# XuyangBai/D3Feat

Hardware: AMD Instinct MI355X
Metric: fragments/sec (30k-pt clouds) (higher is better)
Workload: dtype f32; 1 GPU; SURVEY §8d config #2: synthetic 3DMatch room fragment, 300k raw pts -> grid subsample 0.03 m (~29k pts per cloud) -> self-pair -> 5-level pyramid -> full KPFCNN forward (random-init weights (reference initialiser, seed 42), 14.1M params)...; points_per_cloud=29369, fragments_per_gpu=2141, parallelism=fragment-dp1, fragments_per_replay=12, engine_fallbacks=0, engine_isolated_replays=0

## Files before the change

d3feat_amd/_lib.py:

```python
import ctypes as C
import os

_HERE = os.path.dirname(os.path.abspath(__file__))
LIB_PATH = os.environ.get("D3FEAT_AMD_LIB") or os.path.join(_HERE, "lib", "libd3feat_amd.so")

D3F_OK = 0
ERRORS = {-1: "HIP runtime / kernel launch failure", -2: "workspace too small", -3: "invalid argument"}
ST_EMPTY_ELEMENT, ST_NEG_CELL, ST_KEY_RANGE, ST_HIT_OVERFLOW, ST_OUT_OVERFLOW, ST_KEY_WIDTH = 1, 2, 4, 8, 16, 32
PAD_NUM_SUPPORTS = -2147483648
NEIGHBOR_CAP = 1024
MAX_BATCH = 255
TOPK_MAX = 8192
PAIRS_KMAX = 1024
REPEAT_COUNTS_MAX = 16
MATCH_KMAX = 8192
VALIDATION_NMAX = 1024
SCENES_MAX = 256
VP_INDEX_RANGE, VP_COUNT_RANGE = 1, 2

_vp, _sz, _i, _f = C.c_void_p, C.c_size_t, C.c_int, C.c_float

SIGNATURES = {
    "d3f_version": (_i, []),
    "d3f_trace_marker": (_i, [_i, _vp]),
    "d3f_pack_status": (_i, [_vp, _vp, _i, _vp, _i, _vp, _i, _vp, _i, _vp, _i, _i, _i, _vp]),
    "d3f_grid_subsample_workspace_bytes": (_sz, [_i, _i, _i, _i]),
    "d3f_batch_grid_subsample": (_i, [_vp, _i, _vp, _i, _f, _vp, _i, _vp, _i, _vp, _vp, _vp, _vp, _vp, _vp, _sz, _vp]),
    "d3f_batch_grid_subsample_async": (_i, [_vp, _i, _vp, _i, _f, _vp, _i, _i, _i, _vp, _vp, _vp, _sz, _vp]),
    "d3f_batch_grid_subsample_async_inplace": (_i, [_vp, _i, _vp, _i, _f, _vp, _i, _i, _vp, _vp, _vp, _sz, _vp]),
    "d3f_stack_self_pair": (_i, [_vp, _i, _vp, _i, _vp, _vp, _vp, _vp]),
    "d3f_radius_neighbors_workspace_bytes": (_sz, [_i, _i, _i]),
    "d3f_batch_radius_neighbors": (_i, [_vp, _i, _vp, _i, _vp, _vp, _i, _f, _vp, _i, _i, _i, _vp, _vp, _sz, _vp]),
    "d3f_neighbor_grid_bytes": (_sz, [_i, _i]),
    "d3f_neighbor_grid_order_offset": (_sz, [_i, _i]),
    "d3f_neighbor_grid_build": (_i, [_vp, _i, _vp, _i, _f, _vp, _sz, _vp]),
    "d3f_neighbor_grid_search": (_i, [_vp, _sz, _i, _vp, _i, _vp, _i, _f, _i, _vp, _i, _i, _i, _i, _i, _f, _i, _vp, _vp]),
    "d3f_neighbor_grid_search_ordered": (_i, [_vp, _sz, _i, _vp, _i, _vp, _i, _f, _vp, _sz, _vp, _i, _i, _i, _i, _i, _f, _i, _vp, _vp]),
    "d3f_neighbor_grid_inv_offset": (_sz, [_i, _i]),
    "d3f_neighbor_grid_xyz_offset": (_sz, [_i, _i]),
    "d3f_row_positive": (_i, [_vp, _i, _i, _i, _vp, _vp, _i, _vp]),
    "d3f_kpconv_aggregate": (_i, [_vp, _i, _vp, _i, _vp, _i, _i, _vp, _i, _i, _vp, _vp, _i, _f, _i, _i, _vp, _vp, _vp, _vp,
                                  _vp, _i, _vp]),
    "d3f_kpconv_deform_aggregate": (_i, [_vp, _i, _vp, _i, _vp, _i, _i, _vp, _i, _i, _vp, _i, _f, _vp, _i, _i, _vp, _i, _f, _i, _i, _vp,
                                         _vp, _vp, _vp, _i, _vp]),
    "d3f_kpconv_fused_c1": (_i, [_vp, _i, _vp, _i, _vp, _i, _i, _vp, _i, _vp, _i, _f, _i, _i, _vp, _i, _vp, _vp, _vp, _i, _i,
                                 _f, _vp, _i, _vp, _vp, _vp, _i, _vp]),
    "d3f_kpconv_fused32": (_i, [_vp, _i, _vp, _i, _vp, _i, _i, _vp, _i, _vp, _vp, _i, _f, _i, _i, _vp, _vp, _vp, _vp, _i, _i, _f, _vp,
                                _i, _vp, _vp, _vp, _i, _vp]),
    "d3f_kpconv_fused_supported": (_i, [_i, _i, _i, _i, _i]),
    "d3f_kpconv_pack_weights": (_i, [_vp, _i, _i, _vp, _vp]),
    "d3f_kpconv_fused": (_i, [_vp, _i, _vp, _i, _vp, _i, _i, _vp, _i, _i, _vp, _vp, _i, _f, _i, _i, _vp, _i, _vp, _vp, _vp, _i, _i,
                              _f, _vp, _i, _vp, _vp, _vp, _i, _vp]),
    "d3f_kpconv_fused32_x3": (_i, [_vp, _i, _vp, _i, _vp, _i, _i, _vp, _i, _vp, _vp, _i, _f, _i, _i, _vp, _vp, _vp, _vp, _i, _i, _f, _vp,
                                   _i, _vp, _vp, _vp, _i, _vp]),
    "d3f_kpconv_packed_x3_bytes": (_sz, [_i, _i]),
    "d3f_kpconv_pack_weights_x3": (_i, [_vp, _i, _i, _vp, _vp]),
    "d3f_kpconv_fused_x3": (_i, [_vp, _i, _vp, _i, _vp, _i, _i, _vp, _i, _i, _vp, _vp, _i, _f, _i, _i, _vp, _i, _vp, _vp, _vp, _i, _i,
                                 _f, _vp, _i, _vp, _vp, _vp, _i, _vp]),
    "d3f_gemm_workspace_bytes": (_sz, [_i, _i, _i, _i]),
    "d3f_gemm_bf16_workspace_bytes": (_sz, [_i, _i, _i, _i]),
    "d3f_gemm_f32": (_i, [_vp, _i, _vp, _i, _vp, _i, _i, _i, _i, _vp, _vp, _vp, _vp, _i, _i, _f, _vp, _sz, _vp, _i, _vp]),
    "d3f_gemm_upsample_cat_f32": (_i, [_vp, _i, _i, _i, _vp, _i, _vp, _i, _i, _vp, _i, _vp, _i, _i, _i, _vp, _vp, _i, _f, _vp, _sz,
                                       _vp, _vp, _i, _vp]),
    "d3f_ind_max_pool": (_i, [_vp, _i, _i, _i, _vp, _i, _i, _i, _vp, _i, _vp, _vp, _vp, _vp, _i, _vp]),
    "d3f_closest_pool_cat": (_i, [_vp, _i, _i, _i, _vp, _i, _i, _vp, _i, _i, _vp, _i, _vp, _vp, _vp]),
    "d3f_affine_act": (_i, [_vp, _i, _i, _i, _vp, _vp, _vp, _i, _i, _f, _vp, _i, _vp, _vp]),
    "d3f_pack_descriptors": (_i, [_vp, _vp, _i, _i, _vp, _i, _vp, _i, _vp, _vp]),
    "d3f_pack_descriptors_to": (_i, [_vp, _vp, _i, _i, _vp, _i, _vp, _i, _vp, _vp, _i, _i, _i, _vp, _vp, _vp]),
    "d3f_topk_workspace_bytes": (_sz, [_i, _i, _i, _i]),
    "d3f_topk_records": (_i, [_vp, _i, _vp, _i, _i, _vp, _i, _i, _vp, _vp, _i, _i, _i, _vp, _i, _i, _vp, _i, _vp, _vp, _vp, _vp, _sz,
                              _vp]),
    "d3f_feature_nn_workspace_bytes": (_sz, [_i]),
    "d3f_feature_nn": (_i, [_vp, _i, _i, _vp, _i, _i, _i, _vp, _vp, _vp, _sz, _vp]),
    "d3f_mutual_matches_workspace_bytes": (_sz, [_i]),
    "d3f_mutual_matches": (_i, [_vp, _i, _vp, _i, _vp, _vp, _vp, _sz, _vp]),
    "d3f_ransac_hypotheses": (_i, [_vp, _i, _vp, _i, _vp, _i, _f, _f, C.c_uint64, C.c_uint64, _i, _vp, _vp, _vp]),
    "d3f_ransac_draw": (_i, [C.c_uint64, C.c_uint64, _i, _i]),
    "d3f_neighbor_grid_score": (_i, [_vp, _sz, _i, _vp, _i, _vp, _i, _f, _vp, _vp, _vp, _vp]),
    "d3f_register_pairs_workspace_bytes": (_sz, [_i, _i, _i, _i]),
    "d3f_register_pairs": (_i, [_vp, _i, _i, _i, _i, _vp, _vp, _i, _i, _f, _i, _f, _f, _i, _i, C.c_uint64, _vp, _f] + [_vp] * 11
                           + [_sz, _vp]),
    "d3f_repeatability_pairs": (_i, [_vp, _i, _i, _i, _vp, _vp, _i, _vp, _i, _vp, _vp, _i, _vp, _vp, _vp]),
    "d3f_match_pairs_workspace_bytes": (_sz, [_i, _vp, _i]),
    "d3f_match_pairs": (_i, [_vp, _i, _i, _i, _i, _vp, _vp, _i, _vp, _f, _vp, _i, _vp, _vp, _vp, _sz, _vp]),
    "d3f_register_pairs_counts_workspace_bytes": (_sz, [_i, _i, _i, _vp, _i, _i]),
    "d3f_register_pairs_counts": (_i, [_vp, _i, _i, _i, _i, _vp, _vp, _i, _vp, _i, _f, _i, _f, _f, _i, _i, C.c_uint64, _vp, _f] + [_vp] * 10
                                  + [_sz, _vp]),
    "d3f_overlap_pairs": (_i, [_vp, _sz, _i, _i, _vp, _i, _f, _vp, _vp, _i, _vp]),
    "d3f_validation_pairs_workspace_bytes": (_sz, [_i, _i]),
    "d3f_validation_pairs": (_i, [_vp, _i, _i, _vp, _i, _vp, _i, _i, _vp, _vp, _vp, _i, _vp, _i, _f, _i, _f, _f, _f, _f] + [_vp] * 5
                             + [_sz, _vp]),
    "d3f_pose_errors": (_i, [_vp, _vp, _i, _i, _vp, _vp, _vp, _vp, _vp, _vp]),
    "d3f_sanitize_descriptors": (_i, [_vp, _i, _i, _i, _i, _vp]),
    "d3f_matching_summary": (_i, [_vp, _vp, _vp, _i, _i, _vp, _i, _vp, _vp, _vp, _vp]),
    "d3f_registration_recall": (_i, [_vp, _i, _vp, _vp, _vp, _vp, _vp, _i, _i, _vp, _i, _vp, _vp, _vp, _vp, _vp]),
    "d3f_icp_pairs_workspace_bytes": (_sz, [_i, _i]),
    "d3f_icp_pairs": (_i, [_vp, _sz, _i, _vp, _i, _vp, _i, _vp, _vp, _i, _i] + [_vp] * 9 + [_sz, _vp]),
    "d3f_gemm_pack_bf16": (_i, [_vp, _i, _i, _i, _vp, _vp]),
    "d3f_gemm_pack_f32t": (_i, [_vp, _i, _i, _i, _vp, _vp]),
    "d3f_gemm_f32t": (_i, [_vp, _i, _i, _i, _vp, _i, _vp, _i, _i, _vp, _vp, _i, _i, _i, _vp, _vp, _vp, _vp, _i, _i, _f, _vp, _sz,
                           _vp, _vp, _i, _vp]),
    "d3f_gemm_x3_packed_bytes": (_sz, [_i, _i]),
    "d3f_gemm_pack_x3": (_i, [_vp, _i, _i, _i, _vp, _vp]),
    "d3f_gemm_x3_workspace_bytes": (_sz, [_i, _i, _i, _i]),
    "d3f_gemm_x3_plan": (_i, [_i, _i, _i, _i, _vp, _vp, _vp]),
    "d3f_gemm_x3_resident": (_i, [_i, _i, _i, _i]),
    "d3f_gemm_x3": (_i, [_vp, _i, _i, _i, _vp, _i, _vp, _i, _i, _vp, _vp, _i, _i, _i, _vp, _vp, _vp, _vp, _i, _i, _f, _vp, _sz,
                         _vp, _vp, _i, _vp]),
    "d3f_gemm_x3_gres": (_i, [_vp, _i, _i, _i, _vp, _i, _vp, _i, _i, _vp, _vp, _i, _i, _i, _vp, _vp, _vp, _vp, _i, _vp, _i, _i, _vp, _i, _f,
                              _vp, _sz, _vp, _vp, _i, _vp]),
    "d3f_gemm_bf16": (_i, [_vp, _i, _i, _i, _vp, _i, _vp, _i, _i, _vp, _vp, _i, _i, _i, _vp, _vp, _vp, _vp, _i, _i, _f, _vp, _sz,
                           _vp, _vp, _i, _i, _i, _vp]),
    "d3f_decode_xyz_records": (_i, [_vp, _i, _i, _i, _i, _i, _i, _i, _vp, _vp]),
    "d3f_detect_head": (_i, [_vp, _i, _i, _i, _vp, _i, _i, _vp, _vp, _i, _i, _vp, _i, _vp, _vp, _vp, _vp]),
}

_lib = None

# ... 26 lines not shown
```

d3feat_amd/csrc/grid_subsample.hip:

```cpp
#include <cstdlib>
#include "prims.h"
#include "radix_sort.h"

#define GS_EMPTY 0xFFFFFFFFFFFFFFFFull
#define GS_KEYBITS 56
#define GS_KEYMASK ((1ull << GS_KEYBITS) - 1ull)
#define GS_MAX_PROBE 4096

__constant__ unsigned long long D3F_CHAIN_DEV[D3F_NCHAIN] = {
    13ull, 29ull, 59ull, 127ull, 257ull, 541ull, 1109ull, 2357ull, 5087ull, 10273ull, 20753ull, 42043ull, 85229ull,
    172933ull, 351061ull, 712697ull, 1447153ull, 2938679ull, 5967347ull, 12117689ull, 24607243ull, 49969847ull,
    101473717ull, 206062531ull, 418451333ull, 849749479ull, 1725587117ull, 3504151727ull};

struct GsElem {
    float org[3];
    int pad0;
    unsigned long long NX, NY, NZ;
    long long bbase;
};

static unsigned long long gs_chain_ge(long long n) {
    for (int j = 0; j < D3F_NCHAIN; ++j)
        if ((long long)D3F_CHAIN_HOST[j] >= n) return D3F_CHAIN_HOST[j];
    return D3F_CHAIN_HOST[D3F_NCHAIN - 1];
}

__device__ __forceinline__ unsigned long long gs_mix(unsigned long long x) {
    x ^= x >> 33; x *= 0xff51afd7ed558ccdull; x ^= x >> 33; x *= 0xc4ceb9fe1a85ec53ull; x ^= x >> 33;
    return x;
}

__device__ __forceinline__ int gs_bits(unsigned long long x) {
    int b = 0;
    while (x) { ++b; x >>= 1; }
    return b;
}
__device__ __forceinline__ void gs_prep(const unsigned* __restrict__ bbox, const int* __restrict__ offs, int B, float dl,
                                        GsElem* __restrict__ el, int* __restrict__ status, RsMeta* __restrict__ smeta,
                                        int n_cap) {
    __shared__ unsigned long long sCells[256];
    const int b = threadIdx.x;
    unsigned long long cells = 0ull;
    if (b < B) {
        GsElem e;
        e.pad0 = 0;
        const int len = offs[b + 1] - offs[b];
        if (len <= 0) {
            atomicOr(&status[1], D3F_ST_EMPTY_ELEMENT);
            e.org[0] = e.org[1] = e.org[2] = 0.f;
            e.NX = e.NY = e.NZ = 1;
        } else {
            const float inv = __fdiv_rn(1.0f, dl);
            float mx[3];
#pragma unroll
            for (int d = 0; d < 3; ++d) {
                float mn = d3f_ord2f(__hip_atomic_load(&bbox[b * 6 + d], __ATOMIC_RELAXED, __HIP_MEMORY_SCOPE_AGENT));
                mx[d] = d3f_ord2f(__hip_atomic_load(&bbox[b * 6 + 3 + d], __ATOMIC_RELAXED, __HIP_MEMORY_SCOPE_AGENT));
                e.org[d] = __fmul_rn(floorf(__fmul_rn(mn, inv)), dl);
            }
            e.NX = (unsigned long long)fmaxf(floorf(__fdiv_rn(__fsub_rn(mx[0], e.org[0]), dl)), 0.f) + 1ull;
            e.NY = (unsigned long long)fmaxf(floorf(__fdiv_rn(__fsub_rn(mx[1], e.org[1]), dl)), 0.f) + 1ull;
            e.NZ = (unsigned long long)fmaxf(floorf(__fdiv_rn(__fsub_rn(mx[2], e.org[2]), dl)), 0.f) + 1ull;
        }
        long long base = 0;
        for (int j = 0; j < b; ++j) {
            long long l = offs[j + 1] - offs[j];
            unsigned long long nb = D3F_CHAIN_DEV[D3F_NCHAIN - 1];
            for (int c = 0; c < D3F_NCHAIN; ++c)
                if ((long long)D3F_CHAIN_DEV[c] >= l) { nb = D3F_CHAIN_DEV[c]; break; }
            base += (long long)nb;
        }
        e.bbase = base;
        el[b] = e;
        const double c = (double)e.NX * (double)e.NY * (double)e.NZ;
        cells = c >= 1.8e19 ? 0xFFFFFFFFFFFFFFFFull : e.NX * e.NY * e.NZ;
    }
    if (!smeta) return;
    sCells[threadIdx.x] = cells;
    __syncthreads();
    if (threadIdx.x == 0) {
        unsigned long long mx = 1ull;
        for (int j = 0; j < B; ++j) mx = sCells[j] > mx ? sCells[j] : mx;
        int kb = gs_bits(mx - 1ull);
        if (kb < 1) kb = 1;
        const int eb = gs_bits((unsigned long long)(B - 1));
        RsMeta m;
        m.n = min(offs[B], n_cap);
        m.kb = kb;
        m.bits = kb + eb;
        if (m.bits > 32) {
            atomicOr(&status[1], D3F_ST_KEY_WIDTH);
            m.n = 0;
            m.bits = 8;
        }
        m.npass = (m.bits + 7) / 8;
        *smeta = m;
    }
}
struct GsPrepEpi {
    const unsigned* bbox; const int* offs; int B; float dl; GsElem* el; int* status; RsMeta* smeta; int n_cap;
    __device__ __forceinline__ void operator()() const { gs_prep(bbox, offs, B, dl, el, status, smeta, n_cap); }
};

__global__ void __launch_bounds__(256) gs_insert_kernel(const float* __restrict__ pts, int N, const int* __restrict__ offs,
                                                        int B, float dl, const GsElem* __restrict__ el,
                                                        unsigned long long* __restrict__ tkey, unsigned* __restrict__ tfirst,
                                                        unsigned long long capmask, int* __restrict__ slot,
                                                        int* __restrict__ status) {
    const int i = blockIdx.x * blockDim.x + threadIdx.x;
    if (i >= min(N, offs[B])) return;
    const int b = d3f_find_elem(offs, B, i);
    const GsElem e = el[b];
    const float fx = floorf(__fdiv_rn(__fsub_rn(pts[3 * (size_t)i + 0], e.org[0]), dl));
    const float fy = floorf(__fdiv_rn(__fsub_rn(pts[3 * (size_t)i + 1], e.org[1]), dl));
    const float fz = floorf(__fdiv_rn(__fsub_rn(pts[3 * (size_t)i + 2], e.org[2]), dl));
    int st = 0;
    if (fx < 0.f || fy < 0.f || fz < 0.f) st |= D3F_ST_NEG_CELL;
    const unsigned long long ix = (unsigned long long)fmaxf(fx, 0.f), iy = (unsigned long long)fmaxf(fy, 0.f),
                             iz = (unsigned long long)fmaxf(fz, 0.f);
    const unsigned long long key = ix + e.NX * iy + e.NX * e.NY * iz;
    if (key > GS_KEYMASK) st |= D3F_ST_KEY_RANGE;
    if (st) atomicOr(&status[1], st);
    const unsigned long long word = ((unsigned long long)b << GS_KEYBITS) | (key & GS_KEYMASK);
    unsigned long long h = gs_mix(word) & capmask;
    bool placed = false;
    for (int probe = 0; probe < GS_MAX_PROBE; ++probe) {
        unsigned long long prev = atomicCAS(&tkey[h], GS_EMPTY, word);
        if (prev == GS_EMPTY || prev == word) { placed = true; break; }
        h = (h + 1) & capmask;
    }
    if (!placed) atomicOr(&status[1], D3F_ST_OUT_OVERFLOW);
    atomicMin(&tfirst[h], (unsigned)i);
    slot[i] = (int)h;
}

struct GsMarkIn {
    const int* n_dev; const int* slot; const unsigned* tfirst;
    __device__ __forceinline__ int operator()(int i) const { return (i < *n_dev && tfirst[slot[i]] == (unsigned)i) ? 1 : 0; }
};

__global__ void __launch_bounds__(256) gs_chain_kernel(int N, const int* __restrict__ slot, const unsigned* __restrict__ tfirst,
                                                       const unsigned long long* __restrict__ tkey,
                                                       const int* __restrict__ vscan, const int* __restrict__ vbase,
                                                       int* __restrict__ pvid,
                                                       unsigned long long* __restrict__ vkey, int* __restrict__ vhead,
                                                       int* __restrict__ vcnt, int* __restrict__ pnext,
                                                       const int* __restrict__ n_dev) {
    const int i = blockIdx.x * blockDim.x + threadIdx.x;
    if (i >= min(N, *n_dev)) return;
    const int s = slot[i];
    const int fi = (int)tfirst[s];
    const int v = d3f_scan_at(vscan, vbase, fi);
    pvid[i] = v;
    if (fi == i) vkey[v] = tkey[s] & GS_KEYMASK;
    pnext[i] = atomicExch(&vhead[v], i);
    atomicAdd(&vcnt[v], 1);
}

struct GsRankScan {
    const int* vscan; const int* vbase;
    __device__ __forceinline__ int operator()(int p) const { return d3f_scan_at(vscan, vbase, p); }
};
struct GsRankBits {
    const unsigned* fbits; const int* wscan; const int* wbase;
    __device__ __forceinline__ int operator()(int p) const {
        const int w = p >> 5;
        return d3f_scan_at(wscan, wbase, w) + __popc(fbits[w] & ((1u << (p & 31)) - 1u));
    }
};
template <class Rank>
struct GsMoffsEpi {
    const int* offs; int B; Rank rank; int* meta; int* moffs; int* sub_lens; int* status_dev;
    int out_cap;
    int elem_cap;
    __device__ __forceinline__ void operator()(int M) const {
        if (threadIdx.x != 0) return;
        meta[0] = M;
        const int N = offs[B];
        for (int b = 0; b <= B; ++b) moffs[b] = (b == B || offs[b] >= N) ? M : rank(offs[b]);
        bool over = M > out_cap ||
                    (__hip_atomic_load(&meta[1], __ATOMIC_RELAXED, __HIP_MEMORY_SCOPE_AGENT) & (D3F_ST_OUT_OVERFLOW | D3F_ST_KEY_WIDTH));
        for (int b = 0; b < B; ++b) over = over || (moffs[b + 1] - moffs[b] > elem_cap);
        if (over && !(__hip_atomic_load(&meta[1], __ATOMIC_RELAXED, __HIP_MEMORY_SCOPE_AGENT) & D3F_ST_KEY_WIDTH))
            atomicOr(&meta[1], D3F_ST_OUT_OVERFLOW);
        for (int b = 0; b < B; ++b) {
// ... 343 lines not shown
            const unsigned ix = (unsigned)fmaxf(fx, 0.f), iy = (unsigned)fmaxf(fy, 0.f), iz = (unsigned)fmaxf(fz, 0.f);
            const unsigned k = ix + NX * (iy + NY * iz);
            key[r] = (kb < 32 ? ((unsigned)b << kb) : 0u) | (kb < 32 ? (k & ((1u << kb) - 1u)) : k);
            skey[i] = key[r];
            vm |= 1u << r;
        }
    }
    if (st) atomicOr(&status[1], st);
    rs_tile_histogram(key, vm, 0, sHist, hist + (size_t)tile * 256);
}

__global__ void __launch_bounds__(256) gs_heads_kernel(int N, const RsMeta* __restrict__ smeta, const unsigned* __restrict__ key0,
                                                       const unsigned* __restrict__ key1, const unsigned* __restrict__ val0,
                                                       const unsigned* __restrict__ val1, unsigned* __restrict__ fbits) {
    const int j = blockIdx.x * blockDim.x + threadIdx.x;
    if (j >= min(N, smeta->n)) return;
    const unsigned* __restrict__ ks = (smeta->npass & 1) ? key1 : key0;
    const unsigned* __restrict__ vs = (smeta->npass & 1) ? val1 : val0;
    const unsigned k = ks[j];
    if (j == 0 || ks[j - 1] != k) {
        const unsigned i = vs[j];
        atomicOr(&fbits[i >> 5], 1u << (i & 31u));
    }
}
struct GsBitsIn {
    const unsigned* fbits;
    __device__ __forceinline__ int operator()(int w) const { return __popc(fbits[w]); }
};
__global__ void __launch_bounds__(256) gs_runs_kernel(int N, const RsMeta* __restrict__ smeta, const unsigned* __restrict__ key0,
                                                      const unsigned* __restrict__ key1, const unsigned* __restrict__ val0,
                                                      const unsigned* __restrict__ val1, GsRankBits rank,
                                                      const float* __restrict__ pts, const float* const* __restrict__ ptrs,
                                                      const int* __restrict__ offs, unsigned long long* __restrict__ vkey,
                                                      float* __restrict__ bary) {
    __shared__ float sx[256], sy[256], sz[256];
    __shared__ unsigned sk[256];
    const int n = min(N, smeta->n);
    const int j0 = blockIdx.x * 256;
    if (j0 >= n) return;
    const int t = threadIdx.x, j = j0 + t;
    const unsigned* __restrict__ ks = (smeta->npass & 1) ? key1 : key0;
    const unsigned* __restrict__ vs = (smeta->npass & 1) ? val1 : val0;
    unsigned k = 0u, pi = 0u, kprev = 0u;
    float px = 0.f, py = 0.f, pz = 0.f;
    if (j < n) {
        k = ks[j];
        pi = vs[j];
        kprev = j > 0 ? ks[j - 1] : 0u;
        if (ptrs) {
            const int b = smeta->kb < 32 ? (int)(k >> smeta->kb) : 0;
            pts = ptrs[b] - 3 * (size_t)offs[b];
        }
        px = pts[3 * (size_t)pi + 0]; py = pts[3 * (size_t)pi + 1]; pz = pts[3 * (size_t)pi + 2];
    }
    sx[t] = px; sy[t] = py; sz[t] = pz;
    sk[t] = k;
    __syncthreads();
    if (j >= n || (j != 0 && kprev == k)) return;
    const int v = rank((int)pi);
    float ax = px, ay = py, az = pz;
    int c = 1;
    const int lim = min(256, n - j0);
    while (t + c < lim && sk[t + c] == k) {
        ax = __fadd_rn(ax, sx[t + c]);
        ay = __fadd_rn(ay, sy[t + c]);
        az = __fadd_rn(az, sz[t + c]);
        ++c;
    }
    if (t + c == 256) {
        while (j + c < n && ks[j + c] == k) {
            const size_t q = vs[j + c];
            ax = __fadd_rn(ax, pts[3 * q + 0]);
            ay = __fadd_rn(ay, pts[3 * q + 1]);
            az = __fadd_rn(az, pts[3 * q + 2]);
            ++c;
        }
    }
    const float sc = (float)(1.0 / (double)c);
    vkey[v] = (unsigned long long)(smeta->kb < 32 ? (k & ((1u << smeta->kb) - 1u)) : k);
    bary[3 * (size_t)v + 0] = __fmul_rn(ax, sc);
    bary[3 * (size_t)v + 1] = __fmul_rn(ay, sc);
    bary[3 * (size_t)v + 2] = __fmul_rn(az, sc);
}
__global__ void __launch_bounds__(256) gs_emit_kernel(int* __restrict__ status, const int* __restrict__ moffs, int B,
                                                      const int* __restrict__ vpos, const float* __restrict__ bary,
                                                      float* __restrict__ out_p, int out_cap) {
    const int v = blockIdx.x * blockDim.x + threadIdx.x;
    if (v >= status[0]) return;
    if (status[1] & (D3F_ST_OUT_OVERFLOW | D3F_ST_KEY_WIDTH)) return;
    const int b = d3f_find_elem(moffs, B, v);
    const size_t dest = (size_t)moffs[b] + (size_t)vpos[v];
    if (dest >= (size_t)out_cap) {
        atomicOr(&status[1], D3F_ST_OUT_OVERFLOW);
        return;
    }
    out_p[3 * dest + 0] = bary[3 * (size_t)v + 0];
    out_p[3 * dest + 1] = bary[3 * (size_t)v + 1];
    out_p[3 * dest + 2] = bary[3 * (size_t)v + 2];
}


__global__ void __launch_bounds__(256) gs_accum_kernel(const float* __restrict__ pts, const float* __restrict__ feat,
                                                       int fdim, int* __restrict__ status,
                                                       const int* __restrict__ moffs, int B,
                                                       const int* __restrict__ vstart, const int* __restrict__ sbase,
                                                       const int* __restrict__ vcnt,
                                                       const int* __restrict__ sorted, const int* __restrict__ vpos,
                                                       float* __restrict__ out_p, float* __restrict__ out_f, int out_cap) {
    const int v = blockIdx.x * blockDim.x + threadIdx.x;
    if (v >= status[0]) return;
    const int b = d3f_find_elem(moffs, B, v);
    const int n = vcnt[v], st = sbase ? d3f_scan_at(vstart, sbase, v) : vstart[v];
    const size_t dest = (size_t)moffs[b] + (size_t)vpos[v];
    if (dest >= (size_t)out_cap) {
        atomicOr(&status[1], D3F_ST_OUT_OVERFLOW);
        return;
    }
    float sx = 0.f, sy = 0.f, sz = 0.f;
    for (int t = 0; t < n; ++t) {
        const size_t i = (size_t)sorted[st + t];
        sx = __fadd_rn(sx, pts[3 * i + 0]);
        sy = __fadd_rn(sy, pts[3 * i + 1]);
        sz = __fadd_rn(sz, pts[3 * i + 2]);
    }
    const float sc = (float)(1.0 / (double)n);
    out_p[3 * dest + 0] = __fmul_rn(sx, sc);
    out_p[3 * dest + 1] = __fmul_rn(sy, sc);
    out_p[3 * dest + 2] = __fmul_rn(sz, sc);
    if (fdim > 0) {
        const float cf = (float)n;
        for (int f = 0; f < fdim; ++f) {
            float s = 0.f;
            for (int t = 0; t < n; ++t) s = __fadd_rn(s, feat[(size_t)sorted[st + t] * fdim + f]);
            out_f[dest * fdim + f] = __fdiv_rn(s, cf);
        }
    }
}

__global__ void __launch_bounds__(256) gs_fill_kernel(int* __restrict__ p, size_t n, int v) {
    const size_t i = (size_t)blockIdx.x * blockDim.x + threadIdx.x;
    if (i < n) p[i] = v;
}
__global__ void __launch_bounds__(256) gs_labels_kernel(int N, int ldim, const int* __restrict__ cls,
                                                        const int* __restrict__ pvid, const int* __restrict__ moffs, int B,
                                                        const int* __restrict__ vpos, int* __restrict__ out_c) {
    const int i = blockIdx.x * blockDim.x + threadIdx.x;
    if (i >= N) return;
    const int v = pvid[i];
    const int b = d3f_find_elem(moffs, B, v);
    const size_t dest = (size_t)moffs[b] + (size_t)vpos[v];
    for (int l = 0; l < ldim; ++l) atomicMax(&out_c[dest * ldim + l], cls[(size_t)i * ldim + l]);
}

struct GsLayout {
    size_t cap;
    long long bucket_total;
};
static GsLayout gs_layout(int N, int B, int keys = -1) {
    GsLayout L;
    L.cap = 64;
    const size_t nk = (size_t)((keys > 0 && keys < N) ? keys : (N > 0 ? N : 1));
    while (L.cap < (size_t)2 * nk) L.cap <<= 1;
    L.bucket_total = (long long)(2.24 * (double)N) + 16ll * B + 64;
    return L;
}

extern "C" size_t d3f_grid_subsample_workspace_bytes(int N, int B, int fdim, int ldim) {
    (void)fdim; (void)ldim;
    if (N < 0 || B < 1) return 0;
    GsLayout L = gs_layout(N, B);
    size_t n = (size_t)(N > 0 ? N : 1);
    size_t bytes = 0;
    bytes += d3f_align((B + 1) * sizeof(int)) * 2 + d3f_align((B + 2) * sizeof(int));
    bytes += d3f_align(B * 6 * sizeof(unsigned));
    bytes += d3f_align(B * sizeof(GsElem));
    bytes += d3f_align(L.cap * sizeof(unsigned long long));
    bytes += d3f_align(L.cap * sizeof(int));
    bytes += d3f_align(n * sizeof(unsigned long long));
    bytes += 16 * d3f_align(n * sizeof(int));
    bytes += 6 * d3f_align((size_t)L.bucket_total * sizeof(int));
    bytes += d3f_align((n / GS_TILE + B + 8) * sizeof(int));
    bytes += 2 * d3f_align(d3f_scan_base_ints(N) * sizeof(int)) + d3f_align((4 + D3F_NCHAIN * (size_t)B) * sizeof(unsigned));
    bytes += d3f_align(rs_hist_words(N) * sizeof(unsigned)) + d3f_align((n / 32 + 2) * sizeof(unsigned)) +
             d3f_align(3 * n * sizeof(float)) + d3f_align(sizeof(RsMeta));
    bytes += d3f_align(7 * (size_t)B * (n < 16384 ? n : 16384) * sizeof(float)) + 256 + 2 * d3f_align(B * sizeof(int));
    return bytes + 4096;
}

template <int T, int R>
static int gs_small_launch(const GsSmallArgs& A, float* sub_points, int* sub_lens_dev, int* status_dev, hipStream_t stream) {
    static std::atomic<unsigned long long> lds_done{0ull};
    const void* const fns[] = {(const void*)gs_small_kernel<T, R>};
    if (d3f_opt_in_lds(lds_done, fns, (int)gss_lds_bytes<T, R>(GSS_NB_MAX)) != D3F_OK) return D3F_ERR_HIP;
    gs_small_kernel<T, R><<<A.B, T, gss_lds_bytes<T, R>(A.nbmax), stream>>>(A);
    D3F_LAUNCH_CHECK();
    gs_small_pack_kernel<<<d3f_cdiv(A.out_cap, 256), 256, 0, stream>>>(A, sub_points, sub_lens_dev, status_dev);
    D3F_LAUNCH_CHECK();
    return D3F_OK;
}
static int gs_run_small(const float* points, int N, const int* lens_dev, int B, float dl, float* sub_points, int M_cap, int elem_cap,
                        int pc, int* sub_lens_dev, int* status_dev, void* workspace, size_t workspace_bytes, hipStream_t stream) {
    if (elem_cap <= 0 || elem_cap > M_cap) elem_cap = M_cap;
    if (elem_cap > pc) elem_cap = pc;
    D3fArena ar(workspace, workspace_bytes);
    GsSmallArgs A;
    A.stage = ar.take<float>(3 * (size_t)B * (size_t)elem_cap);
    A.recs = ar.take<float>(4 * (size_t)B * (size_t)elem_cap);
    A.mcount = ar.take<int>(B);
    A.cflags = ar.take<int>(B);
    if (!ar.ok) return D3F_ERR_WORKSPACE;
    A.pts = points; A.lens = lens_dev; A.B = B; A.dl = dl; A.elem_cap = elem_cap; A.pc = pc; A.out_cap = M_cap;
    A.nbmax = GSS_NB_MAX;
    for (int j = 0; j < D3F_NCHAIN; ++j)
        if ((long long)D3F_CHAIN_HOST[j] >= (long long)elem_cap) { A.nbmax = (int)D3F_CHAIN_HOST[j]; break; }
    if (A.nbmax > GSS_NB_MAX) A.nbmax = GSS_NB_MAX;
    if (A.nbmax < 1109) A.nbmax = 1109;
    if (pc <= 2048) return gs_small_launch<256, 8>(A, sub_points, sub_lens_dev, status_dev, stream);
    if (pc <= 4096) return gs_small_launch<512, 8>(A, sub_points, sub_lens_dev, status_dev, stream);
    if (pc <= 8192) return gs_small_launch<1024, 8>(A, sub_points, sub_lens_dev, status_dev, stream);
    if (pc <= 12288) return gs_small_launch<1024, 12>(A, sub_points, sub_lens_dev, status_dev, stream);
    return gs_small_launch<1024, 16>(A, sub_points, sub_lens_dev, status_dev, stream);
}

static int gs_run(const float* points, int N, const int* lens_dev, int B, float dl, const float* features, int fdim,
                  const int* classes, int ldim, float* sub_points, int M_cap, int elem_cap, int elem_points, float* sub_features,
                  int* sub_classes, int* sub_lens_dev, int* status_host, int* status_dev, void* workspace,
                  size_t workspace_bytes, hipStream_t stream, const float* const* ptrs = nullptr) {
    const bool async = status_dev != nullptr;
    if (async && !features && ldim == 0 && !ptrs) {
        const int pc = (elem_points > 0 && elem_points < N) ? elem_points : N;
        int ec = (elem_cap > 0 && elem_cap < M_cap) ? elem_cap : M_cap;
        if (ec > pc) ec = pc;
        if (pc <= 16384 && ec <= GSS_NB_MAX) return gs_run_small(points, N, lens_dev, B, dl, sub_points, M_cap, elem_cap, pc, sub_lens_dev, status_dev,
                                             workspace, workspace_bytes, stream);
    }
    GsLayout L = gs_layout(N, B, async ? M_cap : -1);
    D3fArena ar(workspace, workspace_bytes);
    const size_t n = (size_t)N;
    int* offs = ar.take<int>(B + 1);
    int* moffs = ar.take<int>(B + 1);
    unsigned* bbox = ar.take<unsigned>(B * 6);
    GsElem* el = ar.take<GsElem>(B);
    const int ncounters = 4 + D3F_NCHAIN * B;
    unsigned* counters = ar.take<unsigned>(ncounters);
    unsigned long long* tkey = ar.take<unsigned long long>(L.cap);
    unsigned* tfirst = ar.take<unsigned>(L.cap);
    int* vhead = ar.take<int>(n);
    int* meta = ar.take<int>(B + 2);
    int* vcnt = ar.take<int>(n);
    unsigned long long* vkey = ar.take<unsigned long long>(n);
    int* slot = ar.take<int>(n);
    int* vscan = ar.take<int>(n);
    int* pvid = ar.take<int>(n);
    int* pnext = ar.take<int>(n);
    int* vstart = ar.take<int>(n);
    int* sorted = ar.take<int>(n);
    GsOrderArgs A;
    A.vpos = ar.take<int>(n);
    A.P[0] = ar.take<int>(n);
    A.P[1] = ar.take<int>(n);
    A.nx[0] = ar.take<int>(n);
    A.nx[1] = ar.take<int>(n);
    A.cd = ar.take<int>(n);
    A.bkt[0] = ar.take<int>(n);
    A.bkt[1] = ar.take<int>(n);
    for (int k = 0; k < 2; ++k) {
        A.bf[k] = ar.take<int>((size_t)L.bucket_total);
        A.bc[k] = ar.take<int>((size_t)L.bucket_total);
        A.bh[k] = ar.take<int>((size_t)L.bucket_total);
    }
    A.tsum = ar.take<int>(n / GS_TILE + B + 8);
    int* vbase = ar.take<int>(d3f_scan_base_ints(N));
    int* sbase = ar.take<int>(d3f_scan_base_ints(N));
    const bool use_sort = async && !features && ldim == 0;
    unsigned* rs_hist = ar.take<unsigned>(rs_hist_words(N));
    unsigned* fbits = ar.take<unsigned>(n / 32 + 2);
    float* bary = ar.take<float>(3 * n);
    RsMeta* smeta = ar.take<RsMeta>(1);
    if (!ar.ok) return D3F_ERR_WORKSPACE;
    A.vkey = vkey; A.moffs = moffs; A.offs = offs; A.el = el;
    if (elem_cap <= 0 || elem_cap > M_cap) elem_cap = M_cap;
    if (elem_cap > N) elem_cap = N;
    A.max_m = async ? elem_cap : 0x7fffffff;

    int rc;
    const D3fFill none{nullptr, 0ull, 0u};
    const unsigned long long ones_words = (unsigned long long)((char*)(vhead + n) - (char*)tkey) / 4ull;
    const unsigned long long zero_words = (unsigned long long)((char*)(vcnt + n) - (char*)meta) / 4ull;
    if ((rc = use_sort ? d3f_begin_launch(lens_dev, B, offs, bbox, counters, ncounters, D3fFill{fbits, (unsigned long long)(n / 32 + 2), 0u},
                                          D3fFill{(unsigned*)meta, (unsigned long long)(B + 2), 0u}, none, none, stream)
                       : d3f_begin_launch(lens_dev, B, offs, bbox, counters, ncounters, D3fFill{(unsigned*)tkey, ones_words, 0xFFFFFFFFu},
                                          D3fFill{(unsigned*)meta, zero_words, 0u}, none, none, stream)) != D3F_OK) return rc;
    GsPrepEpi prep{bbox, offs, B, dl, el, meta, use_sort ? smeta : nullptr, N};
    if ((rc = d3f_bbox_launch_t(points, offs, B, N, bbox, counters, prep, stream, ptrs)) != D3F_OK) return rc;
    const int nblk = d3f_cdiv(N, 256);
    const int elem_lim = async ? elem_cap : 0x7fffffff;
    int M, maxM;
    if (use_sort) {
        unsigned *key0 = (unsigned*)slot, *key1 = (unsigned*)pnext, *val0 = (unsigned*)pvid, *val1 = (unsigned*)sorted;
        gs_sortkey_kernel<<<rs_tiles(N), RS_THREADS, 0, stream>>>(points, ptrs, offs, B, dl, el, smeta, key0, rs_hist, meta);
        D3F_LAUNCH_CHECK();
        if ((rc = rs_sort_launch(smeta, N, key0, key1, val0, val1, rs_hist, stream)) != D3F_OK) return rc;
        gs_heads_kernel<<<nblk, 256, 0, stream>>>(N, smeta, key0, key1, val0, val1, fbits);
        D3F_LAUNCH_CHECK();
        const GsRankBits rank{fbits, vscan, vbase};
        GsMoffsEpi<GsRankBits> mepi{offs, B, rank, meta, moffs, sub_lens_dev, status_dev, M_cap, elem_lim};
        if ((rc = d3f_scan_fold_launch(GsBitsIn{fbits}, N / 32 + 1, nullptr, vscan, vbase, counters + 1, mepi, stream)) != D3F_OK)
            return rc;
        gs_runs_kernel<<<nblk, 256, 0, stream>>>(N, smeta, key0, key1, val0, val1, rank, points, ptrs, offs, vkey, bary);
        D3F_LAUNCH_CHECK();
        M = N < M_cap ? N : M_cap;
        maxM = elem_cap;
    } else {
    GsMoffsEpi<GsRankScan> mepi{offs, B, GsRankScan{vscan, vbase}, meta, moffs, sub_lens_dev, status_dev, M_cap, elem_lim};
    gs_insert_kernel<<<nblk, 256, 0, stream>>>(points, N, offs, B, dl, el, tkey, tfirst, (unsigned long long)L.cap - 1ull,
                                               slot, meta);
    D3F_LAUNCH_CHECK();
    if ((rc = d3f_scan_fold_launch(GsMarkIn{offs + B, slot, tfirst}, N, offs + B, vscan, vbase, counters + 1, mepi, stream)) != D3F_OK)
        return rc;
    if (!async) {
        D3F_HIP_TRY(hipMemcpyAsync(status_host, meta, (B + 2) * sizeof(int), hipMemcpyDeviceToHost, stream));
        D3F_HIP_TRY(hipStreamSynchronize(stream));
        M = status_host[0];
        if (status_host[1] != 0 || M <= 0) return D3F_OK;
        maxM = 0;
        for (int b = 0; b < B; ++b) maxM = status_host[2 + b] > maxM ? status_host[2 + b] : maxM;
    } else {
        M = N < M_cap ? N : M_cap;
        maxM = elem_cap;
    }

    gs_chain_kernel<<<nblk, 256, 0, stream>>>(N, slot, tfirst, tkey, vscan, vbase, pvid, vkey, vhead, vcnt, pnext, offs + B);
    D3F_LAUNCH_CHECK();
    if ((rc = d3f_scan_fold_launch(D3fScanIn{vcnt}, async ? N : M, meta, vstart, sbase, counters + 2, D3fNoEpi{}, stream)) != D3F_OK)
        return rc;
    gs_rank_kernel<<<nblk, 256, 0, stream>>>(N, offs + B, pvid, vhead, pnext, vstart, sbase, sorted);
    }
    const int small_last = GS_SMALL_LAST;
    gs_order_small_kernel<<<B, GS_SMALL_T, 0, stream>>>(A, small_last);
    for (int j = small_last + 1; j < D3F_NCHAIN && (long long)D3F_CHAIN_HOST[j - 1] < (long long)maxM; ++j) {
        const long long nbj = (long long)D3F_CHAIN_HOST[j];
        const int hi = (int)((long long)maxM < nbj ? (long long)maxM : nbj);
        const bool more = j + 1 < D3F_NCHAIN && nbj < (long long)maxM;
        const long long nbn = more ? (long long)D3F_CHAIN_HOST[j + 1] : 0;
        const int hin = more ? (int)((long long)maxM < nbn ? (long long)maxM : nbn) : hi;
        dim3 g(d3f_cdiv(hi, 256), B), gt(d3f_cdiv(hi, GS_TILE), B), gp(d3f_cdiv(hin > hi ? hin : hi, 256), B);
        if (j == small_last + 1) gs_order_insert_kernel<<<g, 256, 0, stream>>>(A, j);
        gs_order_scan_tiles_kernel<<<gt, 256, 0, stream>>>(A, j, B, counters + 4 + j * B);
        gs_order_place_kernel<<<gp, 256, 0, stream>>>(A, j);
    }
    if (use_sort)
        gs_emit_kernel<<<d3f_cdiv(M, 256), 256, 0, stream>>>(meta, moffs, B, A.vpos, bary, sub_points, M_cap);
    else
        gs_accum_kernel<<<d3f_cdiv(async ? N : M, 256), 256, 0, stream>>>(points, features, fdim, meta, moffs, B, vstart, sbase,
                                                                         vcnt, sorted, A.vpos, sub_points, sub_features, M_cap);
    if (ldim > 0) {
        const size_t tot = (size_t)M * (size_t)ldim;
        gs_fill_kernel<<<d3f_cdiv((long long)tot, 256), 256, 0, stream>>>(sub_classes, tot, (int)0x80000000);
        gs_labels_kernel<<<nblk, 256, 0, stream>>>(N, ldim, classes, pvid, moffs, B, A.vpos, sub_classes);
    }
    D3F_LAUNCH_CHECK();
    return D3F_OK;
}

extern "C" int d3f_batch_grid_subsample(const float* points, int N, const int* lens_dev, int B, float dl,
                                        const float* features, int fdim, const int* classes, int ldim,
                                        float* sub_points, float* sub_features, int* sub_classes, int* sub_lens_dev,
                                        int* status_host, void* workspace, size_t workspace_bytes, void* stream_) {
    hipStream_t stream = (hipStream_t)stream_;
    if (N < 0 || N > (1 << 30) || B < 1 || B > D3F_MAX_BATCH || !(dl > 0.f) || fdim < 0 || ldim < 0) return D3F_ERR_ARG;
    if (!points || !lens_dev || !sub_points || !sub_lens_dev || !status_host) return D3F_ERR_ARG;
    if ((fdim > 0 && (!features || !sub_features)) || (ldim > 0 && (!classes || !sub_classes))) return D3F_ERR_ARG;
    for (int i = 0; i < B + 2; ++i) status_host[i] = 0;
    if (N == 0) return d3f_fill_u32(sub_lens_dev, B, 0u, stream);
    return gs_run(points, N, lens_dev, B, dl, features, fdim, classes, ldim, sub_points, N, N, 0, sub_features, sub_classes,
                  sub_lens_dev, status_host, nullptr, workspace, workspace_bytes, stream);
}

extern "C" int d3f_batch_grid_subsample_async(const float* points, int N_cap, const int* lens_dev, int B, float dl,
                                              float* sub_points, int M_cap, int elem_cap, int elem_points_cap, int* sub_lens_dev,
                                              int* status_dev, void* workspace, size_t workspace_bytes, void* stream_) {
    hipStream_t stream = (hipStream_t)stream_;
    if (N_cap < 1 || N_cap > (1 << 30) || M_cap < 1 || elem_cap < 0 || elem_points_cap < 0 || B < 1 || B > D3F_MAX_BATCH || !(dl > 0.f))
        return D3F_ERR_ARG;
    if (!points || !lens_dev || !sub_points || !sub_lens_dev || !status_dev) return D3F_ERR_ARG;
    return gs_run(points, N_cap, lens_dev, B, dl, nullptr, 0, nullptr, 0, sub_points, M_cap, elem_cap, elem_points_cap, nullptr,
                  nullptr, sub_lens_dev, nullptr, status_dev, workspace, workspace_bytes, stream);
}

extern "C" int d3f_batch_grid_subsample_async_inplace(const float* const* clouds_dev, int N_cap, const int* lens_dev, int B, float dl,
                                                      float* sub_points, int M_cap, int elem_cap, int* sub_lens_dev, int* status_dev,
                                                      void* workspace, size_t workspace_bytes, void* stream_) {
    hipStream_t stream = (hipStream_t)stream_;
    if (N_cap < 1 || N_cap > (1 << 30) || M_cap < 1 || elem_cap < 0 || B < 1 || B > D3F_MAX_BATCH || !(dl > 0.f)) return D3F_ERR_ARG;
    if (!clouds_dev || !lens_dev || !sub_points || !sub_lens_dev || !status_dev) return D3F_ERR_ARG;
    return gs_run(nullptr, N_cap, lens_dev, B, dl, nullptr, 0, nullptr, 0, sub_points, M_cap, elem_cap, 0, nullptr, nullptr, sub_lens_dev,
                  nullptr, status_dev, workspace, workspace_bytes, stream, clouds_dev);
}

__global__ void __launch_bounds__(256) gs_stack_pair_kernel(const float* __restrict__ pts, int M_cap, const int* __restrict__ lens_in,
                                                            int B, float* __restrict__ out, int* __restrict__ lens_out,
                                                            int* __restrict__ total) {
    const int i = blockIdx.x * blockDim.x + threadIdx.x;
    int tot = 0;
    for (int b = 0; b < B; ++b) tot += lens_in[b];
    tot = min(tot, M_cap);
    if (i == 0) {
        int room = M_cap;
        for (int b = 0; b < B; ++b) {
            const int m = min(lens_in[b], room);
            room -= m;
            lens_out[2 * b] = m;
            lens_out[2 * b + 1] = m;
        }
        *total = 2 * tot;
    }
    if (i >= 3 * tot) return;
    const int pi = i / 3, c = i - 3 * pi;
    int start = 0, m = 0;
    for (int b = 0; b < B; ++b) {
        m = lens_in[b];
        if (pi < start + m || b == B - 1) break;
        start += m;
    }
    m = min(m, tot - start);
    const float v = pts[i];
    const size_t row = 2 * (size_t)start + (size_t)(pi - start);
    out[3 * row + c] = v;
    out[3 * (row + m) + c] = v;
}

extern "C" int d3f_stack_self_pair(const float* pts, int M_cap, const int* lens_in_dev, int B, float* out, int* lens_out_dev,
                                   int* total_dev, void* stream_) {
    hipStream_t stream = (hipStream_t)stream_;
    if (M_cap < 1 || B < 1 || 2 * B > D3F_MAX_BATCH || !pts || !lens_in_dev || !out || !lens_out_dev || !total_dev)
        return D3F_ERR_ARG;
    gs_stack_pair_kernel<<<d3f_cdiv(3ll * M_cap, 256), 256, 0, stream>>>(pts, M_cap, lens_in_dev, B, out, lens_out_dev, total_dev);
    D3F_LAUNCH_CHECK();
    return D3F_OK;
}
```

d3feat_amd/csrc/gs_small.h:

```cpp
#pragma once

#define GSS_NB_MAX 5087

struct GsSmallArgs {
    const float* pts;
    const int* lens;
    int B;
    float dl;
    float* stage;
    float* recs;
    int elem_cap;
    int pc;
    int out_cap;
    int nbmax;
    int* mcount;
    int* cflags;
};

template <int T>
__device__ __forceinline__ int gss_block_excl_scan(int v, int* __restrict__ wsum, int* total) {
    const int lane = threadIdx.x & 63, w = threadIdx.x >> 6;
    int x = v;
#pragma unroll
    for (int d = 1; d < 64; d <<= 1) {
        const int y = __shfl_up(x, d, 64);
        if (lane >= d) x += y;
    }
    if (lane == 63) wsum[w] = x;
    __syncthreads();
    int base = 0, tot = 0;
#pragma unroll
    for (int q = 0; q < T / 64; ++q) {
        const int s = wsum[q];
        if (q < w) base += s;
        tot += s;
    }
    __syncthreads();
    *total = tot;
    return base + x - v;
}

template <int T, int R>
static inline size_t gss_lds_bytes(int nbmax) {
    const size_t sortw = 2 * (size_t)T * R + (size_t)(T / 64) * 256 + 2 * ((size_t)T * R / 32);
    const size_t orderw = 7 * (size_t)nbmax;
    return (128 + (sortw > orderw ? sortw : orderw)) * 4;
}

template <int T, int R>
__global__ void __launch_bounds__(T) gs_small_kernel(GsSmallArgs A) {
    extern __shared__ __attribute__((aligned(16))) unsigned gss_lds[];
    constexpr int W = T / 64, NI = T * R;
    int* sScr = (int*)gss_lds;
    unsigned* sK = gss_lds + 128;
    unsigned* sV = sK + NI;
    unsigned (*sCnt)[256] = (unsigned (*)[256])(sV + NI);
    unsigned* sBits = sV + NI + W * 256;
    int* sWS = (int*)(sBits + NI / 32);
    const int b = blockIdx.x, tid = threadIdx.x, lane = tid & 63, w = tid >> 6;
    int lo = 0;
    for (int j = 0; j < b; ++j) lo += A.lens[j];
    const int len = A.lens[b];
    int* sFlag = sScr + 127;
    if (tid == 0) { A.mcount[b] = 0; *sFlag = 0; }
    if (len <= 0 || len > NI || len > A.pc) {
        if (tid == 0) A.cflags[b] = len <= 0 ? D3F_ST_EMPTY_ELEMENT : D3F_ST_OUT_OVERFLOW;
        return;
    }
    const float* __restrict__ P = A.pts + 3 * (size_t)lo;
    const float dl = A.dl;

    unsigned mn[3] = {0xFFFFFFFFu, 0xFFFFFFFFu, 0xFFFFFFFFu}, mx[3] = {0u, 0u, 0u};
    for (int i = tid; i < len; i += T) {
#pragma unroll
        for (int d = 0; d < 3; ++d) {
            const unsigned u = d3f_f2ord(P[3 * (size_t)i + d]);
            mn[d] = min(mn[d], u);
            mx[d] = max(mx[d], u);
        }
    }
#pragma unroll
    for (int d = 0; d < 3; ++d) {
#pragma unroll
        for (int o = 32; o > 0; o >>= 1) {
            mn[d] = min(mn[d], (unsigned)__shfl_xor((int)mn[d], o, 64));
            mx[d] = max(mx[d], (unsigned)__shfl_xor((int)mx[d], o, 64));
        }
    }
    if (lane == 0) {
#pragma unroll
        for (int d = 0; d < 3; ++d) { sScr[w * 6 + d] = (int)mn[d]; sScr[w * 6 + 3 + d] = (int)mx[d]; }
    }
    __syncthreads();
    float org[3];
    unsigned dims[3];
    {
        const float inv = __fdiv_rn(1.0f, dl);
#pragma unroll
        for (int d = 0; d < 3; ++d) {
// ... 129 lines not shown
    }

    float4* __restrict__ rec = (float4*)A.recs + (size_t)b * (size_t)A.elem_cap;
#pragma unroll
    for (int r = 0; r < R; ++r) {
        if (headmask & (1u << r)) {
            const int i = base + r * 64;
            const unsigned k = key[r];
            unsigned pi = val[r];
            const int vid = sWS[pi >> 5] + __popc(sBits[pi >> 5] & ((1u << (pi & 31u)) - 1u));
            float sx = P[3 * (size_t)pi + 0], sy = P[3 * (size_t)pi + 1], sz = P[3 * (size_t)pi + 2];
            int c = 1;
            while (i + c < len && sK[i + c] == k) {
                pi = sV[i + c];
                sx = __fadd_rn(sx, P[3 * (size_t)pi + 0]);
                sy = __fadd_rn(sy, P[3 * (size_t)pi + 1]);
                sz = __fadd_rn(sz, P[3 * (size_t)pi + 2]);
                ++c;
            }
            const float sc = (float)(1.0 / (double)c);
            rec[vid] = make_float4(__fmul_rn(sx, sc), __fmul_rn(sy, sc), __fmul_rn(sz, sc), __uint_as_float(k));
        }
    }
    __syncthreads();

    const int NB = A.nbmax;
    unsigned* sKey = gss_lds + 128;
    int* sBF = (int*)(sKey + NB);
    int* sBC = sBF + NB;
    int* sBH = sBC + NB;
    int* sNX = sBH + NB;
    int* sL0 = sNX + NB;
    int* sL1 = sL0 + NB;
    for (int v = tid; v < M; v += T) sKey[v] = __float_as_uint(rec[v].w);
    __syncthreads();
    int* La = sL0;
    int* Lb = sL1;
    int lo_r = 0;
    for (int j = 0; j < D3F_NCHAIN; ++j) {
        const int nb = (int)D3F_CHAIN_DEV[j];
        const double inv_nb = 1.0 / (double)nb;
        const bool last = M <= nb;
        const int hi = last ? M : nb;
        for (int t = tid; t < nb; t += T) { sBF[t] = 0x7fffffff; sBC[t] = 0; sBH[t] = -1; }
        __syncthreads();
        for (int t = tid; t < hi; t += T) {
            const int id = (t < lo_r) ? La[t] : t;
            const int bk = gs_mod((unsigned long long)sKey[id], (unsigned)nb, inv_nb);
            atomicMin(&sBF[bk], t);
            atomicAdd(&sBC[bk], 1);
            sNX[t] = atomicExch(&sBH[bk], t);
        }
        __syncthreads();
        int carry = 0;
        for (int c0 = 0; c0 < hi; c0 += T) {
            const int u = c0 + tid, t = hi - 1 - u;
            int c = 0, bk = 0;
            if (u < hi) {
                const int id = (t < lo_r) ? La[t] : t;
                bk = gs_mod((unsigned long long)sKey[id], (unsigned)nb, inv_nb);
                c = (sBF[bk] == t) ? sBC[bk] : 0;
            }
            int tot;
            const int e = gss_block_excl_scan<T>(c, sScr, &tot);
            if (u < hi && sBF[bk] == t) sBC[bk] = carry + e;
            carry += tot;
        }
        __syncthreads();
        for (int t = tid; t < hi; t += T) {
            const int id = (t < lo_r) ? La[t] : t;
            const int bk = gs_mod((unsigned long long)sKey[id], (unsigned)nb, inv_nb);
            int rk = 0;
            for (int q = sBH[bk]; q >= 0; q = sNX[q]) rk += (q > t) ? 1 : 0;
            const int dest = sBC[bk] + rk;
            if (last) Lb[id] = dest;
            else Lb[dest] = id;
        }
        __syncthreads();
        int* tmp = La; La = Lb; Lb = tmp;
        if (last) break;
        lo_r = hi;
    }
    float* __restrict__ out = A.stage + 3 * (size_t)b * (size_t)A.elem_cap;
    for (int v = tid; v < M; v += T) {
        const float4 q = rec[v];
        const size_t d = (size_t)La[v];
        out[3 * d + 0] = q.x;
        out[3 * d + 1] = q.y;
        out[3 * d + 2] = q.z;
    }
    if (tid == 0) { A.mcount[b] = M; A.cflags[b] = *sFlag; }
}

__global__ void __launch_bounds__(256) gs_small_pack_kernel(GsSmallArgs A, float* __restrict__ out, int* __restrict__ sub_lens,
                                                            int* __restrict__ status_dev) {
    __shared__ int sOff[D3F_MAX_BATCH + 1];
    if (threadIdx.x == 0) {
        int s = 0;
        for (int b = 0; b < A.B; ++b) { sOff[b] = s; s += A.mcount[b]; }
        sOff[A.B] = s;
    }
    __syncthreads();
    const int M = sOff[A.B];
    int flags = 0;
    for (int b = 0; b < A.B; ++b) flags |= A.cflags[b];
    const bool over = M > A.out_cap || (flags & (D3F_ST_OUT_OVERFLOW | D3F_ST_KEY_WIDTH));
    if (blockIdx.x == 0) {
        for (int b = threadIdx.x; b < A.B; b += 256) sub_lens[b] = over ? 0 : A.mcount[b];
        if (threadIdx.x == 0) {
            const int fl = flags | ((M > A.out_cap) ? D3F_ST_OUT_OVERFLOW : 0);
            status_dev[0] = over ? 0 : M;
            status_dev[1] = fl;
        }
    }
    if (over) return;
    const int i = blockIdx.x * 256 + threadIdx.x;
    if (i >= M) return;
    int b = 0;
    while (b + 1 < A.B && i >= sOff[b + 1]) ++b;
    const float* __restrict__ src = A.stage + 3 * ((size_t)b * (size_t)A.elem_cap + (size_t)(i - sOff[b]));
    out[3 * (size_t)i + 0] = src[0];
    out[3 * (size_t)i + 1] = src[1];
    out[3 * (size_t)i + 2] = src[2];
}
```

d3feat_amd/csrc/prims.h:

```cpp
#pragma once
#include "common.h"

#define D3F_SCAN_TILE 1024

struct D3fFill {
    unsigned* p;
    unsigned long long n;
    unsigned v;
};

__device__ __forceinline__ bool d3f_last_block(unsigned* counter, unsigned nblocks) {
    __shared__ int last_flag;
    asm volatile("s_waitcnt vmcnt(0)" ::: "memory");
    __syncthreads();
    if (threadIdx.x == 0) {
        __builtin_amdgcn_fence(__ATOMIC_RELEASE, "agent");
        asm volatile("s_waitcnt vmcnt(0)" ::: "memory");
        const unsigned t = atomicAdd(counter, 1u);
        last_flag = (t == nblocks - 1u) ? 1 : 0;
        if (last_flag) __builtin_amdgcn_fence(__ATOMIC_ACQUIRE, "agent");
    }
    __syncthreads();
    return last_flag != 0;
}

static __global__ void __launch_bounds__(256) begin_kernel(const int* __restrict__ lens, int B, int* __restrict__ offs,
                                                    unsigned* __restrict__ bbox, unsigned* __restrict__ counters,
                                                    int ncounters, D3fFill f0, D3fFill f1, D3fFill f2, D3fFill f3) {
    const size_t tid = (size_t)blockIdx.x * blockDim.x + threadIdx.x, stride = (size_t)gridDim.x * blockDim.x;
    if (blockIdx.x == 0) {
        if (threadIdx.x == 0 && lens) {
            int s = 0;
            for (int b = 0; b < B; ++b) { offs[b] = s; s += lens[b]; }
            offs[B] = s;
        }
        if (bbox)
            for (int i = threadIdx.x; i < B * 6; i += blockDim.x) bbox[i] = ((i % 6) < 3) ? 0xFFFFFFFFu : 0u;
        for (int i = threadIdx.x; i < ncounters; i += blockDim.x) counters[i] = 0u;
    }
    const D3fFill f[4] = {f0, f1, f2, f3};
#pragma unroll
    for (int k = 0; k < 4; ++k) {
        unsigned* p = f[k].p;
        const size_t n = (size_t)f[k].n;
        if (n == 0) continue;
        const size_t n4 = (((uintptr_t)p & 15) == 0) ? n / 4 : 0;
        const uint4 v4 = make_uint4(f[k].v, f[k].v, f[k].v, f[k].v);
        for (size_t j = tid; j < n4; j += stride) ((uint4*)p)[j] = v4;
        for (size_t j = n4 * 4 + tid; j < n; j += stride) p[j] = f[k].v;
    }
}

static inline int d3f_begin_launch(const int* lens, int B, int* offs, unsigned* bbox, unsigned* counters, int ncounters,
                                   D3fFill f0, D3fFill f1, D3fFill f2, D3fFill f3, hipStream_t stream) {
    const unsigned long long words = f0.n + f1.n + f2.n + f3.n;
    long long blocks = (long long)(words / 4 / 256) + 1;
    if (blocks > 1024) blocks = 1024;
    begin_kernel<<<(int)blocks, 256, 0, stream>>>(lens, B, offs, bbox, counters, ncounters, f0, f1, f2, f3);
    D3F_LAUNCH_CHECK();
    return D3F_OK;
}

template <class Epi>
__global__ void __launch_bounds__(256) bbox_kernel(const float* __restrict__ pts, const float* const* __restrict__ ptrs,
                                                   const int* __restrict__ offs, int B,
                                                   unsigned* __restrict__ bbox, unsigned* __restrict__ counter, Epi epi) {
    const int b = blockIdx.y;
    const int lo = offs[b], hi = offs[b + 1];
    if (ptrs) pts = ptrs[b] - 3 * (size_t)lo;
    unsigned mn[3] = {0xFFFFFFFFu, 0xFFFFFFFFu, 0xFFFFFFFFu}, mx[3] = {0u, 0u, 0u};
    const int stride = gridDim.x * blockDim.x;
    for (int i = lo + blockIdx.x * blockDim.x + threadIdx.x; i < hi; i += 4 * stride) {
        float v[4][3];
#pragma unroll
        for (int u = 0; u < 4; ++u) {
            const int iu = min(i + u * stride, hi - 1);
#pragma unroll
            for (int d = 0; d < 3; ++d) v[u][d] = pts[3 * (size_t)iu + d];
        }
#pragma unroll
        for (int u = 0; u < 4; ++u) {
#pragma unroll
            for (int d = 0; d < 3; ++d) {
                const unsigned x = d3f_f2ord(v[u][d]);
                mn[d] = min(mn[d], x);
                mx[d] = max(mx[d], x);
            }
        }
    }
#pragma unroll
    for (int d = 0; d < 3; ++d) {
#pragma unroll
        for (int o = 32; o > 0; o >>= 1) {
            mn[d] = min(mn[d], (unsigned)__shfl_xor((int)mn[d], o, 64));
            mx[d] = max(mx[d], (unsigned)__shfl_xor((int)mx[d], o, 64));
        }
    }
    __shared__ unsigned red[4][6];
    const int wv = threadIdx.x >> 6;
    if ((threadIdx.x & 63) == 0) {
#pragma unroll
        for (int d = 0; d < 3; ++d) { red[wv][d] = mn[d]; red[wv][3 + d] = mx[d]; }
    }
    __syncthreads();
    if (threadIdx.x < 6 && lo < hi) {
        unsigned v = red[0][threadIdx.x];
        for (int k = 1; k < 4; ++k) v = (threadIdx.x < 3) ? min(v, red[k][threadIdx.x]) : max(v, red[k][threadIdx.x]);
        if (threadIdx.x < 3) atomicMin(&bbox[b * 6 + threadIdx.x], v);
        else atomicMax(&bbox[b * 6 + threadIdx.x], v);
    }
    if (d3f_last_block(counter, gridDim.x * gridDim.y)) epi();
}

template <class Epi>
static inline int d3f_bbox_launch_t(const float* pts, const int* offs, int B, int N, unsigned* bbox, unsigned* counter, Epi epi,
                                    hipStream_t stream, const float* const* ptrs = nullptr) {
    int chunks = d3f_cdiv(d3f_cdiv(N > 0 ? N : 1, B), 256 * 8);
    const int per_elem = 512 / B > 1 ? 512 / B : 1;
    if (chunks > per_elem) chunks = per_elem;
    bbox_kernel<Epi><<<dim3(chunks, B), 256, 0, stream>>>(pts, ptrs, offs, B, bbox, counter, epi);
    D3F_LAUNCH_CHECK();
    return D3F_OK;
}

__device__ __forceinline__ int d3f_block_excl_scan_256(int v, int* lds4, int* total) {
    const int lane = threadIdx.x & 63, w = threadIdx.x >> 6;
    int x = v;
#pragma unroll
    for (int d = 1; d < 64; d <<= 1) {
        const int y = __shfl_up(x, d, 64);
        if (lane >= d) x += y;
    }
    if (lane == 63) lds4[w] = x;
    __syncthreads();
    int base = 0, tot = 0;
#pragma unroll
    for (int i = 0; i < 4; ++i) {
        const int s = lds4[i];
        if (i < w) base += s;
        tot += s;
    }
    __syncthreads();
    *total = tot;
    return base + x - v;
}

__device__ __forceinline__ int d3f_scan_at(const int* __restrict__ local, const int* __restrict__ base, int i) {
    return local[i] + base[i / D3F_SCAN_TILE];
}

template <class In, class Epi>
__global__ void __launch_bounds__(256) scan_fold_kernel(In in, int n, const int* __restrict__ n_dev, int* __restrict__ local,
                                                        int* __restrict__ base, unsigned* __restrict__ counter, Epi epi) {
    __shared__ int lds[4];
    n = d3f_dyn(n, n_dev);
    const int live = max(1, (n + D3F_SCAN_TILE - 1) / D3F_SCAN_TILE);
    if ((int)blockIdx.x >= live) return;
    const int i0 = blockIdx.x * D3F_SCAN_TILE + threadIdx.x * 4;
    int v[4], s = 0;
#pragma unroll
    for (int k = 0; k < 4; ++k) {
        v[k] = (i0 + k < n) ? in(i0 + k) : 0;
        s += v[k];
    }
    int tot;
    int ex = d3f_block_excl_scan_256(s, lds, &tot);
#pragma unroll
    for (int k = 0; k < 4; ++k) {
        if (i0 + k < n) local[i0 + k] = ex;
        ex += v[k];
    }
    if (threadIdx.x == 0) base[blockIdx.x] = tot;
    if (!d3f_last_block(counter, (unsigned)live)) return;
    const int nblocks = live;
    int carry = 0;
    for (int c = 0; c < nblocks; c += 256) {
        const int i = c + threadIdx.x;
        const int x = (i < nblocks) ? __hip_atomic_load(&base[i], __ATOMIC_RELAXED, __HIP_MEMORY_SCOPE_AGENT) : 0;
        int t;
        const int e = d3f_block_excl_scan_256(x, lds, &t);
        if (i < nblocks) base[i] = carry + e;
        carry += t;
    }
    __syncthreads();
    epi(carry);
}

struct D3fScanIn {
    const int* p;
    __device__ __forceinline__ int operator()(int i) const { return p[i]; }
};
struct D3fNoEpi {
    __device__ __forceinline__ void operator()(int) const {}
    __device__ __forceinline__ void operator()() const {}
};

static inline size_t d3f_scan_base_ints(int n) { return (size_t)d3f_cdiv(n > 0 ? n : 1, D3F_SCAN_TILE) + 64; }

template <class In, class Epi>
static inline int d3f_scan_fold_launch(In in, int n, const int* n_dev, int* local, int* base, unsigned* counter, Epi epi,
                                       hipStream_t stream) {
    const int nb = d3f_cdiv(n > 0 ? n : 1, D3F_SCAN_TILE);
    scan_fold_kernel<In, Epi><<<nb, 256, 0, stream>>>(in, n, n_dev, local, base, counter, epi);
    D3F_LAUNCH_CHECK();
    return D3F_OK;
}
```

d3feat_amd/csrc/radius_neighbors.hip:

```cpp
#include "prims.h"
#include <cstdlib>

struct NbElem {
    double mn[3];
    double inv_h;
    int dims[3];
    int cbase;
};

#define NB_WAVES_PER_BLOCK 4
#define NB_EL_LDS 40

__device__ __forceinline__ void nb_prep(const unsigned* __restrict__ bbox, const int* __restrict__ soffs, int B, float radius,
                                        long long cell_budget, NbElem* __restrict__ el, int* __restrict__ ncells_total) {
    if (threadIdx.x != 0) return;
    long long base = 0;
    const long long per = cell_budget / B;
    for (int b = 0; b < B; ++b) {
        NbElem e;
        const int len = soffs[b + 1] - soffs[b];
        if (len <= 0) {
            e.mn[0] = e.mn[1] = e.mn[2] = 0.0;
            e.inv_h = 1.0;
            e.dims[0] = e.dims[1] = e.dims[2] = 1;
        } else {
            double mx[3];
            for (int d = 0; d < 3; ++d) {
                e.mn[d] = (double)d3f_ord2f(__hip_atomic_load(&bbox[b * 6 + d], __ATOMIC_RELAXED, __HIP_MEMORY_SCOPE_AGENT));
                mx[d] = (double)d3f_ord2f(__hip_atomic_load(&bbox[b * 6 + 3 + d], __ATOMIC_RELAXED, __HIP_MEMORY_SCOPE_AGENT));
            }
            double h = (double)radius * (1.0 + 1.0 / 1048576.0);
            if (!(h > 0.0)) h = 1.0;
            bool fits = false;
            for (int it = 0; it < 64; ++it) {
                e.inv_h = 1.0 / h;
                double tot = 1.0;
                for (int d = 0; d < 3; ++d) {
                    double n = floor((mx[d] - e.mn[d]) * e.inv_h) + 1.0;
                    e.dims[d] = (n < 1073741824.0) ? (int)n : 1073741824;
                    tot *= n;
                }
                if (tot <= (double)per) { fits = true; break; }
                h *= 2.0;
            }
            if (!fits) {
                e.mn[0] = e.mn[1] = e.mn[2] = 0.0;
                e.inv_h = 0.0;
                e.dims[0] = e.dims[1] = e.dims[2] = 1;
            }
        }
        e.cbase = (int)base;
        base += (long long)e.dims[0] * e.dims[1] * e.dims[2];
        el[b] = e;
    }
    ncells_total[0] = (int)base;
    ncells_total[1] = (int)base + 1;
}

struct NbPrepEpi {
    const unsigned* bbox; const int* soffs; int B; float radius; long long cell_budget; NbElem* el; int* ncells;
    __device__ __forceinline__ void operator()() const { nb_prep(bbox, soffs, B, radius, cell_budget, el, ncells); }
};

__device__ __forceinline__ void nb_cell_of(const NbElem& e, float x, float y, float z, int& cx, int& cy, int& cz) {
    cx = (int)floor(((double)x - e.mn[0]) * e.inv_h);
    cy = (int)floor(((double)y - e.mn[1]) * e.inv_h);
    cz = (int)floor(((double)z - e.mn[2]) * e.inv_h);
}

__global__ void __launch_bounds__(256) nb_count_kernel(const float* __restrict__ s, int Ns, const int* __restrict__ soffs,
                                                       int B, const NbElem* __restrict__ el, int* __restrict__ cell_of,
                                                       int* __restrict__ cell_cnt) {
    const int i = blockIdx.x * blockDim.x + threadIdx.x;
    if (i >= min(Ns, soffs[B])) return;
    const int b = d3f_find_elem(soffs, B, i);
    const NbElem e = el[b];
    int cx, cy, cz;
    nb_cell_of(e, s[3 * (size_t)i], s[3 * (size_t)i + 1], s[3 * (size_t)i + 2], cx, cy, cz);
    cx = min(max(cx, 0), e.dims[0] - 1);
    cy = min(max(cy, 0), e.dims[1] - 1);
    cz = min(max(cz, 0), e.dims[2] - 1);
    const int c = e.cbase + cx + e.dims[0] * (cy + e.dims[1] * cz);
    cell_of[i] = c;
    atomicAdd(&cell_cnt[c], 1);
}

__global__ void __launch_bounds__(256) nb_scatter_kernel(const float* __restrict__ s, int Ns, const int* __restrict__ ns_dev,
                                                         const int* __restrict__ cell_of,
                                                         const int* __restrict__ cell_start, const int* __restrict__ cell_base,
                                                         int* __restrict__ cell_cur,
                                                         float4* __restrict__ sorted, int* __restrict__ order,
                                                         int* __restrict__ inv, float* __restrict__ xyz) {
    const int i = blockIdx.x * blockDim.x + threadIdx.x;
    if (i >= min(Ns, *ns_dev)) return;
    const int c = cell_of[i];
    const int pos = d3f_scan_at(cell_start, cell_base, c) + atomicAdd(&cell_cur[c], 1);
    const float x = s[3 * (size_t)i], y = s[3 * (size_t)i + 1], z = s[3 * (size_t)i + 2];
    sorted[pos] = make_float4(x, y, z, __int_as_float(i));
    order[pos] = i;
    inv[i] = pos;
    xyz[3 * (size_t)pos] = x; xyz[3 * (size_t)pos + 1] = y; xyz[3 * (size_t)pos + 2] = z;
}

template <int J>
__device__ __forceinline__ unsigned nb_xor_lane(unsigned v) {
    if constexpr (J == 1) return (unsigned)__builtin_amdgcn_mov_dpp((int)v, 0xB1, 0xF, 0xF, true);
    else if constexpr (J == 2) return (unsigned)__builtin_amdgcn_mov_dpp((int)v, 0x4E, 0xF, 0xF, true);
    else return (unsigned)__builtin_amdgcn_ds_swizzle((int)v, (J << 10) | 0x1F);
}
template <int J>
__device__ __forceinline__ void nb_cmpx(unsigned& hi, unsigned& lo, bool take_min) {
    const unsigned phi = nb_xor_lane<J>(hi), plo = nb_xor_lane<J>(lo);
    const bool p_less = (phi < hi) || (phi == hi && plo < lo);
    const bool take_p = (take_min == p_less);
    hi = take_p ? phi : hi;
    lo = take_p ? plo : lo;
}
__device__ __forceinline__ void nb_bitonic64(int lane, unsigned& h0, unsigned& l0, unsigned& h1, unsigned& l1) {
#define NB_STAGE(K_, J_)                                                                         \
    do {                                                                                         \
        const bool low_ = (lane & (J_)) == 0;                                                    \
        const bool up0_ = ((K_) >= 32) ? true : ((lane & (K_)) == 0);                            \
        const bool up1_ = ((K_) == 64) ? true : (((K_) == 32) ? false : ((lane & (K_)) == 0));   \
        nb_cmpx<J_>(h0, l0, up0_ == low_);                                                       \
        nb_cmpx<J_>(h1, l1, up1_ == low_);                                                       \
    } while (0)
    NB_STAGE(2, 1);
    NB_STAGE(4, 2); NB_STAGE(4, 1);
    NB_STAGE(8, 4); NB_STAGE(8, 2); NB_STAGE(8, 1);
    NB_STAGE(16, 8); NB_STAGE(16, 4); NB_STAGE(16, 2); NB_STAGE(16, 1);
    NB_STAGE(32, 16); NB_STAGE(32, 8); NB_STAGE(32, 4); NB_STAGE(32, 2); NB_STAGE(32, 1);
    {
        const bool swap = (h1 < h0) || (h1 == h0 && l1 < l0);
        const unsigned th = swap ? h1 : h0, tl = swap ? l1 : l0;
        h1 = swap ? h0 : h1; l1 = swap ? l0 : l1;
        h0 = th; l0 = tl;
    }
    NB_STAGE(64, 16); NB_STAGE(64, 8); NB_STAGE(64, 4); NB_STAGE(64, 2); NB_STAGE(64, 1);
#undef NB_STAGE
}

__device__ __forceinline__ void nb_cmpx_own(unsigned& ha, unsigned& la, unsigned& hb, unsigned& lb, bool ascending) {
    const bool b_less = (hb < ha) || (hb == ha && lb < la);
    const bool swap = (b_less == ascending);
    const unsigned th = swap ? hb : ha, tl = swap ? lb : la;
    hb = swap ? ha : hb; lb = swap ? la : lb;
    ha = th; la = tl;
}
__device__ __forceinline__ void nb_bitonic64x16(int lane, unsigned (&h)[4], unsigned (&l)[4]) {
#define NB_UP(K_, S_) (((K_) == 64) ? true : ((K_) >= 16 ? ((((S_) * 16) & (K_)) == 0) : ((lane & (K_)) == 0)))
#define NB_XSTAGE(K_, J_)                                                                        \
    do {                                                                                         \
        const bool low_ = (lane & (J_)) == 0;                                                    \
        nb_cmpx<J_>(h[0], l[0], NB_UP(K_, 0) == low_);                                           \
        nb_cmpx<J_>(h[1], l[1], NB_UP(K_, 1) == low_);                                           \
        nb_cmpx<J_>(h[2], l[2], NB_UP(K_, 2) == low_);                                           \
        nb_cmpx<J_>(h[3], l[3], NB_UP(K_, 3) == low_);                                           \
    } while (0)
    NB_XSTAGE(2, 1);
    NB_XSTAGE(4, 2); NB_XSTAGE(4, 1);
    NB_XSTAGE(8, 4); NB_XSTAGE(8, 2); NB_XSTAGE(8, 1);
    NB_XSTAGE(16, 8); NB_XSTAGE(16, 4); NB_XSTAGE(16, 2); NB_XSTAGE(16, 1);
    nb_cmpx_own(h[0], l[0], h[1], l[1], true);
    nb_cmpx_own(h[2], l[2], h[3], l[3], false);
    NB_XSTAGE(32, 8); NB_XSTAGE(32, 4); NB_XSTAGE(32, 2); NB_XSTAGE(32, 1);
    nb_cmpx_own(h[0], l[0], h[2], l[2], true);
    nb_cmpx_own(h[1], l[1], h[3], l[3], true);
    nb_cmpx_own(h[0], l[0], h[1], l[1], true);
    nb_cmpx_own(h[2], l[2], h[3], l[3], true);
    NB_XSTAGE(64, 8); NB_XSTAGE(64, 4); NB_XSTAGE(64, 2); NB_XSTAGE(64, 1);
#undef NB_XSTAGE
#undef NB_UP
}

template <bool FIRST_ONLY, int LPQ, bool HINT>
__device__ __forceinline__ void
nb_search_body(const float* __restrict__ q, int Nq, const int* __restrict__ qlens, int B,
               const NbElem* __restrict__ el, const int* __restrict__ cell_start, const int* __restrict__ cell_base,
               const float4* __restrict__ sorted,
               const float4* __restrict__ qorder, float r2, int pad, const int* __restrict__ ns_dev, int* __restrict__ out,
               int ld, int width, int cap, int* __restrict__ status, int want_kmax, float nn_hint, const int* __restrict__ inv) {
    extern __shared__ __attribute__((aligned(16))) char smem[];
    constexpr int QPB = 64 * NB_WAVES_PER_BLOCK / LPQ;
    const int grp = threadIdx.x / LPQ, lane = threadIdx.x % LPQ;
// ... 110 lines not shown
    };
    if (FIRST_ONLY && HINT) {
        scan(true);
        if (!(n > 0 && bd2 <= 0.998f * nn_hint * nn_hint)) scan(false);
    } else {
        scan(false);
    }
    if (lane == 0) {
        if (want_kmax && n > __hip_atomic_load(&status[0], __ATOMIC_RELAXED, __HIP_MEMORY_SCOPE_AGENT)) atomicMax(&status[0], n);
        if (!FIRST_ONLY && n > cap) atomicOr(&status[1], D3F_ST_HIT_OVERFLOW);
    }
    int* row = out + (size_t)(inv ? wq : qi) * ld;
    if (FIRST_ONLY) {
        if (lane == 0 && width > 0) row[0] = (n > 0) ? (inv ? inv[bidx] : bidx) : pad;
        for (int j = 1 + lane; j < width; j += LPQ) row[j] = pad;
        return;
    }
    const int m = min(n, cap);
    const int m4 = (m + 3) & ~3;
    if (m + lane < m4) { hd2[m + lane] = 3.4e38f; hidx[m + lane] = 0x7fffffff; }
    __builtin_amdgcn_fence(__ATOMIC_RELEASE, "wavefront");
    __builtin_amdgcn_wave_barrier();
    if (LPQ == 16 && n <= 64 && cap >= 64) {
        unsigned h[4], l4[4];
#pragma unroll
        for (int sl = 0; sl < 4; ++sl) {
            h[sl] = 0xFFFFFFFFu; l4[sl] = 0xFFFFFFFFu;
            if (lane + 16 * sl < m) { h[sl] = __float_as_uint(hd2[lane + 16 * sl]); l4[sl] = (unsigned)hidx[lane + 16 * sl]; }
        }
        nb_bitonic64x16(lane, h, l4);
        const int mw = min(m, width);
#pragma unroll
        for (int sl = 0; sl < 4; ++sl)
            if (lane + 16 * sl < mw) row[lane + 16 * sl] = inv ? inv[(int)l4[sl]] : (int)l4[sl];
        for (int j = m + lane; j < width; j += LPQ) row[j] = pad;
        return;
    }
    if (LPQ == 32 && n <= 64 && cap >= 64) {
        unsigned h0 = 0xFFFFFFFFu, l0 = 0xFFFFFFFFu, h1 = 0xFFFFFFFFu, l1 = 0xFFFFFFFFu;
        if (lane < m) { h0 = __float_as_uint(hd2[lane]); l0 = (unsigned)hidx[lane]; }
        if (lane + 32 < m) { h1 = __float_as_uint(hd2[lane + 32]); l1 = (unsigned)hidx[lane + 32]; }
        nb_bitonic64(lane, h0, l0, h1, l1);
        const int mw = min(m, width);
        if (lane < mw) row[lane] = inv ? inv[(int)l0] : (int)l0;
        if (lane + 32 < mw) row[lane + 32] = inv ? inv[(int)l1] : (int)l1;
        for (int j = m + lane; j < width; j += LPQ) row[j] = pad;
        return;
    }
    for (int e0 = 0; e0 < m; e0 += LPQ) {
        const int ei = e0 + lane;
        if (ei < m) {
            const float kd = hd2[ei];
            const int ki = hidx[ei];
            int rank = 0;
            for (int j = 0; j < m4; j += 4) {
                const float4 dj = *(const float4*)&hd2[j];
                const int4 ij = *(const int4*)&hidx[j];
                rank += (dj.x < kd || (dj.x == kd && ij.x < ki)) ? 1 : 0;
                rank += (dj.y < kd || (dj.y == kd && ij.y < ki)) ? 1 : 0;
                rank += (dj.z < kd || (dj.z == kd && ij.z < ki)) ? 1 : 0;
                rank += (dj.w < kd || (dj.w == kd && ij.w < ki)) ? 1 : 0;
            }
            if (rank < width) row[rank] = inv ? inv[ki] : ki;
        }
    }
    for (int j = m + lane; j < width; j += LPQ) row[j] = pad;
}

template <bool FIRST_ONLY, int LPQ, bool HINT>
__global__ void __launch_bounds__(64 * NB_WAVES_PER_BLOCK)
nb_search_kernel(const float* __restrict__ q, int Nq, const int* __restrict__ qlens, int B,
                 const NbElem* __restrict__ el, const int* __restrict__ cell_start, const int* __restrict__ cell_base,
                 const float4* __restrict__ sorted,
                 const float4* __restrict__ qorder, float r2, int pad, const int* __restrict__ ns_dev, int* __restrict__ out,
                 int ld, int width, int cap, int* __restrict__ status, int want_kmax, float nn_hint, const int* __restrict__ inv) {
    nb_search_body<FIRST_ONLY, LPQ, HINT>(q, Nq, qlens, B, el, cell_start, cell_base, sorted, qorder, r2, pad, ns_dev, out, ld, width,
                                          cap, status, want_kmax, nn_hint, inv);
}

#include "nb_cell_search.h"
#include "nb_nearest.h"
#include "nb_overlap.h"

static long long nb_cell_budget(int Ns) {
    long long b = 4ll * (long long)(Ns > 0 ? Ns : 1);
    if (b < (1ll << 16)) b = 1ll << 16;
    if (b > (1ll << 28)) b = 1ll << 28;
    return b;
}

struct NbGrid {
    int* soffs; unsigned* bbox; NbElem* el; int* ncells; unsigned* counters; int* cell_cnt; int* cell_cur; int* cell_start; int* cell_of;
    float4* sorted; int* order; int* stmp;
    int* inv;
    float* xyz;
    long long cells;
    bool ok;
};
static NbGrid nb_carve(void* ws, size_t bytes, int Ns, int B) {
    NbGrid g;
    g.cells = nb_cell_budget(Ns) + 8;
    D3fArena ar(ws, bytes);
    const size_t ns = (size_t)(Ns > 0 ? Ns : 1);
    g.soffs = ar.take<int>(B + 1);
    g.bbox = ar.take<unsigned>(B * 6);
    g.el = ar.take<NbElem>(B);
    g.ncells = ar.take<int>(16);
    g.counters = (unsigned*)(g.ncells + 8);
    g.cell_cnt = ar.take<int>((size_t)g.cells * 2);
    g.cell_cur = g.cell_cnt ? g.cell_cnt + g.cells : nullptr;
    g.cell_start = ar.take<int>((size_t)g.cells);
    g.cell_of = ar.take<int>(ns);
    g.sorted = ar.take<float4>(ns);
    g.order = ar.take<int>(ns);
    g.stmp = ar.take<int>(d3f_scan_base_ints((int)g.cells));
    g.inv = ar.take<int>(ns);
    g.xyz = ar.take<float>(3 * ns);
    g.ok = ar.ok;
    return g;
}

extern "C" size_t d3f_neighbor_grid_bytes(int Ns, int B) {
    if (Ns < 0 || B < 1) return 0;
    const long long cells = nb_cell_budget(Ns) + 8;
    const size_t ns = (size_t)(Ns > 0 ? Ns : 1);
    size_t bytes = 0;
    bytes += d3f_align((B + 1) * sizeof(int)) + d3f_align(B * 6 * sizeof(unsigned)) + d3f_align(B * sizeof(NbElem)) + d3f_align(64);
    bytes += d3f_align((size_t)cells * 2 * sizeof(int)) + d3f_align((size_t)cells * sizeof(int));
    bytes += 2 * d3f_align(ns * sizeof(int)) + d3f_align(ns * sizeof(float4));
    bytes += d3f_align(d3f_scan_base_ints((int)cells) * sizeof(int));
    bytes += d3f_align(ns * sizeof(int)) + d3f_align(3 * ns * sizeof(float));
    return bytes + 1024;
}

extern "C" size_t d3f_neighbor_grid_order_offset(int Ns, int B) {
    if (Ns < 0 || B < 1) return 0;
    NbGrid g = nb_carve((void*)0x1000, (size_t)1 << 60, Ns, B);
    return (size_t)((char*)g.order - (char*)0x1000);
}

extern "C" size_t d3f_neighbor_grid_inv_offset(int Ns, int B) {
    if (Ns < 0 || B < 1) return 0;
    NbGrid g = nb_carve((void*)0x1000, (size_t)1 << 60, Ns, B);
    return (size_t)((char*)g.inv - (char*)0x1000);
}
extern "C" size_t d3f_neighbor_grid_xyz_offset(int Ns, int B) {
    if (Ns < 0 || B < 1) return 0;
    NbGrid g = nb_carve((void*)0x1000, (size_t)1 << 60, Ns, B);
    return (size_t)((char*)g.xyz - (char*)0x1000);
}

extern "C" int d3f_neighbor_grid_build(const float* supports, int Ns, const int* s_lens_dev, int B, float radius,
                                       void* grid, size_t grid_bytes, void* stream_) {
    hipStream_t stream = (hipStream_t)stream_;
    if (Ns < 0 || B < 1 || B > D3F_MAX_BATCH || !(radius >= 0.f) || !s_lens_dev || (Ns > 0 && !supports) || !grid)
        return D3F_ERR_ARG;
    NbGrid g = nb_carve(grid, grid_bytes, Ns, B);
    if (!g.ok) return D3F_ERR_WORKSPACE;
    int rc;
    const D3fFill none{nullptr, 0ull, 0u};
    if ((rc = d3f_begin_launch(s_lens_dev, B, g.soffs, g.bbox, g.counters, 2,
                               D3fFill{(unsigned*)g.cell_cnt, (unsigned long long)g.cells * 2ull, 0u}, none, none, none,
                               stream)) != D3F_OK) return rc;
    NbPrepEpi prep{g.bbox, g.soffs, B, radius, nb_cell_budget(Ns), g.el, g.ncells};
    if ((rc = d3f_bbox_launch_t(supports, g.soffs, B, Ns, g.bbox, g.counters, prep, stream)) != D3F_OK) return rc;
    if (Ns > 0) {
        nb_count_kernel<<<d3f_cdiv(Ns, 256), 256, 0, stream>>>(supports, Ns, g.soffs, B, g.el, g.cell_of, g.cell_cnt);
        D3F_LAUNCH_CHECK();
    }
    if ((rc = d3f_scan_fold_launch(D3fScanIn{g.cell_cnt}, (int)g.cells, g.ncells + 1, g.cell_start, g.stmp, g.counters + 1, D3fNoEpi{},
                                   stream)) != D3F_OK) return rc;
    if (Ns > 0) {
        nb_scatter_kernel<<<d3f_cdiv(Ns, 256), 256, 0, stream>>>(supports, Ns, g.soffs + B, g.cell_of, g.cell_start, g.stmp,
                                                                 g.cell_cur, g.sorted, g.order, g.inv, g.xyz);
        D3F_LAUNCH_CHECK();
    }
    return D3F_OK;
}

static int nb_env(const char* name, int dflt) {
    const char* e = getenv(name);
    return e ? atoi(e) : dflt;
}
static int nb_search_dispatch(const NbGrid& g, const float* queries, int Nq, const int* q_lens_dev, int B, float radius,
                              const float4* qsorted, bool queries_are_supports, int* out, int ld, int width, int pad_value, int cap,
                              int first_only, float nn_hint, int want_kmax, int* status_dev, hipStream_t stream, bool internal = false) {
    const float r2 = radius * radius;
    if (internal && !qsorted) return D3F_ERR_ARG;
    const int* inv = internal ? g.inv : nullptr;
    if (first_only && !want_kmax) {
        const int mode = nb_env("D3F_NB_NEAREST", 1);
        if (mode == 2 || (mode == 1 && Nq >= 40000)) {
            const int blocks = d3f_cdiv(Nq, 64);
            if (nn_hint > 0.f)
                nb_nearest_kernel<true><<<blocks, 256, 0, stream>>>(queries, Nq, q_lens_dev, B, g.el, g.cell_start, g.stmp, g.sorted, qsorted,
                                                                    r2, pad_value, g.soffs + B, out, ld, width, nn_hint, inv);
            else
                nb_nearest_kernel<false><<<blocks, 256, 0, stream>>>(queries, Nq, q_lens_dev, B, g.el, g.cell_start, g.stmp, g.sorted, qsorted,
                                                                     r2, pad_value, g.soffs + B, out, ld, width, nn_hint, inv);
            D3F_LAUNCH_CHECK();
            return D3F_OK;
        }
    }
    if (!first_only && queries_are_supports) {
        const int mode = nb_env("D3F_NB_CELL", 1);
        if (mode == 2 || (mode == 1 && (Nq >= 40000 || Nq < 6000))) {
            cap = (cap + 1) & ~1;
            const int q_forced = nb_env("D3F_NBC_Q", 0);
            int Q = q_forced > 0 ? q_forced : Nq / 2048;
            Q = Q < 1 ? 1 : (Q > 16 ? 16 : Q);
            if (Q > NBC_QMAX) Q = NBC_QMAX;
            const int dbg = nb_env("D3F_NBC_DBG", 0);
            const char* prof_env = getenv("D3F_NBC_PROF");
            unsigned long long* prof = prof_env ? (unsigned long long*)strtoull(prof_env, nullptr, 16) : nullptr;
            const int blocks = d3f_cdiv(d3f_cdiv(Nq, Q), 4);
            const size_t lds = (size_t)4 * ((size_t)cap * 8 + NBC_BATCH * 64 * 8);
            if (inv)
                nb_cell_search_kernel<true, true><<<blocks, 256, lds, stream>>>(queries, Nq, q_lens_dev, B, g.el, g.cell_start, g.stmp, g.sorted, r2,
                                                                                pad_value, g.soffs + B, out, ld, width, cap, status_dev, want_kmax, Q, dbg, prof, inv);
            else
                nb_cell_search_kernel<true, false><<<blocks, 256, lds, stream>>>(queries, Nq, q_lens_dev, B, g.el, g.cell_start, g.stmp, g.sorted, r2,
                                                                                 pad_value, g.soffs + B, out, ld, width, cap, status_dev, want_kmax, Q, dbg, prof, inv);
            D3F_LAUNCH_CHECK();
            return D3F_OK;
        }
    }
    cap = (cap + 3) & ~3;
    const int lpq = cap > 256 ? 64 : (Nq >= 100000 ? 16 : 32);
    const int qpb = 64 * NB_WAVES_PER_BLOCK / lpq;
    const int blocks = d3f_cdiv(Nq, qpb);
    const size_t lds = first_only ? 0 : (size_t)qpb * cap * 2 * sizeof(float);
    const int kcap = first_only ? 1 : cap;
#define D3F_NB(FO_, LPQ_)                                                                                              \
    if (FO_ && nn_hint > 0.f)                                                                                          \
        nb_search_kernel<FO_, LPQ_, FO_><<<blocks, 64 * NB_WAVES_PER_BLOCK, lds, stream>>>(                             \
            queries, Nq, q_lens_dev, B, g.el, g.cell_start, g.stmp, g.sorted, qsorted, r2, pad_value, g.soffs + B, out, ld, width, \
            kcap, status_dev, want_kmax, nn_hint, inv);                                                                \
    else                                                                                                               \
    nb_search_kernel<FO_, LPQ_, false><<<blocks, 64 * NB_WAVES_PER_BLOCK, lds, stream>>>(                               \
        queries, Nq, q_lens_dev, B, g.el, g.cell_start, g.stmp, g.sorted, qsorted, r2, pad_value, g.soffs + B, out, ld, width, \
        kcap, status_dev, want_kmax, nn_hint, inv)
    if (first_only) { if (lpq == 64) D3F_NB(true, 64); else if (lpq == 32) D3F_NB(true, 32); else D3F_NB(true, 16); }
    else { if (lpq == 64) D3F_NB(false, 64); else if (lpq == 32) D3F_NB(false, 32); else D3F_NB(false, 16); }
#undef D3F_NB
    D3F_LAUNCH_CHECK();
    return D3F_OK;
}

extern "C" int d3f_neighbor_grid_search_ordered(const void* grid, size_t grid_bytes, int Ns, const float* queries, int Nq,
                                                const int* q_lens_dev, int B, float radius, const void* query_grid,
                                                size_t query_grid_bytes, int* out, int ld, int width, int pad_value, int cap,
                                                int first_only, float nn_hint, int flags, int* status_dev, void* stream_) {
    hipStream_t stream = (hipStream_t)stream_;
    if (Nq < 0 || Ns < 0 || B < 1 || B > D3F_MAX_BATCH || width < 0 || ld < width || !(radius >= 0.f)) return D3F_ERR_ARG;
    if (!(nn_hint >= 0.f) || nn_hint >= radius) nn_hint = 0.f;
    if (cap < 1 || cap > D3F_NEIGHBOR_CAP) return D3F_ERR_ARG;
    if (!grid || !status_dev || !q_lens_dev || (Nq > 0 && (!queries || (width > 0 && !out)))) return D3F_ERR_ARG;
    if (flags & 1) { int rc0 = d3f_fill_u32(status_dev, 2, 0u, stream); if (rc0 != D3F_OK) return rc0; }
    const int want_kmax = (flags & D3F_NB_NO_KMAX) ? 0 : 1;
    if (Nq == 0) return D3F_OK;
    NbGrid g = nb_carve((void*)grid, grid_bytes, Ns, B);
    if (!g.ok) return D3F_ERR_WORKSPACE;
    const float4* qsorted = nullptr;
    bool same = false;
    if (query_grid == grid) {
        if (Nq != Ns) return D3F_ERR_ARG;
// ... 140 lines not shown
```

d3feat_amd/datasets/common.py:

```python
import time

import numpy as np
import torch

from .. import _lib, ops
from .. import tf_custom_ops


def tf_batch_subsampling(points, batches_len, sampleDl):
    return tf_custom_ops.batch_grid_subsampling(points, batches_len, sampleDl)


def tf_batch_neighbors(queries, supports, q_batches, s_batches, radius):
    return tf_custom_ops.batch_ordered_neighbors(queries, supports, q_batches, s_batches, radius)


def _host_lens(lens):
    return ops.host_lens(lens)


class Dataset:

    def __init__(self, name):
        self.name = name
# ... 127 lines not shown
            else:
                input_neighbors.append(empty_i)
            if pooled:
                if 'deformable' in block:
                    r = r_normal * config.density_parameter / (config.KP_extent * 2.5)
                else:
                    r = r_normal
                request(pool_p, stacked_points, pool_b, stacked_lengths, r, layer, input_pools)
                flush()
                request(stacked_points, pool_p, stacked_lengths, pool_b, 2 * r, layer, input_upsamples,
                        first_only=up_first_column_only, nn_hint=1.75 * dl)
            else:
                flush()
                input_pools.append(empty_i)
                pool_p = torch.zeros((0, 3), dtype=torch.float32, device=dev)
                pool_b = torch.zeros((0,), dtype=torch.int32, device=dev)
                input_upsamples.append(empty_i)
            input_points += [stacked_points]
            input_batches_len += [stacked_lengths]
            stacked_points = pool_p
            stacked_lengths = pool_b
            r_normal *= 2
            layer_blocks = []
        flush()

        overflow = False
        self.static_status = status_all[:len(pending)] if caps is not None else None
        self.level_lengths = input_batches_len
        if pending and caps is None:
            for kmax, flags in status_all[:len(pending)].tolist():
                if flags & _lib.ST_HIT_OVERFLOW and cap < _lib.NEIGHBOR_CAP:
                    overflow = True
                else:
                    ops._raise_flags(flags, 'tf_descriptor_input/neighbors')
        if overflow:
            self._neighbor_cap = _lib.NEIGHBOR_CAP
            return self.tf_descriptor_input(config, first_points, stacked_features, first_lengths, batch_inds,
                                            exact_shapes=exact_shapes, up_first_column_only=up_first_column_only)

        for l in range(len(input_pools) - 1):
            o = getattr(input_points[l + 1], 'order', None)
            if o is not None and input_pools[l].shape[0] > 0:
                input_pools[l].order = o

        if exact_shapes:
            stacked_batch_inds_0 = self.tf_stack_batch_inds(input_batches_len[0])
            stacked_batch_inds_1 = self.tf_stack_batch_inds(input_batches_len[-1])
        else:
            stacked_batch_inds_0 = ops.StackGroups(getattr(self, 'stack_group', 0))
            stacked_batch_inds_1 = None
        li = input_points + input_neighbors + input_pools + input_upsamples
        li += [stacked_features, stacked_weights, stacked_batch_inds_0, stacked_batch_inds_1]
        return li

    def _descriptor_input_internal(self, config, stacked_points, stacked_features, stacked_lengths, caps):
        dev = stacked_points.device
        lens_dev = ops.as_lens(stacked_lengths, dev)
        r_normal = config.first_subsampling_dl * config.KP_extent * 2.5
        status_all = getattr(self, "_status_all", None)
        if status_all is None or status_all.device != dev:
            status_all = self._status_all = torch.zeros((64, 2), dtype=torch.int32, device=dev)
        elif not torch.cuda.is_current_stream_capturing():
            status_all[:, 1].zero_()
        arch = config.architecture
        cap = getattr(self, '_neighbor_cap', 192)
        pending = []

        def status():
            st = status_all[len(pending)]
            pending.append(st)
            return st

        def search(grid, q, ql, qgrid, layer, first_only=False, nn_hint=0.0):
            lim = 1 if first_only else int(self.neighborhood_limits[layer])
            out, _ = grid.search(q, ql, lim, cap=cap, first_only=first_only, status=status(), reset_status=False, want_kmax=False,
                                 nn_hint=nn_hint, query_grid=qgrid, internal=True)
            return out
        empty_i = torch.zeros((0, 1), dtype=torch.int32, device=dev)
        points, lens_l, grids = [stacked_points], [lens_dev], []
        neighbors, pools, ups = [], [], []
        layer_blocks = []
        hints = getattr(self, 'hints', None)
        units = max(int(getattr(self, 'cap_units', 1)), 1)
        grids.append(ops.NeighborGrid(stacked_points, lens_dev, r_normal))
        for block_i, block in enumerate(arch):
            if 'global' in block or 'upsample' in block:
                break
            if 'deformable' in block:
                raise ValueError("internal numbering: deformable blocks are outside the inference path")
            if not ('pool' in block or 'strided' in block):
                layer_blocks += [block]
                if block_i < len(arch) - 1 and not ('upsample' in arch[block_i + 1]):
                    continue
            layer = len(neighbors)
            P, L, G = points[layer], lens_l[layer], grids[layer]
            pooled = 'pool' in block or 'strided' in block
            if pooled:
                dl = 2 * r_normal / (config.KP_extent * 2.5)
                pool_p, pool_b, _ = ops.batch_grid_subsample_async(P, L, dl, caps[layer + 1], status=status(),
                                                                   m_hint=hints[layer + 1] if hints else 0,
                                                                   elem_cap=-(-caps[layer + 1] // units),
                                                                   elem_points=-(-caps[layer] // units))
                Gn = ops.NeighborGrid(pool_p, pool_b, 2 * r_normal)
            neighbors.append(search(G, P, L, G, layer) if layer_blocks else empty_i)
            if pooled:
                pools.append(search(G, pool_p, pool_b, Gn, layer))
                ups.append(search(Gn, P, L, G, layer, first_only=True, nn_hint=1.75 * dl))
                points.append(pool_p)
                lens_l.append(pool_b)
                grids.append(Gn)
            else:
                pools.append(empty_i)
                ups.append(empty_i)
            r_normal *= 2
            layer_blocks = []
        self.static_status = status_all[:len(pending)]
        self.level_lengths = lens_l
        self.orders = [g.order for g in grids]
        self.level_points = points
        self._grids = grids
        li = [g.xyz for g in grids] + neighbors + pools + ups
        li += [stacked_features, None, ops.StackGroups(getattr(self, 'stack_group', 0)), None]
        return li

    def calibrate_neighbors(self, config, keep_ratio=0.8, samples_threshold=10000, verbose=False):
        split = 'train' if len(getattr(self, 'anc_points', {}).get('train', [])) > 0 else 'test'
        gen_function, _, _ = self.get_batch_gen(split, config)
        map_func = self.get_tf_mapping(config)
        hist_n = int(np.ceil(4 / 3 * np.pi * (config.density_parameter + 1) ** 3))
        neighb_hists = np.zeros((config.num_layers, hist_n), dtype=np.int64)
        for sample in gen_function():
            if np.min(np.sum(neighb_hists, axis=1)) >= samples_threshold:
                break
            flat = map_func(*self._to_device(sample))
            neighbors = flat[config.num_layers:2 * config.num_layers]
            for l, mat in enumerate(neighbors):
                neighb_hists[l] += self.neighbor_histogram(mat, hist_n)
        cumsum = np.cumsum(neighb_hists.T, axis=0)
        percentiles = np.sum(cumsum < (keep_ratio * cumsum[hist_n - 1, :]), axis=0)
        self.neighborhood_limits = percentiles.astype(np.int32)
        if verbose:
            print('neighborhood_limits', self.neighborhood_limits)
        return neighb_hists

    @staticmethod
    def neighbor_histogram(neighb_mat, hist_n):
        mat = neighb_mat.cpu().numpy()
        counts = np.sum(mat < mat.shape[0], axis=1)
        return np.bincount(counts, minlength=hist_n)[:hist_n].astype(np.int64)

    def _to_device(self, sample):
        pts, anc_k, pos_k, obj, lens, ids, backup = sample
        return (torch.from_numpy(np.ascontiguousarray(pts, dtype=np.float32)).to(self.device), anc_k, pos_k, obj,
                torch.from_numpy(np.ascontiguousarray(lens, dtype=np.int32)).to(self.device), ids,
                torch.from_numpy(np.ascontiguousarray(backup, dtype=np.float32)).to(self.device))

    def init_test_input_pipeline(self, config):
        config.num_classes = self.num_classes - len(self.ignored_labels)
        config.network_model = self.network_model
        hist_n = int(np.ceil(4 / 3 * np.pi * (config.density_parameter + 1) ** 3))
        self.neighborhood_limits = np.full(config.num_layers, hist_n, dtype=np.int32)
        self.calibrate_neighbors(config)
        print("self.neighborhood:", self.neighborhood_limits)
        gen_function, _, _ = self.get_batch_gen('test', config)
        map_func = self.get_tf_mapping(config)
        dataset = self

        class _Repeat:
            def __init__(self):
                self.it = None

            def reset(self):
                self.it = iter(gen_function())

            def __iter__(self):
                return self

            def __next__(self):
                if self.it is None:
                    self.reset()
                try:
                    sample = next(self.it)
                except StopIteration:
                    self.reset()
                    sample = next(self.it)
                return map_func(*dataset._to_device(sample))
# ... 42 lines not shown
```

d3feat_amd/engine.py:

```python
import warnings

import numpy as np
import torch

from . import _lib, keypoints as kpts, ops
from . import tf_custom_ops as tfo
from .datasets.common import FragmentDataset
from .models.KPFCNN_model import KernelPointFCNN


def level_caps(n0_cap, num_layers, ratio=0.4, clouds=2):
    caps = [clouds * int(n0_cap)]
    for _ in range(1, num_layers):
        caps.append(max(int(np.ceil(caps[-1] * ratio)), 256))
    return caps


def level_hints(n0_hint, num_layers, ratio=0.26, clouds=2):
    h = [clouds * int(n0_hint)]
    for _ in range(1, num_layers):
        h.append(max(int(h[-1] * ratio), 64))
    return h


class _Slot:
    pass


class FragmentEngine:
    def __init__(self, config, weights, neighborhood_limits, raw_cap=320000, n0_cap=40000, level_ratio=0.4, slots=2,
                 device=None, seed=42, n0_hint=None, mirror_self_pair=False, streams=None, two_clouds=False, batch=1,
                 bf16=False, bf16_features=False, stage0=True, internal_order=None, keypoints=None):
        if device is None:
            device = torch.device("cuda", torch.cuda.current_device())
        self.cfg, self.device = config, device
        self.limits = np.asarray(neighborhood_limits, np.int32)
        self.raw_cap, self.n0_cap = int(raw_cap), int(n0_cap)
        self.mirror = bool(mirror_self_pair)
        self.two = bool(two_clouds)
        if internal_order is None:
            import os
            internal_order = os.environ.get("D3F_INTERNAL_ORDER", "1") != "0" and \
                not any("deformable" in b for b in config.architecture)
        self.internal = bool(internal_order)
        self.stage0 = bool(stage0)
        if keypoints is not None and not 1 <= int(keypoints) <= _lib.TOPK_MAX:
            raise ValueError("keypoints = %s outside 1..%d" % (keypoints, _lib.TOPK_MAX))
        self.keypoints = int(keypoints) if keypoints is not None else None
        if not self.stage0:
            if self.mirror:
                raise ValueError("stage0=False is implemented for stacked self-pairs and for pairs of two clouds")
            self.raw_cap = self.n0_cap
        self.F = int(batch)
        self.bf16 = bool(bf16) or bool(bf16_features)
        self.bf16_features = bool(bf16_features)
        if self.two and self.mirror:
            raise ValueError("mirror_self_pair and two_clouds exclude each other")
        if self.F < 1 or 2 * self.F * (2 if self.two else 1) > _lib.MAX_BATCH:
            raise ValueError("batch out of range")
        self.nin = self.F * (2 if self.two else 1)
        self.keep_clouds = 2 if self.two else 1
        clouds = self.F * (1 if (self.mirror or self.two) else 2)
        self.level_ratio = float(level_ratio)
        self.caps = level_caps(n0_cap, config.num_layers, level_ratio, clouds)
        self.cap_units = clouds
        self.n0_hint = int(n0_hint if n0_hint is not None else n0_cap / 1.3)
        self.hints = level_hints(self.n0_hint, config.num_layers, clouds=clouds)
        self.model = KernelPointFCNN(None, config, weights=weights, seed=seed, device=device)
        self._eager_ds = FragmentDataset([], fast=True)
        self._eager_ds.device = device
        self._eager_ds.neighborhood_limits = self.limits
        self._eager_map = self._eager_ds.get_tf_mapping(config)
        g = torch.Generator(device="cpu").manual_seed(1)
        self._dummy = (torch.rand((256, 3), generator=g) * (6.0 * config.first_subsampling_dl)).to(device)
        self.neighbor_cap = 192
        if any("deformable" in b for b in config.architecture):
            self.neighbor_cap = self._eager_ds._neighbor_cap = _lib.NEIGHBOR_CAP
        self.slots = [self._build_slot(streams[i] if streams else None) for i in range(int(slots))]
        self.fallbacks = 0
        self.isolated = 0
        self.fragments = 0
        self._hit_overflows = 0
        self._warned = False

    def refresh_weights(self, values):
        assert not any(sl.busy for sl in self.slots), "refresh_weights with replays in flight"
        torch.cuda.synchronize(self.device)
        touched = self.model.variables.update_in_place(values)
        n = ops.refresh_packed_weights(touched)
        torch.cuda.synchronize(self.device)
        return n

    def _sequence(self, sl):
        cfg = self.cfg
        if self.stage0:
            sub, sub_l, st0 = ops.batch_grid_subsample_async(None, sl.raw_len, cfg.first_subsampling_dl, self.F * self.n0_cap,
                                                             status=sl.status0, m_hint=self.F * self.n0_hint,
                                                             elem_cap=self.n0_cap, clouds=sl.raw_ptrs, n_cap=self.F * self.raw_cap)
        else:
            sub, sub_l = sl.raw, sl.raw_len
            sub.n_hint = self.F * self.n0_hint
            if self.two:
                torch.sum(sub_l, 0, keepdim=True, dtype=torch.int32, out=sl.raw_total)
                sub.n_dev = sl.raw_total
        if self.mirror or self.two:
            pts, lens = sub, sub_l
        else:
            pts, lens = ops.stack_self_pair(sub, sub_l)
        flat = sl.map(pts, None, None, None, lens, ("a", "a"), pts)
        with ops.bf16_contraction(self.bf16, features=self.bf16_features):
            desc, score = self.model.run(flat)
        sl.flat, sl.level_lengths = flat, sl.ds.level_lengths
        row_map = None
        if self.internal:
            row_map = sl.ds.orders[0]
            ipts = flat[0]
            ipts.n_dev = pts.n_dev
            sl.orders = sl.ds.orders
        per = 1 if self.mirror else 2
        sl.packed = ops.pack_descriptors(flat[0] if self.internal else pts, desc, score, lens=lens, group=per, keep=self.keep_clouds,
                                         dst=sl.dst_ptrs, row_map=row_map)
        if self.keypoints:
            kpts.topk(flat[0] if self.internal else pts, desc, score, self.keypoints, lens=lens, group=per, keep=self.keep_clouds,
                      row_map=row_map, out=sl.kp, count=sl.kp_count, n_cap=self.n0_cap)
        if self.internal:
            desc, score = sl.packed[:, 3:3 + desc.shape[1]], sl.packed[:, 3 + desc.shape[1]:]
        return pts, desc, score, sl.ds.static_status, lens

    def _build_slot(self, stream=None):
        dev = self.device
        sl = _Slot()
        sl.stream = stream if stream is not None else torch.cuda.Stream(device=dev)
        sl.raw = torch.zeros((self.F * self.raw_cap, 3), dtype=torch.float32, device=dev)
        nw = 2 * self.nin + 2 * self.F
        sl.meta_dev = torch.zeros((nw + self.nin,), dtype=torch.int32, device=dev)
        sl.meta_host = torch.zeros((nw + self.nin,), dtype=torch.int32).pin_memory()
        sl.raw_ptrs = sl.meta_dev[: 2 * self.nin].view(torch.int64)
        sl.dst_ptrs = sl.meta_dev[2 * self.nin: nw].view(torch.int64)
        sl.raw_len = sl.meta_dev[nw:]
        sl.host_ptrs = sl.meta_host[: 2 * self.nin].view(torch.int64)
        sl.host_dst = sl.meta_host[2 * self.nin: nw].view(torch.int64)
        sl.host_n = sl.meta_host[nw:]
        sl.status0 = torch.zeros((2,), dtype=torch.int32, device=dev)
        sl.raw_total = torch.zeros((1,), dtype=torch.int32, device=dev)
        if self.keypoints:
            sl.kp = torch.zeros((self.F * self.keep_clouds, self.keypoints, 36), dtype=torch.float32, device=dev)
            sl.kp_count = torch.zeros((self.F * self.keep_clouds,), dtype=torch.int32, device=dev)
        sl.ds = FragmentDataset([], fast=True)
        sl.ds.device = dev
        sl.ds.neighborhood_limits = self.limits
        sl.ds.caps = self.caps
        sl.ds.hints = self.hints
        sl.ds.cap_units = self.cap_units
        sl.ds.stack_group = 1 if self.mirror else 2
        sl.ds.internal_order = self.internal
        sl.ds._neighbor_cap = self.neighbor_cap
        sl.cap = self.neighbor_cap
        sl.map = sl.ds.get_tf_mapping(self.cfg)
        sl.busy = False
        sl.raw_src = None
        with torch.cuda.stream(sl.stream):
            g = torch.Generator(device="cpu").manual_seed(0)
            per = min(2048, self.raw_cap)
            warm = (torch.rand((per * self.nin, 3), generator=g) * torch.tensor([1.0, 1.0, 0.05])).to(dev)
            sl.raw[: per * self.nin].copy_(warm)
            sl.raw_len.fill_(per)
            sl.raw_ptrs.copy_(torch.tensor([sl.raw.data_ptr() + 12 * per * i for i in range(self.nin)], dtype=torch.int64))
            with ops.private_workspace():
                _, _, _, w_status, w_lens = self._sequence(sl)
            w_status[:, 1].zero_()
        sl.stream.synchronize()
        sl.nl = w_lens.numel()
        sl.nstat = 1 + 2 + 2 * w_status.shape[0]
        sl.host_stat = torch.zeros((sl.nstat + sl.nl,), dtype=torch.int32).pin_memory()
        sl.dev_stat = torch.zeros((sl.nstat + sl.nl,), dtype=torch.int32, device=dev)
        sl.graph = torch.cuda.CUDAGraph()
        with ops.private_workspace() as pw:
            with torch.cuda.graph(sl.graph, stream=sl.stream):
                sl.pts, sl.desc, sl.score, sl.status, sl.lens = self._sequence(sl)
                ops.pack_status(sl.dev_stat, [sl.pts.n_dev, sl.status0, sl.status, sl.lens], clear=sl.status)
        sl.keep = pw.kept
        assert sl.lens.numel() == sl.nl and 1 + 2 + 2 * sl.status.shape[0] == sl.nstat
        sl.done = torch.cuda.Event()
        return sl

    def kept_rows_cap(self):
        return self.n0_cap * min(self.keep_clouds, self.F)

    def submit(self, slot, raw, out=None):
        sl = self.slots[slot]
        assert not sl.busy, "slot %d still holds an unfetched fragment" % slot
        single = not isinstance(raw, list)
        frags = [raw] if single else list(raw)
        if not 1 <= len(frags) <= self.F:
            raise ValueError("submit: %d fragments for a batch-%d engine" % (len(frags), self.F))
        outs = None
        if out is not None and not self.mirror:
            outs = [out] if (single and isinstance(out, torch.Tensor)) else list(out)
            assert len(outs) == len(frags) and all(o.is_cuda and o.dtype == torch.float32 and o.is_contiguous() and o.dim() == 2
                                                   and o.shape[1] == 36 for o in outs)
            need = self.kept_rows_cap()
            short = [int(o.shape[0]) for o in outs if int(o.shape[0]) < need]
            if short:
                raise ValueError("submit: a destination of %d rows, but a fragment of this engine can keep up to %d rows "
                                 "(n0_cap %d)" % (min(short), need, self.n0_cap))
        if sl.cap != self.neighbor_cap:
            sl = self.slots[slot] = self._build_slot(sl.stream)
        sl.single, sl.raw_src, sl.nfrag = single, frags, len(frags)
        sl.busy = True
        sl.out_dst = outs
        sl.out_given = outs is not None
        parts = []
        for fr in frags:
            p = list(fr) if self.two else [fr]
            if self.two and len(p) != 2:
                raise ValueError("two_clouds engine: a fragment is a pair (raw_a, raw_b)")
            parts += p
        per_frag = 2 if self.two else 1
        sizes = [sum(int(x.shape[0]) for x in parts[i * per_frag:(i + 1) * per_frag]) for i in range(len(frags))]
        if max(sizes) > self.raw_cap or min(int(x.shape[0]) for x in parts) == 0:
            sl.oversize = True
            return
        sl.oversize = False
        parts += [self._dummy] * (self.nin - len(parts))
        for i, p in enumerate(parts):
            sl.host_n[i] = int(p.shape[0])
        cur = torch.cuda.current_stream(self.device)
        with torch.cuda.stream(sl.stream):
            sl.stream.wait_stream(cur)
            o = 0
            sl.keep_in = []
            for i, p in enumerate(parts):
                n = int(p.shape[0])
                if isinstance(p, ops.RawRecords):
                    p.decode(self.device, out=sl.raw[o:o + n])
                    addr = sl.raw[o:].data_ptr()
                elif self.stage0 and isinstance(p, torch.Tensor) and p.is_cuda and p.device == self.device:
                    q = p if (p.dtype == torch.float32 and p.is_contiguous()) else p.to(torch.float32).contiguous()
# ... 169 lines not shown
```

d3feat_amd/ops.py:

```python
import ctypes

import os

import numpy as np
import torch

from . import _lib

_WS = {}

PROFILE = None


class _timed:
    def __init__(self, name, info, device):
        self.on = PROFILE is not None
        self.name, self.info, self.device = name, info, device

    def __enter__(self):
        if self.on:
            self.start = torch.cuda.Event(enable_timing=True)
            self.end = torch.cuda.Event(enable_timing=True)
            self.start.record(torch.cuda.current_stream(self.device))
        return self
# ... 76 lines not shown
        raise ValueError("%s has overlapping rows" % name)
    return t, int(max(ld, 1))


def as_lens(lens, device):
    if isinstance(lens, torch.Tensor):
        out = lens.to(device=device, dtype=torch.int32).contiguous()
        if out is not lens and hasattr(lens, "host_lens"):
            out.host_lens = lens.host_lens
        return out
    host = np.asarray(lens, dtype=np.int32).reshape(-1)
    out = torch.as_tensor(host, device=device)
    out.host_lens = [int(x) for x in host]
    return out


def host_lens(lens):
    if isinstance(lens, torch.Tensor):
        h = getattr(lens, "host_lens", None)
        return list(h) if h is not None else [int(x) for x in lens.tolist()]
    return [int(x) for x in np.asarray(lens).reshape(-1)]


def _raise_flags(flags, what):
    if flags:
        msgs = []
        if flags & _lib.ST_EMPTY_ELEMENT:
            msgs.append("a batch element is empty")
        if flags & _lib.ST_NEG_CELL:
            msgs.append("negative voxel index (origin above a point after fp32 rounding)")
        if flags & _lib.ST_KEY_RANGE:
            msgs.append("voxel key exceeds 2^56")
        if flags & _lib.ST_HIT_OVERFLOW:
            msgs.append("a query has more than %d in-radius supports" % _lib.NEIGHBOR_CAP)
        if flags & _lib.ST_OUT_OVERFLOW:
            msgs.append("more output rows than the capacity of the output buffer")
        if flags & _lib.ST_KEY_WIDTH:
            msgs.append("(element, voxel key) wider than the 32-bit sort key of the capacity-mode subsampling")
        raise _lib.D3FeatLibraryError("d3feat_amd.%s: %s" % (what, "; ".join(msgs)))
    return 0


def check_status(status, what):
    st = status.tolist()
    _raise_flags(st[1], what)
    return st[0]


def batch_grid_subsample(points, lens, dl, features=None, classes=None):
    lib = _lib.load()
    points = _req(points, torch.float32, "points", 2).contiguous()
    dev = points.device
    N = points.shape[0]
    lens_t = as_lens(lens, dev)
    B = lens_t.numel()
    fdim = ldim = 0
    if features is not None:
        features = _req(features, torch.float32, "features", 2).contiguous()
        fdim = features.shape[1]
    if classes is not None:
        classes = _req(classes, torch.int32, "classes", 2).contiguous()
        ldim = classes.shape[1]
    sub_p = torch.empty((max(N, 1), 3), dtype=torch.float32, device=dev)
    sub_f = torch.empty((max(N, 1), fdim), dtype=torch.float32, device=dev) if fdim else None
    sub_c = torch.empty((max(N, 1), ldim), dtype=torch.int32, device=dev) if ldim else None
    sub_l = torch.empty((B,), dtype=torch.int32, device=dev)
    status = (ctypes.c_int * (B + 2))()
    nbytes = lib.d3f_grid_subsample_workspace_bytes(N, B, fdim, ldim)
    ws = workspace(nbytes, dev)
    with _timed("grid_subsample", dict(N=N, M=None), dev) as tm:
        rc = lib.d3f_batch_grid_subsample(points.data_ptr(), N, lens_t.data_ptr(), B, float(dl),
                                          features.data_ptr() if fdim else None, fdim,
                                          classes.data_ptr() if ldim else None, ldim,
                                          sub_p.data_ptr(), sub_f.data_ptr() if fdim else None,
                                          sub_c.data_ptr() if ldim else None, sub_l.data_ptr(),
                                          ctypes.addressof(status), ws.data_ptr(), ws.numel(), _stream(dev))
        tm.info["M"] = int(status[0])
    _lib.check(rc, "batch_grid_subsample")
    M = _raise_flags(status[1], "batch_grid_subsample") or status[0]
    sub_l.host_lens = [int(status[2 + b]) for b in range(B)]
    return sub_p[:M], sub_l, (sub_f[:M] if fdim else None), (sub_c[:M] if ldim else None)


def batch_grid_subsample_async(points, lens, dl, m_cap, status=None, m_hint=0, elem_cap=0, elem_points=0, clouds=None, n_cap=0):
    lib = _lib.load()
    if clouds is not None:
        assert points is None and clouds.dtype == torch.int64 and clouds.is_contiguous() and int(n_cap) > 0
        dev, N = clouds.device, int(n_cap)
    else:
        points = _req(points, torch.float32, "points", 2).contiguous()
        dev = points.device
        N = points.shape[0]
    lens_t = as_lens(lens, dev)
    B = lens_t.numel()
    sub_p = torch.empty((int(m_cap), 3), dtype=torch.float32, device=dev)
    sub_l = torch.empty((B,), dtype=torch.int32, device=dev)
    if status is None:
        status = torch.empty((2,), dtype=torch.int32, device=dev)
    nbytes = lib.d3f_grid_subsample_workspace_bytes(N, B, 0, 0)
    ws = workspace(nbytes, dev)
    with _timed("grid_subsample", dict(N=N, M=int(m_cap)), dev):
        if clouds is not None:
            assert clouds.numel() == B
            rc = lib.d3f_batch_grid_subsample_async_inplace(clouds.data_ptr(), N, lens_t.data_ptr(), B, float(dl), sub_p.data_ptr(),
                                                            int(m_cap), int(elem_cap), sub_l.data_ptr(), status.data_ptr(),
                                                            ws.data_ptr(), ws.numel(), _stream(dev))
        else:
            rc = lib.d3f_batch_grid_subsample_async(points.data_ptr(), N, lens_t.data_ptr(), B, float(dl), sub_p.data_ptr(),
                                                    int(m_cap), int(elem_cap), int(elem_points), sub_l.data_ptr(), status.data_ptr(),
                                                    ws.data_ptr(), ws.numel(), _stream(dev))
    _lib.check(rc, "batch_grid_subsample_async")
    sub_p.n_dev = status[0:1]
    sub_p.n_hint = int(m_hint)
    return sub_p, sub_l, status


def pack_status(dst, blocks, clear=None):
    lib = _lib.load()
    assert 1 <= len(blocks) <= 4 and all(b.dtype == torch.int32 and b.is_contiguous() for b in blocks) and dst.dtype == torch.int32
    assert dst.is_contiguous()
    blocks = [b.view(-1) for b in blocks]
    assert dst.numel() >= sum(b.numel() for b in blocks)
    args = []
    for i in range(4):
        args += [blocks[i].data_ptr(), blocks[i].numel()] if i < len(blocks) else [None, 0]
    if clear is not None:
        assert clear.dtype == torch.int32 and clear.is_contiguous() and clear.dim() == 2 and clear.shape[1] == 2
    _lib.check(lib.d3f_pack_status(dst.data_ptr(), *args, _ptr(clear),
                                   clear.shape[0] if clear is not None else 0, 1, 2, _stream(dst.device)), "pack_status")
    return dst


def stack_self_pair(pts, lens=None):
    lib = _lib.load()
    pts = _req(pts, torch.float32, "pts", 2).contiguous()
    dev = pts.device
    cap = pts.shape[0]
    if lens is None:
        lens = getattr(pts, "n_dev", None)
        if lens is None:
            lens = torch.full((1,), cap, dtype=torch.int32, device=dev)
    B = lens.numel()
    out = torch.empty((2 * cap, 3), dtype=torch.float32, device=dev)
    lens_out = torch.empty((2 * B,), dtype=torch.int32, device=dev)
    total = torch.empty((1,), dtype=torch.int32, device=dev)
    rc = lib.d3f_stack_self_pair(pts.data_ptr(), cap, lens.data_ptr(), B, out.data_ptr(), lens_out.data_ptr(),
                                 total.data_ptr(), _stream(dev))
    _lib.check(rc, "stack_self_pair")
    out.n_dev = total
    out.n_hint = 2 * int(getattr(pts, "n_hint", 0) or 0)
    return out, lens_out


class NeighborGrid:

    def __init__(self, supports, s_lens, radius):
        lib = _lib.load()
        self.supports = _tag(_req(supports, torch.float32, "supports", 2).contiguous(), supports)
        dev = self.supports.device
        self.Ns = self.supports.shape[0]
        self.s_lens = as_lens(s_lens, dev)
        self.B = self.s_lens.numel()
        self.radius = float(radius)
        self.nbytes = lib.d3f_neighbor_grid_bytes(self.Ns, self.B)
        self.mem = torch.empty((self.nbytes,), dtype=torch.uint8, device=dev)
        with _timed("nb_grid_build", dict(Ns=self.Ns), dev):
            rc = lib.d3f_neighbor_grid_build(self.supports.data_ptr(), self.Ns, self.s_lens.data_ptr(), self.B, self.radius,
                                             self.mem.data_ptr(), self.nbytes, _stream(dev))
        _lib.check(rc, "neighbor_grid_build")
        off = lib.d3f_neighbor_grid_order_offset(self.Ns, self.B)
        self.order = self.mem[off: off + 4 * max(self.Ns, 1)].view(torch.int32)
        off = lib.d3f_neighbor_grid_inv_offset(self.Ns, self.B)
        self.inv = self.mem[off: off + 4 * max(self.Ns, 1)].view(torch.int32)
        off = lib.d3f_neighbor_grid_xyz_offset(self.Ns, self.B)
        self.xyz = self.mem[off: off + 12 * max(self.Ns, 1)].view(torch.float32).view(-1, 3)
        for a in ("n_dev", "n_hint"):
            if getattr(self.supports, a, None) is not None:
                setattr(self.xyz, a, getattr(self.supports, a))

    def search(self, queries, q_lens, width, ld=None, pad_value=None, cap=192, first_only=False, out=None, status=None,
               reset_status=True, want_kmax=True, nn_hint=0.0, query_grid=None, internal=False):
        lib = _lib.load()
        queries = _req(queries, torch.float32, "queries", 2).contiguous()
        dev = queries.device
        Nq = queries.shape[0]
        ql = as_lens(q_lens, dev)
        if ql.numel() != self.B:
            raise ValueError("q_batches and s_batches must have the same number of elements")
        ld = int(ld if ld is not None else width)
        if out is None:
            out = torch.empty((Nq, ld), dtype=torch.int32, device=dev)
        if status is None:
            status = torch.empty((2,), dtype=torch.int32, device=dev)
        same = 1 if (queries.data_ptr() == self.supports.data_ptr() and Nq == self.Ns) else 0
        if pad_value is None:
            pad_value = _lib.PAD_NUM_SUPPORTS if getattr(self.supports, "n_dev", None) is not None else self.Ns
        if query_grid is not None:
            if query_grid.Ns != Nq or query_grid.B != self.B or query_grid.supports.data_ptr() != queries.data_ptr():
                raise ValueError("query_grid was not built over these queries")
            with _timed("nb_search", dict(Nq=Nq, Ns=self.Ns, width=int(width), first_only=int(bool(first_only))), dev):
                rc = lib.d3f_neighbor_grid_search_ordered(self.mem.data_ptr(), self.nbytes, self.Ns, queries.data_ptr(), Nq, ql.data_ptr(),
                                                          self.B, self.radius, query_grid.mem.data_ptr(), query_grid.nbytes,
                                                          out.data_ptr(), ld, int(width), int(pad_value), int(cap),
                                                          1 if first_only else 0, float(nn_hint),
                                                          (1 if reset_status else 0) | (0 if want_kmax else 2) | (4 if internal else 0),
                                                          status.data_ptr(), _stream(dev))
            _lib.check(rc, "neighbor_grid_search_ordered")
            o = getattr(queries, "order", None)
            if o is not None and not internal:
                out.order = o
            return _tag(out, queries), status
        if internal:
            raise ValueError("internal numbering needs the queries' grid")
        with _timed("nb_search", dict(Nq=Nq, Ns=self.Ns, width=int(width), first_only=int(bool(first_only))), dev):
            rc = lib.d3f_neighbor_grid_search(self.mem.data_ptr(), self.nbytes, self.Ns, queries.data_ptr(), Nq,
                                              ql.data_ptr(), self.B, self.radius, same, out.data_ptr(), ld, int(width),
                                              int(pad_value), int(cap),
                                              1 if first_only else 0, float(nn_hint),
                                              (1 if reset_status else 0) | (0 if want_kmax else 2),
                                              status.data_ptr(),
                                              _stream(dev))
        _lib.check(rc, "neighbor_grid_search")
        o = getattr(queries, "order", None)
        if o is not None:
            out.order = o
        return _tag(out, queries), status


def batch_radius_neighbors(queries, supports, q_lens, s_lens, radius, width, ld=None, out=None, pad_value=None, cap=192,
                           first_only=False):
    grid = NeighborGrid(supports, s_lens, radius)
    return grid.search(queries, q_lens, width, ld=ld, pad_value=pad_value, cap=cap, first_only=first_only, out=out)


class StackGroups:

    def __init__(self, group=0):
        self.group = int(group)


_KP_HOST = {}


def _kp_host(K_points):
    if isinstance(K_points, torch.Tensor):
        key = (K_points.data_ptr(), K_points._version, tuple(K_points.shape))
        hit = _KP_HOST.get(key)
        if hit is None:
            if len(_KP_HOST) > 256:
                _KP_HOST.clear()
            hit = _KP_HOST[key] = (K_points, np.ascontiguousarray(K_points.detach().cpu().numpy(), dtype=np.float32))
        return hit[1]
# ... 667 lines not shown
```

include/d3feat_amd.h:

```cpp
#ifndef D3FEAT_AMD_H
#define D3FEAT_AMD_H

#include <stddef.h>
#include <stdint.h>

#ifdef __cplusplus
extern "C" {
#endif

#define D3F_OK 0
#define D3F_ERR_HIP (-1)
#define D3F_ERR_WORKSPACE (-2)
#define D3F_ERR_ARG (-3)

#define D3F_ST_EMPTY_ELEMENT 1
#define D3F_ST_NEG_CELL 2
#define D3F_ST_KEY_RANGE 4
#define D3F_ST_HIT_OVERFLOW 8
#define D3F_ST_OUT_OVERFLOW 16
#define D3F_ST_KEY_WIDTH 32

#define D3F_NB_NO_KMAX 2
#define D3F_PAD_NUM_SUPPORTS (-2147483647 - 1)

#define D3F_MAX_BATCH 255
#define D3F_NEIGHBOR_CAP 1024
#define D3F_TOPK_MAX 8192
#define D3F_PAIRS_KMAX 1024
#define D3F_REPEAT_COUNTS_MAX 16
#define D3F_SCENES_MAX 256
#define D3F_MATCH_KMAX 8192
#define D3F_VALIDATION_NMAX 1024
#define D3F_NUM_KP_MAX 16

int d3f_version(void);

int d3f_trace_marker(int id, void* stream);
int d3f_pack_status(int* dst, const int* a, int na, const int* b, int nb, const int* c, int nc, const int* d, int nd,
                    int* clear, int nclear, int clear_first, int clear_step, void* stream);


size_t d3f_grid_subsample_workspace_bytes(int N, int B, int fdim, int ldim);
int d3f_batch_grid_subsample_async(const float* points, int N_cap, const int* lens_dev, int B, float dl,
                                   float* sub_points, int M_cap, int elem_cap, int elem_points_cap, int* sub_lens_dev,
                                   int* status_dev, void* workspace, size_t workspace_bytes, void* stream);
int d3f_batch_grid_subsample_async_inplace(const float* const* clouds_dev, int N_cap, const int* lens_dev, int B, float dl,
                                           float* sub_points, int M_cap, int elem_cap, int* sub_lens_dev, int* status_dev,
                                           void* workspace, size_t workspace_bytes, void* stream);

int d3f_stack_self_pair(const float* pts, int M_cap, const int* lens_in_dev, int B, float* out, int* lens_out_dev,
                        int* total_dev, void* stream);
int d3f_batch_grid_subsample(const float* points, int N, const int* lens_dev, int B, float dl,
                             const float* features, int fdim, const int* classes, int ldim,
                             float* sub_points, float* sub_features, int* sub_classes, int* sub_lens_dev,
                             int* status_host, void* workspace, size_t workspace_bytes, void* stream);

size_t d3f_radius_neighbors_workspace_bytes(int Nq, int Ns, int B);
int d3f_batch_radius_neighbors(const float* queries, int Nq, const float* supports, int Ns,
                               const int* q_lens_dev, const int* s_lens_dev, int B, float radius,
                               int* out, int ld, int width, int pad_value, int* status_dev,
                               void* workspace, size_t workspace_bytes, void* stream);

size_t d3f_neighbor_grid_bytes(int Ns, int B);
size_t d3f_neighbor_grid_order_offset(int Ns, int B);
int d3f_neighbor_grid_build(const float* supports, int Ns, const int* s_lens_dev, int B, float radius,
                            void* grid, size_t grid_bytes, void* stream);
int d3f_neighbor_grid_search(const void* grid, size_t grid_bytes, int Ns, const float* queries, int Nq,
                             const int* q_lens_dev, int B, float radius, int queries_are_supports,
                             int* out, int ld, int width, int pad_value, int cap, int first_only, float nn_hint,
                             int reset_status, int* status_dev, void* stream);
#define D3F_NB_INTERNAL 4
int d3f_neighbor_grid_search_ordered(const void* grid, size_t grid_bytes, int Ns, const float* queries, int Nq,
                                     const int* q_lens_dev, int B, float radius, const void* query_grid, size_t query_grid_bytes,
                                     int* out, int ld, int width, int pad_value, int cap, int first_only, float nn_hint, int flags,
                                     int* status_dev, void* stream);
size_t d3f_neighbor_grid_inv_offset(int Ns, int B);
size_t d3f_neighbor_grid_xyz_offset(int Ns, int B);



int d3f_row_positive(const void* f, int Ns, int ldf, int Cin, unsigned char* row_pos, const int* Ns_dev, int feat_bf16,
                     void* stream);
int d3f_kpconv_aggregate(const float* q, int Nq, const float* s, int Ns, const int* idx, int ld_idx, int K,
                         const void* f, int ldf, int Cin, const unsigned char* row_pos, const float* kp_host,
                         int num_kp, float KP_extent, int influence, int aggregation, float* wf, float* inv_cnt,
                         const int* Nq_dev, const int* Ns_dev, const int* q_order, int feat_bf16, void* stream);

int d3f_kpconv_deform_aggregate(const float* q, int Nq, const float* s, int Ns, const int* idx, int ld_idx, int K,
                                const void* f, int ldf, int Cin, const float* offsets, int ld_off, float offset_scale,
                                const float* modulations, int ld_mod, int mod_logits, const float* kp_host, int num_kp,
                                float KP_extent, int influence, int aggregation, float* wf, const int* Nq_dev, const int* Ns_dev,
                                const int* q_order, int feat_bf16, void* stream);

int d3f_kpconv_fused_c1(const float* q, int Nq, const float* s, int Ns, const int* idx, int ld_idx, int K,
                        const float* f, int ldf, const float* kp_host, int num_kp, float KP_extent, int influence,
                        int aggregation, const float* W, int Cout, const float* col_scale, const float* col_shift,
                        const float* residual, int ldr, int leaky, float alpha, void* out, int ldo,
                        const int* Nq_dev, const int* Ns_dev, const int* q_order, int out_bf16, void* stream);

int d3f_kpconv_fused32(const float* q, int Nq, const float* s, int Ns, const int* idx, int ld_idx, int K,
                       const void* f, int ldf, const unsigned char* row_pos, const float* kp_host, int num_kp,
                       float KP_extent, int influence, int aggregation, const float* W, const float* col_scale,
                       const float* col_shift, const float* residual, int ldr, int leaky, float alpha, void* out, int ldo,
                       const int* Nq_dev, const int* Ns_dev, const int* q_order, int feat_bf16, void* stream);

int d3f_kpconv_fused_supported(int Cin, int Cout, int num_kp, int influence, int aggregation);
int d3f_kpconv_pack_weights(const float* W, int K, int N, float* W_packed, void* stream);
size_t d3f_kpconv_packed_x3_bytes(int K, int N);
int d3f_kpconv_pack_weights_x3(const float* W, int K, int N, void* W_planes, void* stream);
int d3f_kpconv_fused32_x3(const float* q, int Nq, const float* s, int Ns, const int* idx, int ld_idx, int K,
                          const void* f, int ldf, const unsigned char* rowpos, const float* kp_host, int num_kp,
                          float KP_extent, int influence, int aggregation, const float* W_planes, const float* col_scale,
                          const float* col_shift, const float* residual, int ldr, int leaky, float alpha, void* out,
                          int ldo, const int* Nq_dev, const int* Ns_dev, const int* q_order, int feat_bf16, void* stream);
int d3f_kpconv_fused_x3(const float* q, int Nq, const float* s, int Ns, const int* idx, int ld_idx, int K,
                        const void* f, int ldf, int Cin, const unsigned char* rowpos, const float* kp_host, int num_kp,
                        float KP_extent, int influence, int aggregation, const float* W_planes, int Cout,
                        const float* col_scale, const float* col_shift, const float* residual, int ldr, int leaky,
                        float alpha, void* out, int ldo, const int* Nq_dev, const int* Ns_dev, const int* q_order,
                        int feat_bf16, void* stream);
int d3f_kpconv_fused(const float* q, int Nq, const float* s, int Ns, const int* idx, int ld_idx, int K,
                     const void* f, int ldf, int Cin, const unsigned char* rowpos, const float* kp_host, int num_kp,
                     float KP_extent, int influence, int aggregation, const float* W_packed, int Cout,
                     const float* col_scale, const float* col_shift, const float* residual, int ldr, int leaky,
                     float alpha, void* out, int ldo, const int* Nq_dev, const int* Ns_dev, const int* q_order,
                     int feat_bf16, void* stream);

size_t d3f_gemm_workspace_bytes(int M, int N, int K, int M_hint);
int d3f_gemm_f32(const float* A, int lda, const float* B, int ldb, float* C, int ldc, int M, int N, int K,
                 const float* row_scale, const float* col_scale, const float* col_shift,
                 const float* residual, int ldr, int leaky, float alpha,
                 void* workspace, size_t workspace_bytes, const int* M_dev, int M_hint, void* stream);

int d3f_gemm_upsample_cat_f32(const float* x, int N1, int ldx, int C1, const int* idx, int ld_idx,
                              const float* skip, int lds, int C2, const float* W, int ldb, float* C, int ldc,
                              int M, int N, const float* col_scale, const float* col_shift, int leaky, float alpha,
                              void* workspace, size_t workspace_bytes, const int* M_dev, const int* N1_dev,
                              int M_hint, void* stream);

int d3f_ind_max_pool(const void* x, int N1, int ldx, int C, const int* idx, int N2, int ld_idx, int K,
                     void* out, int ldo, float* col_min_dev, const int* N1_dev, const int* N2_dev, const int* row_order,
                     int feat_bf16, void* stream);
int d3f_closest_pool_cat(const float* x, int N1, int ldx, int C1, const int* idx, int N2, int ld_idx,
                         const float* skip, int lds, int C2, float* out, int ldo, const int* N1_dev, const int* N2_dev,
                         void* stream);

int d3f_affine_act(const float* x, int ldx, int M, int N, const float* col_scale, const float* col_shift,
                   const float* residual, int ldr, int leaky, float alpha, float* out, int ldo, const int* M_dev,
                   void* stream);
// ... 124 lines not shown
```

Baseline: 1921 fragments/s.

## Carry per-cloud bounding boxes through subsample/stack into neighbor grid builds

Grid subsampling now computes per-cloud bounding boxes as a by-product of its emit stage, and the self-pair stack duplicates them. The neighbor-grid build consumes these precomputed boxes instead of running its own bbox reduction pass. A single geometry-reset launch clears all box buffers and grids for a pyramid chain of preallocated grids. The goal is to remove the separate bbox kernels and fill/begin launches at each level, at the cost of more plumbing and a larger emit block size.

```diff
diff --git a/d3feat_amd/_lib.py b/d3feat_amd/_lib.py
--- a/d3feat_amd/_lib.py
+++ b/d3feat_amd/_lib.py
@@ -16,6 +16,7 @@
 MATCH_KMAX = 8192
 VALIDATION_NMAX = 1024
 SCENES_MAX = 256
+GRID_RESET_MAX = 8
 VP_INDEX_RANGE, VP_COUNT_RANGE = 1, 2
 
 _vp, _sz, _i, _f = C.c_void_p, C.c_size_t, C.c_int, C.c_float
@@ -34,6 +35,11 @@
     "d3f_neighbor_grid_bytes": (_sz, [_i, _i]),
     "d3f_neighbor_grid_order_offset": (_sz, [_i, _i]),
     "d3f_neighbor_grid_build": (_i, [_vp, _i, _vp, _i, _f, _vp, _sz, _vp]),
+    "d3f_neighbor_grid_boxed_form": (_i, [_i, _i]),
+    "d3f_geometry_reset": (_i, [_vp, _i, _vp, _vp, _vp, _vp, _i, _vp]),
+    "d3f_neighbor_grid_build_boxed": (_i, [_vp, _i, _vp, _i, _f, _vp, _vp, _sz, _vp]),
+    "d3f_stack_self_pair_boxed": (_i, [_vp, _i, _vp, _i, _vp, _vp, _vp, _vp, _vp, _vp]),
+    "d3f_batch_grid_subsample_async_boxed": (_i, [_vp, _vp, _i, _vp, _i, _f, _vp, _i, _i, _i, _vp, _vp, _vp, _vp, _vp, _sz, _vp]),
     "d3f_neighbor_grid_search": (_i, [_vp, _sz, _i, _vp, _i, _vp, _i, _f, _i, _vp, _i, _i, _i, _i, _i, _f, _i, _vp, _vp]),
     "d3f_neighbor_grid_search_ordered": (_i, [_vp, _sz, _i, _vp, _i, _vp, _i, _f, _vp, _sz, _vp, _i, _i, _i, _i, _i, _f, _i, _vp, _vp]),
     "d3f_neighbor_grid_inv_offset": (_sz, [_i, _i]),
diff --git a/d3feat_amd/csrc/grid_subsample.hip b/d3feat_amd/csrc/grid_subsample.hip
--- a/d3feat_amd/csrc/grid_subsample.hip
+++ b/d3feat_amd/csrc/grid_subsample.hip
@@ -101,6 +101,25 @@
     const unsigned* bbox; const int* offs; int B; float dl; GsElem* el; int* status; RsMeta* smeta; int n_cap;
     __device__ __forceinline__ void operator()() const { gs_prep(bbox, offs, B, dl, el, status, smeta, n_cap); }
 };
+
+__global__ void __launch_bounds__(256) gs_begin_boxed_kernel(const int* __restrict__ lens, int B, int* __restrict__ offs,
+                                                             const unsigned* __restrict__ bbox, unsigned* __restrict__ counters,
+                                                             int ncounters, D3fFill f0, D3fFill fmeta, float dl, GsElem* __restrict__ el,
+                                                             int* __restrict__ status, RsMeta* __restrict__ smeta, int n_cap) {
+    const size_t tid = (size_t)blockIdx.x * blockDim.x + threadIdx.x, stride = (size_t)gridDim.x * blockDim.x;
+    d3f_fill_words(f0, tid, stride);
+    if (blockIdx.x != 0) return;
+    if (threadIdx.x == 0) {
+        int s = 0;
+        for (int b = 0; b < B; ++b) { offs[b] = s; s += lens[b]; }
+        offs[B] = s;
+    }
+    for (int i = threadIdx.x; i < ncounters; i += blockDim.x) counters[i] = 0u;
+    for (int i = threadIdx.x; i < (int)fmeta.n; i += blockDim.x) fmeta.p[i] = fmeta.v;
+    asm volatile("s_waitcnt vmcnt(0)" ::: "memory");
+    __syncthreads();
+    gs_prep(bbox, offs, B, dl, el, status, smeta, n_cap);
+}
 
 __global__ void __launch_bounds__(256) gs_insert_kernel(const float* __restrict__ pts, int N, const int* __restrict__ offs,
                                                         int B, float dl, const GsElem* __restrict__ el,
@@ -610,21 +629,28 @@
     bary[3 * (size_t)v + 1] = __fmul_rn(ay, sc);
     bary[3 * (size_t)v + 2] = __fmul_rn(az, sc);
 }
-__global__ void __launch_bounds__(256) gs_emit_kernel(int* __restrict__ status, const int* __restrict__ moffs, int B,
+template <bool BOX>
+__global__ void __launch_bounds__(BOX ? 1024 : 256) gs_emit_kernel(int* __restrict__ status, const int* __restrict__ moffs, int B,
                                                       const int* __restrict__ vpos, const float* __restrict__ bary,
-                                                      float* __restrict__ out_p, int out_cap) {
+                                                      float* __restrict__ out_p, int out_cap, unsigned* __restrict__ bbox_out) {
     const int v = blockIdx.x * blockDim.x + threadIdx.x;
-    if (v >= status[0]) return;
-    if (status[1] & (D3F_ST_OUT_OVERFLOW | D3F_ST_KEY_WIDTH)) return;
-    const int b = d3f_find_elem(moffs, B, v);
-    const size_t dest = (size_t)moffs[b] + (size_t)vpos[v];
-    if (dest >= (size_t)out_cap) {
-        atomicOr(&status[1], D3F_ST_OUT_OVERFLOW);
-        return;
-    }
-    out_p[3 * dest + 0] = bary[3 * (size_t)v + 0];
-    out_p[3 * dest + 1] = bary[3 * (size_t)v + 1];
-    out_p[3 * dest + 2] = bary[3 * (size_t)v + 2];
+    bool ok = v < status[0] && !(status[1] & (D3F_ST_OUT_OVERFLOW | D3F_ST_KEY_WIDTH));
+    int b = -1;
+    float x = 0.f, y = 0.f, z = 0.f;
+    if (ok) {
+        b = d3f_find_elem(moffs, B, v);
+        const size_t dest = (size_t)moffs[b] + (size_t)vpos[v];
+        if (dest >= (size_t)out_cap) {
+            atomicOr(&status[1], D3F_ST_OUT_OVERFLOW);
+            ok = false;
+        } else {
+            x = bary[3 * (size_t)v + 0]; y = bary[3 * (size_t)v + 1]; z = bary[3 * (size_t)v + 2];
+            out_p[3 * dest + 0] = x;
+            out_p[3 * dest + 1] = y;
+            out_p[3 * dest + 2] = z;
+        }
+    }
+    if constexpr (BOX) d3f_box_accum_block(bbox_out, ok ? b : -1, x, y, z);
 }
 
 
@@ -727,7 +753,8 @@
     return D3F_OK;
 }
 static int gs_run_small(const float* points, int N, const int* lens_dev, int B, float dl, float* sub_points, int M_cap, int elem_cap,
-                        int pc, int* sub_lens_dev, int* status_dev, void* workspace, size_t workspace_bytes, hipStream_t stream) {
+                        int pc, int* sub_lens_dev, int* status_dev, void* workspace, size_t workspace_bytes, hipStream_t stream,
+                        unsigned* bbox_out = nullptr) {
     if (elem_cap <= 0 || elem_cap > M_cap) elem_cap = M_cap;
     if (elem_cap > pc) elem_cap = pc;
     D3fArena ar(workspace, workspace_bytes);
@@ -737,6 +764,7 @@
     A.mcount = ar.take<int>(B);
     A.cflags = ar.take<int>(B);
     if (!ar.ok) return D3F_ERR_WORKSPACE;
+    A.bbox_out = bbox_out;
     A.pts = points; A.lens = lens_dev; A.B = B; A.dl = dl; A.elem_cap = elem_cap; A.pc = pc; A.out_cap = M_cap;
     A.nbmax = GSS_NB_MAX;
     for (int j = 0; j < D3F_NCHAIN; ++j)
@@ -753,14 +781,15 @@
 static int gs_run(const float* points, int N, const int* lens_dev, int B, float dl, const float* features, int fdim,
                   const int* classes, int ldim, float* sub_points, int M_cap, int elem_cap, int elem_points, float* sub_features,
                   int* sub_classes, int* sub_lens_dev, int* status_host, int* status_dev, void* workspace,
-                  size_t workspace_bytes, hipStream_t stream, const float* const* ptrs = nullptr) {
+                  size_t workspace_bytes, hipStream_t stream, const float* const* ptrs = nullptr, const unsigned* bbox_in = nullptr,
+                  unsigned* bbox_out = nullptr) {
     const bool async = status_dev != nullptr;
     if (async && !features && ldim == 0 && !ptrs) {
         const int pc = (elem_points > 0 && elem_points < N) ? elem_points : N;
         int ec = (elem_cap > 0 && elem_cap < M_cap) ? elem_cap : M_cap;
         if (ec > pc) ec = pc;
         if (pc <= 16384 && ec <= GSS_NB_MAX) return gs_run_small(points, N, lens_dev, B, dl, sub_points, M_cap, elem_cap, pc, sub_lens_dev, status_dev,
-                                             workspace, workspace_bytes, stream);
+                                             workspace, workspace_bytes, stream, bbox_out);
     }
     GsLayout L = gs_layout(N, B, async ? M_cap : -1);
     D3fArena ar(workspace, workspace_bytes);
@@ -815,12 +844,22 @@
     const D3fFill none{nullptr, 0ull, 0u};
     const unsigned long long ones_words = (unsigned long long)((char*)(vhead + n) - (char*)tkey) / 4ull;
     const unsigned long long zero_words = (unsigned long long)((char*)(vcnt + n) - (char*)meta) / 4ull;
+    if (bbox_in && use_sort) {
+        const unsigned long long words = (unsigned long long)(n / 32 + 2);
+        long long blocks = (long long)(words / 4 / 256) + 1;
+        if (blocks > 1024) blocks = 1024;
+        gs_begin_boxed_kernel<<<(int)blocks, 256, 0, stream>>>(lens_dev, B, offs, bbox_in, counters, ncounters, D3fFill{fbits, words, 0u},
+                                                               D3fFill{(unsigned*)meta, (unsigned long long)(B + 2), 0u}, dl, el, meta,
+                                                               smeta, N);
+        D3F_LAUNCH_CHECK();
+    } else {
     if ((rc = use_sort ? d3f_begin_launch(lens_dev, B, offs, bbox, counters, ncounters, D3fFill{fbits, (unsigned long long)(n / 32 + 2), 0u},
                                           D3fFill{(unsigned*)meta, (unsigned long long)(B + 2), 0u}, none, none, stream)
                        : d3f_begin_launch(lens_dev, B, offs, bbox, counters, ncounters, D3fFill{(unsigned*)tkey, ones_words, 0xFFFFFFFFu},
                                           D3fFill{(unsigned*)meta, zero_words, 0u}, none, none, stream)) != D3F_OK) return rc;
     GsPrepEpi prep{bbox, offs, B, dl, el, meta, use_sort ? smeta : nullptr, N};
     if ((rc = d3f_bbox_launch_t(points, offs, B, N, bbox, counters, prep, stream, ptrs)) != D3F_OK) return rc;
+    }
     const int nblk = d3f_cdiv(N, 256);
     const int elem_lim = async ? elem_cap : 0x7fffffff;
     int M, maxM;
@@ -878,7 +917,8 @@
         gs_order_place_kernel<<<gp, 256, 0, stream>>>(A, j);
     }
     if (use_sort)
-        gs_emit_kernel<<<d3f_cdiv(M, 256), 256, 0, stream>>>(meta, moffs, B, A.vpos, bary, sub_points, M_cap);
+        if (bbox_out) gs_emit_kernel<true><<<d3f_cdiv(M, 1024), 1024, 0, stream>>>(meta, moffs, B, A.vpos, bary, sub_points, M_cap, bbox_out);
+        else gs_emit_kernel<false><<<d3f_cdiv(M, 256), 256, 0, stream>>>(meta, moffs, B, A.vpos, bary, sub_points, M_cap, nullptr);
     else
         gs_accum_kernel<<<d3f_cdiv(async ? N : M, 256), 256, 0, stream>>>(points, features, fdim, meta, moffs, B, vstart, sbase,
                                                                          vcnt, sorted, A.vpos, sub_points, sub_features, M_cap);
@@ -926,10 +966,25 @@
                   nullptr, status_dev, workspace, workspace_bytes, stream, clouds_dev);
 }
 
+extern "C" int d3f_batch_grid_subsample_async_boxed(const float* points, const float* const* clouds_dev, int N_cap, const int* lens_dev,
+                                                    int B, float dl, float* sub_points, int M_cap, int elem_cap, int elem_points_cap,
+                                                    int* sub_lens_dev, int* status_dev, const unsigned* bbox_in_dev,
+                                                    unsigned* bbox_out_dev, void* workspace, size_t workspace_bytes, void* stream_) {
+    hipStream_t stream = (hipStream_t)stream_;
+    if (N_cap < 1 || N_cap > (1 << 30) || M_cap < 1 || elem_cap < 0 || elem_points_cap < 0 || B < 1 || B > D3F_MAX_BATCH || !(dl > 0.f))
+        return D3F_ERR_ARG;
+    if ((!points && !clouds_dev) || (points && clouds_dev) || !lens_dev || !sub_points || !sub_lens_dev || !status_dev) return D3F_ERR_ARG;
+    return gs_run(points, N_cap, lens_dev, B, dl, nullptr, 0, nullptr, 0, sub_points, M_cap, elem_cap, clouds_dev ? 0 : elem_points_cap,
+                  nullptr, nullptr, sub_lens_dev, nullptr, status_dev, workspace, workspace_bytes, stream, clouds_dev, bbox_in_dev,
+                  bbox_out_dev);
+}
+
 __global__ void __launch_bounds__(256) gs_stack_pair_kernel(const float* __restrict__ pts, int M_cap, const int* __restrict__ lens_in,
                                                             int B, float* __restrict__ out, int* __restrict__ lens_out,
-                                                            int* __restrict__ total) {
+                                                            int* __restrict__ total, const unsigned* __restrict__ bbox_in,
+                                                            unsigned* __restrict__ bbox_out) {
     const int i = blockIdx.x * blockDim.x + threadIdx.x;
+    if (bbox_out && i < 12 * B) bbox_out[i] = bbox_in[(i / 12) * 6 + i % 6];
     int tot = 0;
     for (int b = 0; b < B; ++b) tot += lens_in[b];
     tot = min(tot, M_cap);
@@ -958,12 +1013,18 @@
     out[3 * (row + m) + c] = v;
 }
 
+extern "C" int d3f_stack_self_pair_boxed(const float* pts, int M_cap, const int* lens_in_dev, int B, float* out, int* lens_out_dev,
+                                         int* total_dev, const unsigned* bbox_in_dev, unsigned* bbox_out_dev, void* stream_) {
+    hipStream_t stream = (hipStream_t)stream_;
+    if (M_cap < 1 || B < 1 || 2 * B > D3F_MAX_BATCH || !pts || !lens_in_dev || !out || !lens_out_dev || !total_dev ||
+        (bbox_out_dev && !bbox_in_dev))
+        return D3F_ERR_ARG;
+    gs_stack_pair_kernel<<<d3f_cdiv(3ll * M_cap, 256), 256, 0, stream>>>(pts, M_cap, lens_in_dev, B, out, lens_out_dev, total_dev,
+                                                                         bbox_in_dev, bbox_out_dev);
+    D3F_LAUNCH_CHECK();
+    return D3F_OK;
+}
 extern "C" int d3f_stack_self_pair(const float* pts, int M_cap, const int* lens_in_dev, int B, float* out, int* lens_out_dev,
                                    int* total_dev, void* stream_) {
-    hipStream_t stream = (hipStream_t)stream_;
-    if (M_cap < 1 || B < 1 || 2 * B > D3F_MAX_BATCH || !pts || !lens_in_dev || !out || !lens_out_dev || !total_dev)
-        return D3F_ERR_ARG;
-    gs_stack_pair_kernel<<<d3f_cdiv(3ll * M_cap, 256), 256, 0, stream>>>(pts, M_cap, lens_in_dev, B, out, lens_out_dev, total_dev);
-    D3F_LAUNCH_CHECK();
-    return D3F_OK;
-}
+    return d3f_stack_self_pair_boxed(pts, M_cap, lens_in_dev, B, out, lens_out_dev, total_dev, nullptr, nullptr, stream_);
+}
diff --git a/d3feat_amd/csrc/gs_small.h b/d3feat_amd/csrc/gs_small.h
--- a/d3feat_amd/csrc/gs_small.h
+++ b/d3feat_amd/csrc/gs_small.h
@@ -15,6 +15,7 @@
     int nbmax;
     int* mcount;
     int* cflags;
+    unsigned* bbox_out;
 };
 
 template <int T>
@@ -310,14 +311,39 @@
         lo_r = hi;
     }
     float* __restrict__ out = A.stage + 3 * (size_t)b * (size_t)A.elem_cap;
+    unsigned bmn[3] = {0xFFFFFFFFu, 0xFFFFFFFFu, 0xFFFFFFFFu}, bmx[3] = {0u, 0u, 0u};
     for (int v = tid; v < M; v += T) {
         const float4 q = rec[v];
         const size_t d = (size_t)La[v];
         out[3 * d + 0] = q.x;
         out[3 * d + 1] = q.y;
         out[3 * d + 2] = q.z;
+        const unsigned ux = d3f_f2ord(q.x), uy = d3f_f2ord(q.y), uz = d3f_f2ord(q.z);
+        bmn[0] = min(bmn[0], ux); bmn[1] = min(bmn[1], uy); bmn[2] = min(bmn[2], uz);
+        bmx[0] = max(bmx[0], ux); bmx[1] = max(bmx[1], uy); bmx[2] = max(bmx[2], uz);
     }
     if (tid == 0) { A.mcount[b] = M; A.cflags[b] = *sFlag; }
+    if (A.bbox_out) {
+#pragma unroll
+        for (int d = 0; d < 3; ++d) {
+#pragma unroll
+            for (int o = 32; o > 0; o >>= 1) {
+                bmn[d] = min(bmn[d], (unsigned)__shfl_xor((int)bmn[d], o, 64));
+                bmx[d] = max(bmx[d], (unsigned)__shfl_xor((int)bmx[d], o, 64));
+            }
+        }
+        __syncthreads();
+        if (lane == 0) {
+#pragma unroll
+            for (int d = 0; d < 3; ++d) { sScr[w * 6 + d] = (int)bmn[d]; sScr[w * 6 + 3 + d] = (int)bmx[d]; }
+        }
+        __syncthreads();
+        if (tid < 6) {
+            unsigned r = (unsigned)sScr[tid];
+            for (int k = 1; k < W; ++k) r = tid < 3 ? min(r, (unsigned)sScr[k * 6 + tid]) : max(r, (unsigned)sScr[k * 6 + tid]);
+            A.bbox_out[b * 6 + tid] = r;
+        }
+    }
 }
 
 __global__ void __launch_bounds__(256) gs_small_pack_kernel(GsSmallArgs A, float* __restrict__ out, int* __restrict__ sub_lens,
diff --git a/d3feat_amd/csrc/prims.h b/d3feat_amd/csrc/prims.h
--- a/d3feat_amd/csrc/prims.h
+++ b/d3feat_amd/csrc/prims.h
@@ -22,6 +22,16 @@
     }
     __syncthreads();
     return last_flag != 0;
+}
+
+__device__ __forceinline__ void d3f_fill_words(const D3fFill& f, size_t tid, size_t stride) {
+    unsigned* p = f.p;
+    const size_t n = (size_t)f.n;
+    if (n == 0) return;
+    const size_t n4 = (((uintptr_t)p & 15) == 0) ? n / 4 : 0;
+    const uint4 v4 = make_uint4(f.v, f.v, f.v, f.v);
+    for (size_t j = tid; j < n4; j += stride) ((uint4*)p)[j] = v4;
+    for (size_t j = n4 * 4 + tid; j < n; j += stride) p[j] = f.v;
 }
 
 static __global__ void __launch_bounds__(256) begin_kernel(const int* __restrict__ lens, int B, int* __restrict__ offs,
@@ -38,17 +48,10 @@
             for (int i = threadIdx.x; i < B * 6; i += blockDim.x) bbox[i] = ((i % 6) < 3) ? 0xFFFFFFFFu : 0u;
         for (int i = threadIdx.x; i < ncounters; i += blockDim.x) counters[i] = 0u;
     }
-    const D3fFill f[4] = {f0, f1, f2, f3};
-#pragma unroll
-    for (int k = 0; k < 4; ++k) {
-        unsigned* p = f[k].p;
-        const size_t n = (size_t)f[k].n;
-        if (n == 0) continue;
-        const size_t n4 = (((uintptr_t)p & 15) == 0) ? n / 4 : 0;
-        const uint4 v4 = make_uint4(f[k].v, f[k].v, f[k].v, f[k].v);
-        for (size_t j = tid; j < n4; j += stride) ((uint4*)p)[j] = v4;
-        for (size_t j = n4 * 4 + tid; j < n; j += stride) p[j] = f[k].v;
-    }
+    d3f_fill_words(f0, tid, stride);
+    d3f_fill_words(f1, tid, stride);
+    d3f_fill_words(f2, tid, stride);
+    d3f_fill_words(f3, tid, stride);
 }
 
 static inline int d3f_begin_launch(const int* lens, int B, int* offs, unsigned* bbox, unsigned* counters, int ncounters,
@@ -123,6 +126,81 @@
     return D3F_OK;
 }
 
+__device__ __forceinline__ void d3f_box_flush(unsigned* __restrict__ bbox, int b, int slot, unsigned v) {
+    unsigned* p = &bbox[b * 6 + slot];
+    const unsigned old = __hip_atomic_load(p, __ATOMIC_RELAXED, __HIP_MEMORY_SCOPE_AGENT);
+    if (slot < 3) { if (v < old) atomicMin(p, v); }
+    else if (v > old) atomicMax(p, v);
+}
+__device__ __forceinline__ void d3f_box_accum_block(unsigned* __restrict__ bbox, int b, float x, float y, float z) {
+    __shared__ unsigned sBox[16][6];
+    __shared__ int sElem[16];
+    const int lane = threadIdx.x & 63, w = threadIdx.x >> 6, nw = blockDim.x >> 6;
+    unsigned v[6] = {d3f_f2ord(x), d3f_f2ord(y), d3f_f2ord(z), 0u, 0u, 0u};
+#pragma unroll
+    for (int d = 0; d < 3; ++d) {
+        v[3 + d] = b < 0 ? 0u : v[d];
+        v[d] = b < 0 ? 0xFFFFFFFFu : v[d];
+    }
+    const unsigned long long live = __ballot(b >= 0);
+    int bw = -1;
+    if (live) {
+        bw = __shfl(b, __ffsll((long long)live) - 1, 64);
+        if (__ballot(b >= 0 && b != bw)) {
+            unsigned long long rem = live;
+            while (rem) {
+                const int bs = __shfl(b, __ffsll((long long)rem) - 1, 64);
+                const bool mine = b == bs;
+                unsigned r[6], sel = 0u;
+#pragma unroll
+                for (int t = 0; t < 6; ++t) {
+                    r[t] = mine ? v[t] : (t < 3 ? 0xFFFFFFFFu : 0u);
+#pragma unroll
+                    for (int o = 32; o > 0; o >>= 1) {
+                        const unsigned q = (unsigned)__shfl_xor((int)r[t], o, 64);
+                        r[t] = t < 3 ? min(r[t], q) : max(r[t], q);
+                    }
+                    sel = lane == t ? r[t] : sel;
+                }
+                if (lane < 6) d3f_box_flush(bbox, bs, lane, sel);
+                rem &= ~__ballot(mine);
+            }
+            bw = -1;
+        } else {
+#pragma unroll
+            for (int d = 0; d < 3; ++d) {
+#pragma unroll
+                for (int o = 32; o > 0; o >>= 1) {
+                    v[d] = min(v[d], (unsigned)__shfl_xor((int)v[d], o, 64));
+                    v[3 + d] = max(v[3 + d], (unsigned)__shfl_xor((int)v[3 + d], o, 64));
+                }
+            }
+        }
+    }
+    if (lane == 0) {
+        sElem[w] = bw;
+#pragma unroll
+        for (int t = 0; t < 6; ++t) sBox[w][t] = v[t];
+    }
+    __syncthreads();
+    if (threadIdx.x < 6) {
+        const int t = threadIdx.x;
+        int cur = -1;
+        unsigned acc = 0u;
+        for (int k = 0; k <= nw; ++k) {
+            const int bk = k < nw ? sElem[k] : -2;
+            if (bk == -1) continue;
+            if (bk != cur) {
+                if (cur >= 0) d3f_box_flush(bbox, cur, t, acc);
+                cur = bk;
+                acc = k < nw ? sBox[k][t] : 0u;
+            } else {
+                acc = t < 3 ? min(acc, sBox[k][t]) : max(acc, sBox[k][t]);
+            }
+        }
+    }
+}
+
 __device__ __forceinline__ int d3f_block_excl_scan_256(int v, int* lds4, int* total) {
     const int lane = threadIdx.x & 63, w = threadIdx.x >> 6;
     int x = v;
diff --git a/d3feat_amd/csrc/radius_neighbors.hip b/d3feat_amd/csrc/radius_neighbors.hip
--- a/d3feat_amd/csrc/radius_neighbors.hip
+++ b/d3feat_amd/csrc/radius_neighbors.hip
@@ -10,6 +10,40 @@
 
 #define NB_WAVES_PER_BLOCK 4
 #define NB_EL_LDS 40
+
+__device__ __forceinline__ void nb_elem_geometry(const unsigned* __restrict__ bbox, int b, int len, float radius, long long per,
+                                                 NbElem& e) {
+    if (len <= 0) {
+        e.mn[0] = e.mn[1] = e.mn[2] = 0.0;
+        e.inv_h = 1.0;
+        e.dims[0] = e.dims[1] = e.dims[2] = 1;
+    } else {
+        double mx[3];
+        for (int d = 0; d < 3; ++d) {
+            e.mn[d] = (double)d3f_ord2f(__hip_atomic_load(&bbox[b * 6 + d], __ATOMIC_RELAXED, __HIP_MEMORY_SCOPE_AGENT));
+            mx[d] = (double)d3f_ord2f(__hip_atomic_load(&bbox[b * 6 + 3 + d], __ATOMIC_RELAXED, __HIP_MEMORY_SCOPE_AGENT));
+        }
+        double h = (double)radius * (1.0 + 1.0 / 1048576.0);
+        if (!(h > 0.0)) h = 1.0;
+        bool fits = false;
+        for (int it = 0; it < 64; ++it) {
+            e.inv_h = 1.0 / h;
+            double tot = 1.0;
+            for (int d = 0; d < 3; ++d) {
+                double n = floor((mx[d] - e.mn[d]) * e.inv_h) + 1.0;
+                e.dims[d] = (n < 1073741824.0) ? (int)n : 1073741824;
+                tot *= n;
+            }
+            if (tot <= (double)per) { fits = true; break; }
+            h *= 2.0;
+        }
+        if (!fits) {
+            e.mn[0] = e.mn[1] = e.mn[2] = 0.0;
+            e.inv_h = 0.0;
+            e.dims[0] = e.dims[1] = e.dims[2] = 1;
+        }
+    }
+}
 
 __device__ __forceinline__ void nb_prep(const unsigned* __restrict__ bbox, const int* __restrict__ soffs, int B, float radius,
                                         long long cell_budget, NbElem* __restrict__ el, int* __restrict__ ncells_total) {
@@ -18,37 +52,7 @@
     const long long per = cell_budget / B;
     for (int b = 0; b < B; ++b) {
         NbElem e;
-        const int len = soffs[b + 1] - soffs[b];
-        if (len <= 0) {
-            e.mn[0] = e.mn[1] = e.mn[2] = 0.0;
-            e.inv_h = 1.0;
-            e.dims[0] = e.dims[1] = e.dims[2] = 1;
-        } else {
-            double mx[3];
-            for (int d = 0; d < 3; ++d) {
-                e.mn[d] = (double)d3f_ord2f(__hip_atomic_load(&bbox[b * 6 + d], __ATOMIC_RELAXED, __HIP_MEMORY_SCOPE_AGENT));
-                mx[d] = (double)d3f_ord2f(__hip_atomic_load(&bbox[b * 6 + 3 + d], __ATOMIC_RELAXED, __HIP_MEMORY_SCOPE_AGENT));
-            }
-            double h = (double)radius * (1.0 + 1.0 / 1048576.0);
-            if (!(h > 0.0)) h = 1.0;
-            bool fits = false;
-            for (int it = 0; it < 64; ++it) {
-                e.inv_h = 1.0 / h;
-                double tot = 1.0;
-                for (int d = 0; d < 3; ++d) {
-                    double n = floor((mx[d] - e.mn[d]) * e.inv_h) + 1.0;
-                    e.dims[d] = (n < 1073741824.0) ? (int)n : 1073741824;
-                    tot *= n;
-                }
-                if (tot <= (double)per) { fits = true; break; }
-                h *= 2.0;
-            }
-            if (!fits) {
-                e.mn[0] = e.mn[1] = e.mn[2] = 0.0;
-                e.inv_h = 0.0;
-                e.dims[0] = e.dims[1] = e.dims[2] = 1;
-            }
-        }
+        nb_elem_geometry(bbox, b, soffs[b + 1] - soffs[b], radius, per, e);
         e.cbase = (int)base;
         base += (long long)e.dims[0] * e.dims[1] * e.dims[2];
         el[b] = e;
@@ -100,6 +104,146 @@
     order[pos] = i;
     inv[i] = pos;
     xyz[3 * (size_t)pos] = x; xyz[3 * (size_t)pos + 1] = y; xyz[3 * (size_t)pos + 2] = z;
+}
+
+#define NBX_SMALL_T 512
+#define NBX_LDS_CELLS 8192
+#define NBX_COUNT_PTS 1024
+
+struct NbxGeom {
+    int offs[D3F_MAX_BATCH + 1];
+    NbElem el[D3F_MAX_BATCH];
+    int ncells;
+};
+__device__ __forceinline__ void nbx_geometry(NbxGeom& G, const int* __restrict__ lens, const unsigned* __restrict__ bbox, int B, float radius,
+                                             long long per) {
+    if (threadIdx.x == 0) {
+        int s = 0;
+        for (int b = 0; b < B; ++b) { G.offs[b] = s; s += lens[b]; }
+        G.offs[B] = s;
+    }
+    __syncthreads();
+    for (int b = threadIdx.x; b < B; b += blockDim.x) {
+        NbElem e;
+        nb_elem_geometry(bbox, b, G.offs[b + 1] - G.offs[b], radius, per, e);
+        e.cbase = 0;
+        G.el[b] = e;
+    }
+    __syncthreads();
+    if (threadIdx.x == 0) {
+        long long base = 0;
+        for (int b = 0; b < B; ++b) {
+            G.el[b].cbase = (int)base;
+            base += (long long)G.el[b].dims[0] * G.el[b].dims[1] * G.el[b].dims[2];
+        }
+        G.ncells = (int)base;
+    }
+    __syncthreads();
+}
+__device__ __forceinline__ void nbx_publish(const NbxGeom& G, int B, int* __restrict__ soffs, NbElem* __restrict__ el, int* __restrict__ ncells) {
+    for (int b = threadIdx.x; b <= B; b += blockDim.x) soffs[b] = G.offs[b];
+    for (int b = threadIdx.x; b < B; b += blockDim.x) el[b] = G.el[b];
+    if (threadIdx.x == 0) { ncells[0] = G.ncells; ncells[1] = G.ncells + 1; }
+}
+__device__ __forceinline__ int nbx_local_cell(const NbElem& e, float x, float y, float z) {
+    int cx, cy, cz;
+    nb_cell_of(e, x, y, z, cx, cy, cz);
+    cx = min(max(cx, 0), e.dims[0] - 1);
+    cy = min(max(cy, 0), e.dims[1] - 1);
+    cz = min(max(cz, 0), e.dims[2] - 1);
+    return cx + e.dims[0] * (cy + e.dims[1] * cz);
+}
+
+__global__ void __launch_bounds__(256) nbx_count_kernel(const float* __restrict__ s, int Ns, const int* __restrict__ lens, int B,
+                                                        const unsigned* __restrict__ bbox, float radius, long long per,
+                                                        int* __restrict__ soffs, NbElem* __restrict__ el, int* __restrict__ ncells,
+                                                        int* __restrict__ cell_of, int* __restrict__ cell_cnt, int* __restrict__ rank) {
+    __shared__ NbxGeom G;
+    nbx_geometry(G, lens, bbox, B, radius, per);
+    if (blockIdx.x == 0) nbx_publish(G, B, soffs, el, ncells);
+    const int n = min(Ns, G.offs[B]);
+#pragma unroll
+    for (int u = 0; u < NBX_COUNT_PTS / 256; ++u) {
+        const int i = blockIdx.x * NBX_COUNT_PTS + u * 256 + threadIdx.x;
+        if (i >= n) continue;
+        const int b = d3f_find_elem(G.offs, B, i);
+        const int c = G.el[b].cbase + nbx_local_cell(G.el[b], s[3 * (size_t)i], s[3 * (size_t)i + 1], s[3 * (size_t)i + 2]);
+        cell_of[i] = c;
+        rank[i] = atomicAdd(&cell_cnt[c], 1);
+    }
+}
+
+__global__ void __launch_bounds__(256) nbx_scatter_kernel(const float* __restrict__ s, int Ns, const int* __restrict__ ns_dev,
+                                                          const int* __restrict__ cell_of, const int* __restrict__ cell_start,
+                                                          const int* __restrict__ cell_base, float4* __restrict__ sorted,
+                                                          int* __restrict__ order, int* __restrict__ inv, float* __restrict__ xyz) {
+    const int i = blockIdx.x * blockDim.x + threadIdx.x;
+    if (i >= min(Ns, *ns_dev)) return;
+    const int pos = d3f_scan_at(cell_start, cell_base, cell_of[i]) + inv[i];
+    const float x = s[3 * (size_t)i], y = s[3 * (size_t)i + 1], z = s[3 * (size_t)i + 2];
+    sorted[pos] = make_float4(x, y, z, __int_as_float(i));
+    order[pos] = i;
+    inv[i] = pos;
+    xyz[3 * (size_t)pos] = x; xyz[3 * (size_t)pos + 1] = y; xyz[3 * (size_t)pos + 2] = z;
+}
+
+__global__ void __launch_bounds__(NBX_SMALL_T) nbx_small_kernel(const float* __restrict__ s, int Ns, const int* __restrict__ lens, int B,
+                                                                const unsigned* __restrict__ bbox, float radius, long long per,
+                                                                int* __restrict__ soffs, NbElem* __restrict__ el, int* __restrict__ ncells,
+                                                                int* __restrict__ cell_of, int* __restrict__ cell_start,
+                                                                int* __restrict__ cell_base, float4* __restrict__ sorted,
+                                                                int* __restrict__ order, int* __restrict__ inv, float* __restrict__ xyz) {
+    __shared__ NbxGeom G;
+    __shared__ int sCnt[NBX_LDS_CELLS];
+    __shared__ int sW[NBX_SMALL_T / 64];
+    const int b = blockIdx.x, tid = threadIdx.x;
+    nbx_geometry(G, lens, bbox, B, radius, per);
+    if (b == 0) nbx_publish(G, B, soffs, el, ncells);
+    const NbElem e = G.el[b];
+    const int nc = e.dims[0] * e.dims[1] * e.dims[2];
+    const int n = min(Ns, G.offs[B]);
+    const int lo = min(G.offs[b], n), hi = min(G.offs[b + 1], n);
+    for (int j = tid; j < nc; j += NBX_SMALL_T) sCnt[j] = 0;
+    __syncthreads();
+    for (int i = lo + tid; i < hi; i += NBX_SMALL_T) {
+        const int c = nbx_local_cell(e, s[3 * (size_t)i], s[3 * (size_t)i + 1], s[3 * (size_t)i + 2]);
+        cell_of[i] = e.cbase + c;
+        inv[i] = atomicAdd(&sCnt[c], 1);
+    }
+    __syncthreads();
+    const int per_t = (nc + NBX_SMALL_T - 1) / NBX_SMALL_T;
+    const int j0 = min(tid * per_t, nc), j1 = min(j0 + per_t, nc);
+    int sum = 0;
+    for (int j = j0; j < j1; ++j) sum += sCnt[j];
+    int x = sum;
+    const int lane = tid & 63, w = tid >> 6;
+#pragma unroll
+    for (int d = 1; d < 64; d <<= 1) {
+        const int y = __shfl_up(x, d, 64);
+        if (lane >= d) x += y;
+    }
+    if (lane == 63) sW[w] = x;
+    __syncthreads();
+    int run = lo + x - sum;
+    for (int k = 0; k < w; ++k) run += sW[k];
+    for (int j = j0; j < j1; ++j) {
+        const int c = sCnt[j];
+        sCnt[j] = run;
+        run += c;
+    }
+    __syncthreads();
+    for (int j = tid; j < nc; j += NBX_SMALL_T) cell_start[e.cbase + j] = sCnt[j];
+    const int t0 = e.cbase / D3F_SCAN_TILE, t1 = (e.cbase + nc - (b == B - 1 ? 0 : 1)) / D3F_SCAN_TILE;
+    for (int t = t0 + tid; t <= t1; t += NBX_SMALL_T) cell_base[t] = 0;
+    if (b == B - 1 && tid == 0) cell_start[e.cbase + nc] = n;
+    for (int i = lo + tid; i < hi; i += NBX_SMALL_T) {
+        const int pos = sCnt[cell_of[i] - e.cbase] + inv[i];
+        const float px = s[3 * (size_t)i], py = s[3 * (size_t)i + 1], pz = s[3 * (size_t)i + 2];
+        sorted[pos] = make_float4(px, py, pz, __int_as_float(i));
+        order[pos] = i;
+        inv[i] = pos;
+        xyz[3 * (size_t)pos] = px; xyz[3 * (size_t)pos + 1] = py; xyz[3 * (size_t)pos + 2] = pz;
+    }
 }
 
 template <int J>
@@ -376,6 +520,10 @@
 #include "nb_nearest.h"
 #include "nb_overlap.h"
 
+static int nb_env(const char* name, int dflt) {
+    const char* e = getenv(name);
+    return e ? atoi(e) : dflt;
+}
 static long long nb_cell_budget(int Ns) {
     long long b = 4ll * (long long)(Ns > 0 ? Ns : 1);
     if (b < (1ll << 16)) b = 1ll << 16;
@@ -472,10 +620,80 @@
     return D3F_OK;
 }
 
-static int nb_env(const char* name, int dflt) {
-    const char* e = getenv(name);
-    return e ? atoi(e) : dflt;
-}
+static int nbx_small_t() { return nb_env("D3F_NB_SMALL_T", 4096); }
+static bool nbx_is_small(int Ns, int B) { return d3f_cdiv(Ns > 0 ? Ns : 0, B) <= nbx_small_t(); }
+static long long nbx_per(int Ns, int B, bool small) {
+    const long long per = nb_cell_budget(Ns) / B;
+    return (small && per > NBX_LDS_CELLS) ? NBX_LDS_CELLS : per;
+}
+
+extern "C" int d3f_neighbor_grid_boxed_form(int Ns, int B) {
+    if (Ns < 0 || B < 1 || B > D3F_MAX_BATCH) return 0;
+    return nbx_is_small(Ns, B) ? 1 : 2;
+}
+
+struct NbxReset {
+    unsigned* boxes; int n_box_words; int n;
+    D3fFill f[2 * D3F_GRID_RESET_MAX];
+};
+__global__ void __launch_bounds__(256) nbx_reset_kernel(NbxReset R) {
+    const size_t tid = (size_t)blockIdx.x * blockDim.x + threadIdx.x, stride = (size_t)gridDim.x * blockDim.x;
+    for (size_t i = tid; i < (size_t)R.n_box_words; i += stride) R.boxes[i] = ((i % 6) < 3) ? 0xFFFFFFFFu : 0u;
+    for (int k = 0; k < R.n; ++k) d3f_fill_words(R.f[k], tid, stride);
+}
+extern "C" int d3f_geometry_reset(unsigned* boxes_dev, int n_boxes, const void* const* grids, const size_t* grid_bytes, const int* Ns,
+                                  const int* B, int n_grids, void* stream_) {
+    hipStream_t stream = (hipStream_t)stream_;
+    if (n_boxes < 0 || (n_boxes > 0 && !boxes_dev) || n_grids < 0 || n_grids > D3F_GRID_RESET_MAX ||
+        (n_grids > 0 && (!grids || !grid_bytes || !Ns || !B)))
+        return D3F_ERR_ARG;
+    NbxReset R;
+    R.boxes = boxes_dev; R.n_box_words = 6 * n_boxes; R.n = 0;
+    unsigned long long words = (unsigned long long)R.n_box_words;
+    for (int k = 0; k < n_grids; ++k) {
+        if (Ns[k] < 0 || B[k] < 1 || B[k] > D3F_MAX_BATCH || !grids[k]) return D3F_ERR_ARG;
+        if (nbx_is_small(Ns[k], B[k])) continue;
+        NbGrid g = nb_carve((void*)grids[k], grid_bytes[k], Ns[k], B[k]);
+        if (!g.ok) return D3F_ERR_WORKSPACE;
+        R.f[R.n++] = D3fFill{(unsigned*)g.cell_cnt, (unsigned long long)g.cells, 0u};
+        R.f[R.n++] = D3fFill{g.counters, 2ull, 0u};
+        words += (unsigned long long)g.cells + 2ull;
+    }
+    if (words == 0) return D3F_OK;
+    long long blocks = (long long)(words / 4 / 256) + 1;
+    if (blocks > 1024) blocks = 1024;
+    nbx_reset_kernel<<<(int)blocks, 256, 0, stream>>>(R);
+    D3F_LAUNCH_CHECK();
+    return D3F_OK;
+}
+
+extern "C" int d3f_neighbor_grid_build_boxed(const float* supports, int Ns, const int* s_lens_dev, int B, float radius,
+                                             const unsigned* bbox_dev, void* grid, size_t grid_bytes, void* stream_) {
+    hipStream_t stream = (hipStream_t)stream_;
+    if (Ns < 0 || B < 1 || B > D3F_MAX_BATCH || !(radius >= 0.f) || !s_lens_dev || (Ns > 0 && !supports) || !grid || !bbox_dev)
+        return D3F_ERR_ARG;
+    NbGrid g = nb_carve(grid, grid_bytes, Ns, B);
+    if (!g.ok) return D3F_ERR_WORKSPACE;
+    const bool small = nbx_is_small(Ns, B);
+    const long long per = nbx_per(Ns, B, small);
+    if (small) {
+        nbx_small_kernel<<<B, NBX_SMALL_T, 0, stream>>>(supports, Ns, s_lens_dev, B, bbox_dev, radius, per, g.soffs, g.el, g.ncells,
+                                                        g.cell_of, g.cell_start, g.stmp, g.sorted, g.order, g.inv, g.xyz);
+        D3F_LAUNCH_CHECK();
+        return D3F_OK;
+    }
+    int rc;
+    nbx_count_kernel<<<d3f_cdiv(Ns, NBX_COUNT_PTS), 256, 0, stream>>>(supports, Ns, s_lens_dev, B, bbox_dev, radius, per, g.soffs, g.el,
+                                                                      g.ncells, g.cell_of, g.cell_cnt, g.inv);
+    D3F_LAUNCH_CHECK();
+    if ((rc = d3f_scan_fold_launch(D3fScanIn{g.cell_cnt}, (int)g.cells, g.ncells + 1, g.cell_start, g.stmp, g.counters + 1, D3fNoEpi{},
+                                   stream)) != D3F_OK) return rc;
+    nbx_scatter_kernel<<<d3f_cdiv(Ns, 256), 256, 0, stream>>>(supports, Ns, g.soffs + B, g.cell_of, g.cell_start, g.stmp, g.sorted,
+                                                              g.order, g.inv, g.xyz);
+    D3F_LAUNCH_CHECK();
+    return D3F_OK;
+}
+
 static int nb_search_dispatch(const NbGrid& g, const float* queries, int Nq, const int* q_lens_dev, int B, float radius,
                               const float4* qsorted, bool queries_are_supports, int* out, int ld, int width, int pad_value, int cap,
                               int first_only, float nn_hint, int want_kmax, int* status_dev, hipStream_t stream, bool internal = false) {
diff --git a/d3feat_amd/datasets/common.py b/d3feat_amd/datasets/common.py
--- a/d3feat_amd/datasets/common.py
+++ b/d3feat_amd/datasets/common.py
@@ -233,7 +233,9 @@
         layer_blocks = []
         hints = getattr(self, 'hints', None)
         units = max(int(getattr(self, 'cap_units', 1)), 1)
-        grids.append(ops.NeighborGrid(stacked_points, lens_dev, r_normal))
+        chain = getattr(self, 'grid_chain', None)
+        box = (lambda l: chain.box(l) if chain.boxed[l] else None) if chain is not None else (lambda l: None)
+        grids.append(ops.NeighborGrid(stacked_points, lens_dev, r_normal, chain=chain, level=0))
         for block_i, block in enumerate(arch):
             if 'global' in block or 'upsample' in block:
                 break
@@ -251,8 +253,9 @@
                 pool_p, pool_b, _ = ops.batch_grid_subsample_async(P, L, dl, caps[layer + 1], status=status(),
                                                                    m_hint=hints[layer + 1] if hints else 0,
                                                                    elem_cap=-(-caps[layer + 1] // units),
-                                                                   elem_points=-(-caps[layer] // units))
-                Gn = ops.NeighborGrid(pool_p, pool_b, 2 * r_normal)
+                                                                   elem_points=-(-caps[layer] // units),
+                                                                   bbox_in=box(layer), bbox_out=box(layer + 1))
+                Gn = ops.NeighborGrid(pool_p, pool_b, 2 * r_normal, chain=chain, level=layer + 1)
             neighbors.append(search(G, P, L, G, layer) if layer_blocks else empty_i)
             if pooled:
                 pools.append(search(G, pool_p, pool_b, Gn, layer))
diff --git a/d3feat_amd/engine.py b/d3feat_amd/engine.py
--- a/d3feat_amd/engine.py
+++ b/d3feat_amd/engine.py
@@ -93,10 +93,17 @@
 
     def _sequence(self, sl):
         cfg = self.cfg
+        chain = sl.chain
+        box0 = chain.box(0) if chain is not None and chain.boxed[0] else None
+        stacked_here = not (self.mirror or self.two)
+        pre = chain.pre[: self.nin] if box0 is not None and stacked_here else None
+        if chain is not None:
+            chain.reset()
         if self.stage0:
             sub, sub_l, st0 = ops.batch_grid_subsample_async(None, sl.raw_len, cfg.first_subsampling_dl, self.F * self.n0_cap,
                                                              status=sl.status0, m_hint=self.F * self.n0_hint,
-                                                             elem_cap=self.n0_cap, clouds=sl.raw_ptrs, n_cap=self.F * self.raw_cap)
+                                                             elem_cap=self.n0_cap, clouds=sl.raw_ptrs, n_cap=self.F * self.raw_cap,
+                                                             bbox_out=pre if stacked_here else box0)
         else:
             sub, sub_l = sl.raw, sl.raw_len
             sub.n_hint = self.F * self.n0_hint
@@ -106,7 +113,7 @@
         if self.mirror or self.two:
             pts, lens = sub, sub_l
         else:
-            pts, lens = ops.stack_self_pair(sub, sub_l)
+            pts, lens = ops.stack_self_pair(sub, sub_l, bbox_in=pre, bbox_out=box0 if pre is not None else None)
         flat = sl.map(pts, None, None, None, lens, ("a", "a"), pts)
         with ops.bf16_contraction(self.bf16, features=self.bf16_features):
             desc, score = self.model.run(flat)
@@ -154,6 +161,11 @@
         sl.ds.cap_units = self.cap_units
         sl.ds.stack_group = 1 if self.mirror else 2
         sl.ds.internal_order = self.internal
+        sl.chain = None
+        if ops.GRID_BOXED and self.internal and len(self.caps) <= _lib.GRID_RESET_MAX:
+            fed = not self.stage0
+            sl.chain = ops.GridChain(self.caps, self.F * (1 if self.mirror else 2), dev, boxed=[not fed] + [True] * (len(self.caps) - 1))
+        sl.ds.grid_chain = sl.chain
         sl.ds._neighbor_cap = self.neighbor_cap
         sl.cap = self.neighbor_cap
         sl.map = sl.ds.get_tf_mapping(self.cfg)
diff --git a/d3feat_amd/ops.py b/d3feat_amd/ops.py
--- a/d3feat_amd/ops.py
+++ b/d3feat_amd/ops.py
@@ -182,7 +182,8 @@
     return sub_p[:M], sub_l, (sub_f[:M] if fdim else None), (sub_c[:M] if ldim else None)
 
 
-def batch_grid_subsample_async(points, lens, dl, m_cap, status=None, m_hint=0, elem_cap=0, elem_points=0, clouds=None, n_cap=0):
+def batch_grid_subsample_async(points, lens, dl, m_cap, status=None, m_hint=0, elem_cap=0, elem_points=0, clouds=None, n_cap=0,
+                               bbox_in=None, bbox_out=None):
     lib = _lib.load()
     if clouds is not None:
         assert points is None and clouds.dtype == torch.int64 and clouds.is_contiguous() and int(n_cap) > 0
@@ -200,7 +201,14 @@
     nbytes = lib.d3f_grid_subsample_workspace_bytes(N, B, 0, 0)
     ws = workspace(nbytes, dev)
     with _timed("grid_subsample", dict(N=N, M=int(m_cap)), dev):
-        if clouds is not None:
+        if bbox_in is not None or bbox_out is not None:
+            assert all(b is None or (b.dtype == torch.int32 and b.is_contiguous() and b.numel() == 6 * B) for b in (bbox_in, bbox_out))
+            assert clouds is None or clouds.numel() == B
+            rc = lib.d3f_batch_grid_subsample_async_boxed(_ptr(points), _ptr(clouds), N, lens_t.data_ptr(), B, float(dl),
+                                                          sub_p.data_ptr(), int(m_cap), int(elem_cap), int(elem_points),
+                                                          sub_l.data_ptr(), status.data_ptr(), _ptr(bbox_in), _ptr(bbox_out),
+                                                          ws.data_ptr(), ws.numel(), _stream(dev))
+        elif clouds is not None:
             assert clouds.numel() == B
             rc = lib.d3f_batch_grid_subsample_async_inplace(clouds.data_ptr(), N, lens_t.data_ptr(), B, float(dl), sub_p.data_ptr(),
                                                             int(m_cap), int(elem_cap), sub_l.data_ptr(), status.data_ptr(),
@@ -231,7 +239,7 @@
     return dst
 
 
-def stack_self_pair(pts, lens=None):
+def stack_self_pair(pts, lens=None, bbox_in=None, bbox_out=None):
     lib = _lib.load()
     pts = _req(pts, torch.float32, "pts", 2).contiguous()
     dev = pts.device
@@ -244,18 +252,61 @@
     out = torch.empty((2 * cap, 3), dtype=torch.float32, device=dev)
     lens_out = torch.empty((2 * B,), dtype=torch.int32, device=dev)
     total = torch.empty((1,), dtype=torch.int32, device=dev)
-    rc = lib.d3f_stack_self_pair(pts.data_ptr(), cap, lens.data_ptr(), B, out.data_ptr(), lens_out.data_ptr(),
-                                 total.data_ptr(), _stream(dev))
+    if bbox_out is not None:
+        assert bbox_out.dtype == torch.int32 and bbox_out.is_contiguous() and bbox_out.numel() == 12 * B
+        assert bbox_in is not None and bbox_in.dtype == torch.int32 and bbox_in.is_contiguous() and bbox_in.numel() == 6 * B
+        rc = lib.d3f_stack_self_pair_boxed(pts.data_ptr(), cap, lens.data_ptr(), B, out.data_ptr(), lens_out.data_ptr(),
+                                           total.data_ptr(), bbox_in.data_ptr(), bbox_out.data_ptr(), _stream(dev))
+    else:
+        rc = lib.d3f_stack_self_pair(pts.data_ptr(), cap, lens.data_ptr(), B, out.data_ptr(), lens_out.data_ptr(),
+                                     total.data_ptr(), _stream(dev))
     _lib.check(rc, "stack_self_pair")
     out.n_dev = total
     out.n_hint = 2 * int(getattr(pts, "n_hint", 0) or 0)
     return out, lens_out
 
 
+GRID_BOXED = os.environ.get("D3F_GRID_BOXED", "1") != "0"
+
+
+class GridChain:
+
+    def __init__(self, rows, B, device, boxed=None):
+        lib = _lib.load()
+        self.rows, self.B = [int(r) for r in rows], int(B)
+        self.boxed = list(boxed) if boxed is not None else [True] * len(self.rows)
+        assert len(self.rows) <= _lib.GRID_RESET_MAX and len(self.boxed) == len(self.rows)
+        self.boxes = torch.zeros((len(self.rows) + 1, self.B, 6), dtype=torch.int32, device=device)
+        self.pre = self.boxes[len(self.rows)]
+        self.nbytes = [lib.d3f_neighbor_grid_bytes(r, self.B) for r in self.rows]
+        self.mems = [torch.empty((n,), dtype=torch.uint8, device=device) for n in self.nbytes]
+        self.forms = [lib.d3f_neighbor_grid_boxed_form(r, self.B) if on else 0 for r, on in zip(self.rows, self.boxed)]
+
+    def box(self, level):
+        return self.boxes[level]
+
+    def reset(self):
+        import ctypes
+        lib = _lib.load()
+        ks = [k for k, on in enumerate(self.boxed) if on]
+        n = len(ks)
+        grids = (ctypes.c_void_p * max(n, 1))(*[self.mems[k].data_ptr() for k in ks])
+        nbytes = (ctypes.c_size_t * max(n, 1))(*[self.nbytes[k] for k in ks])
+        rows = (ctypes.c_int * max(n, 1))(*[self.rows[k] for k in ks])
+        Bs = (ctypes.c_int * max(n, 1))(*([self.B] * n))
+        rc = lib.d3f_geometry_reset(self.boxes.data_ptr(), self.boxes.numel() // 6, ctypes.addressof(grids), ctypes.addressof(nbytes),
+                                    ctypes.addressof(rows), ctypes.addressof(Bs), n, _stream(self.boxes.device))
+        _lib.check(rc, "geometry_reset")
+
+
 class NeighborGrid:
 
-    def __init__(self, supports, s_lens, radius):
+    def __init__(self, supports, s_lens, radius, chain=None, level=0):
         lib = _lib.load()
+        if chain is not None and chain.boxed[level]:
+            self._init_boxed(lib, supports, s_lens, radius, chain, level)
+            self._views(lib)
+            return
         self.supports = _tag(_req(supports, torch.float32, "supports", 2).contiguous(), supports)
         dev = self.supports.device
         self.Ns = self.supports.shape[0]
@@ -268,6 +319,27 @@
             rc = lib.d3f_neighbor_grid_build(self.supports.data_ptr(), self.Ns, self.s_lens.data_ptr(), self.B, self.radius,
                                              self.mem.data_ptr(), self.nbytes, _stream(dev))
         _lib.check(rc, "neighbor_grid_build")
+        self._views(lib)
+
+    def _init_boxed(self, lib, supports, s_lens, radius, chain, level):
+        self.supports = _tag(_req(supports, torch.float32, "supports", 2).contiguous(), supports)
+        dev = self.supports.device
+        self.Ns = self.supports.shape[0]
+        self.s_lens = as_lens(s_lens, dev)
+        self.B = self.s_lens.numel()
+        self.radius = float(radius)
+        if self.Ns != chain.rows[level] or self.B != chain.B:
+            raise ValueError("grid chain level %d was laid out for %d rows / %d clouds, not %d / %d"
+                             % (level, chain.rows[level], chain.B, self.Ns, self.B))
+        self.nbytes, self.mem = chain.nbytes[level], chain.mems[level]
+        self.form = chain.forms[level]
+        with _timed("nb_grid_build", dict(Ns=self.Ns), dev):
+            rc = lib.d3f_neighbor_grid_build_boxed(self.supports.data_ptr(), self.Ns, self.s_lens.data_ptr(), self.B, self.radius,
+                                                   chain.box(level).data_ptr(), self.mem.data_ptr(), self.nbytes, _stream(dev))
+        _lib.check(rc, "neighbor_grid_build_boxed")
+
+    def _views(self, lib):
+        dev = self.supports.device
         off = lib.d3f_neighbor_grid_order_offset(self.Ns, self.B)
         self.order = self.mem[off: off + 4 * max(self.Ns, 1)].view(torch.int32)
         off = lib.d3f_neighbor_grid_inv_offset(self.Ns, self.B)
diff --git a/include/d3feat_amd.h b/include/d3feat_amd.h
--- a/include/d3feat_amd.h
+++ b/include/d3feat_amd.h
@@ -50,6 +50,12 @@
 
 int d3f_stack_self_pair(const float* pts, int M_cap, const int* lens_in_dev, int B, float* out, int* lens_out_dev,
                         int* total_dev, void* stream);
+int d3f_stack_self_pair_boxed(const float* pts, int M_cap, const int* lens_in_dev, int B, float* out, int* lens_out_dev,
+                              int* total_dev, const unsigned* bbox_in_dev, unsigned* bbox_out_dev, void* stream);
+int d3f_batch_grid_subsample_async_boxed(const float* points, const float* const* clouds_dev, int N_cap, const int* lens_dev,
+                                         int B, float dl, float* sub_points, int M_cap, int elem_cap, int elem_points_cap,
+                                         int* sub_lens_dev, int* status_dev, const unsigned* bbox_in_dev,
+                                         unsigned* bbox_out_dev, void* workspace, size_t workspace_bytes, void* stream);
 int d3f_batch_grid_subsample(const float* points, int N, const int* lens_dev, int B, float dl,
                              const float* features, int fdim, const int* classes, int ldim,
                              float* sub_points, float* sub_features, int* sub_classes, int* sub_lens_dev,
@@ -65,6 +71,12 @@
 size_t d3f_neighbor_grid_order_offset(int Ns, int B);
 int d3f_neighbor_grid_build(const float* supports, int Ns, const int* s_lens_dev, int B, float radius,
                             void* grid, size_t grid_bytes, void* stream);
+#define D3F_GRID_RESET_MAX 8
+int d3f_neighbor_grid_boxed_form(int Ns, int B);
+int d3f_geometry_reset(unsigned* boxes_dev, int n_boxes, const void* const* grids, const size_t* grid_bytes, const int* Ns,
+                       const int* B, int n_grids, void* stream);
+int d3f_neighbor_grid_build_boxed(const float* supports, int Ns, const int* s_lens_dev, int B, float radius,
+                                  const unsigned* bbox_dev, void* grid, size_t grid_bytes, void* stream);
 int d3f_neighbor_grid_search(const void* grid, size_t grid_bytes, int Ns, const float* queries, int Nq,
                              const int* q_lens_dev, int B, float radius, int queries_are_supports,
                              int* out, int ld, int width, int pad_value, int cap, int first_only, float nn_hint,
```

Measured after the change: 1962 fragments/s, median of 6. 2.1% higher.
